# jonepatr/lets_face_it

Measured on AMD Instinct MI355X. Metric: FLAME frames/s, full training step (fwd+bwd+clip+Adam), final_model.yaml batch 256 per GPU, higher is better.
Workload: dtype f32 (GEMM operands split into bf16 hi+lo, f32 accumulate; three products in the forward GEMMs, two in the backward GEMMs)

## Files before the change

### include/lfi.h

```cpp
#ifndef LFI_H
#define LFI_H

#ifdef __cplusplus
extern "C" {
#endif

#define LFI_OK 0
#define LFI_ERR_ARG (-1)
#define LFI_ERR_LAUNCH (-2)
#define LFI_ERR_UNSUPPORTED (-3)

const char* lfi_last_error(void);
int lfi_version(void);

typedef struct {
  int M, N, K;
  const float* A; long lda; int a_kcontig;
  const float* B; long ldb; int b_kcontig;
  float* C; long ldc;
  const float* bias;
  const float* G; long ldg;
  int batch; long strideA, strideB, strideC, strideBias, strideG;
  int accumulate;
  int act; float slope;
  int splitk; float* work;
  int precision;
  int a_bf16;
  float* colsum_part; long ld_part;
} lfi_gemm_desc;

long lfi_gemm_work_floats(const lfi_gemm_desc* d);
long lfi_gemm_colpart_rows(const lfi_gemm_desc* d);
int lfi_gemm_f32(const lfi_gemm_desc* d, void* stream);

long lfi_planes_elems(long rows, int cols);
int lfi_planes_from_f32(const float* X, long ldx, long rows, int cols, void* planes, void* stream);
typedef struct {
  int M, N, K;
  const void* Ap; int a_nkt; long a_stride;
  const void* Bp; int b_nkt; long b_stride;
  float* C; long ldc;
  const float* bias; const float* G; long ldg;
  int batch; long strideC, strideBias, strideG;
  int accumulate, act; float slope;
  int skip;
  int a_fmt, b_fmt;
  int splitk; float* work;
  int store_f32;
  void* Cr; int cr_nkt; long cr_col0;
  const void* Gr; int gr_nkt; long gr_col0;
  float* colsum_part; long ld_part;
  int out_hi_only;
  int tile;
} lfi_pgemm_desc;
long lfi_gemm_planes_work_floats(const lfi_pgemm_desc* d);
long lfi_gemm_planes_colpart_rows(const lfi_pgemm_desc* d);
int lfi_gemm_planes(const lfi_pgemm_desc* d, void* stream);

long lfi_colsum_work_floats(int rows, int cols, int batch);
int lfi_colsum_f32(const float* X, long ldx, long strideX, int rows, int cols, int batch,
                   float* out, long strideOut, float scale, int accumulate, float* work, void* stream);

int lfi_cols_fold(const float* src, long lds, long rows, const int* a, const int* b, int ncols, float* dst, long ldd,
                  void* stream);

typedef struct {
  int B, T, N, start;
  int hist, hid;
  int ldcond, col;
  int precision;
  int dup;
  int lstm;
  int bwd_two_products;
  int stash_f16;
} lfi_enc_desc;

long lfi_encode_windows_work_floats(const lfi_enc_desc* d);
int lfi_encode_windows_fwd(const lfi_enc_desc* d, const float* Xp, const float* whh ,
                           const float* b_ih, const float* b_hh, const float* mask,
                           float* cond, float* gates, float* hseq, float* work, void* stream);
int lfi_encode_windows_bwd(const lfi_enc_desc* d, const float* dcond, int lddcond, const float* whh ,
                           const float* gates, const float* hseq, float* dgi, float* dgh,
                           float* bias_part , float* work, void* stream);
long lfi_encode_windows_bias_rows(const lfi_enc_desc* d);
int lfi_encode_windows_bias_grads(const float* bias_part, long rows, int hid, float* db_ih, float* db_hh, void* stream);
int lfi_encode_windows_compact_dgi(const lfi_enc_desc* d);
int lfi_encode_windows_grad_stash_bf16(const lfi_enc_desc* d);
int lfi_encode_windows_stash_f16_ok(const lfi_enc_desc* d);
int lfi_encode_windows_fwd_variant(const lfi_enc_desc* d, int masked, int stashed);
int lfi_encode_windows_scatter(const lfi_enc_desc* d, const float* dgi, const float* dgh, const float* mask, float* dXp,
                               void* stream);
int lfi_gather_windows(const float* X, int B, int T, int dim, int N, int start, int hist, int incl, const float* mask,
                       float* cond, int ldcond, int col, void* stream);
int lfi_pad_rows(const float* src, long rows, int cols, long lds, float* dst, long ldd, void* stream);
int lfi_dropout_masks(int count, float* const* out, const long* n, const float* keep, unsigned long long seed,
                      unsigned long long offset, void* stream);
int lfi_fill_frame_nb(const float* base, float offset, int B, int N, float* cond, int ldcond, int col, void* stream);
int lfi_leaky_grad(float* d, long ldd, const float* y, long ldy, int rows, int cols, float slope, void* stream);

typedef struct {
  int B, N, C, H, D, Ks;
  int affine;
  int lstm;
  float scale_eps;
  int gemm_precision;
} lfi_flow_dims;

typedef struct {
  const float *an_bias, *an_logs;
  const float *inv_l, *inv_u, *inv_logs;
  const float *inv_p, *inv_sign;
  const float *inv_w;
  const float *w_ih, *w_hh, *b_ih, *b_hh;
  const float *w_fl, *b_fl, *l_fl;
} lfi_flow_params;

long lfi_flow_prep_floats(const lfi_flow_dims* d);
int lfi_flow_prep(const lfi_flow_dims* d, const lfi_flow_params* p, float* prep, int with_inverse, void* stream);

long lfi_flow_stash_floats(const lfi_flow_dims* d);
int lfi_flow_seq_fwd(const lfi_flow_dims* d, const lfi_flow_params* p, const float* prep,
                     const float* x0, int T, int start, const float* gic,
                     float* stash, float* z, float* nll, void* stream);
long lfi_flow_bstash_floats(const lfi_flow_dims* d);
int lfi_flow_seq_bwd(const lfi_flow_dims* d, const lfi_flow_params* p, const float* prep,
                     const float* stash, float gscale, float* bstash, void* stream);

int lfi_flow_bwd_emits_planes(const lfi_flow_dims* d);
int lfi_flow_seq_bwd_planes(const lfi_flow_dims* d, const lfi_flow_params* p, const float* prep,
                            const float* stash, float gscale, float* bstash, void* dgi_planes,
                            int hi_only , void* stream);

typedef struct {
  float *an_bias, *an_logs, *inv_l, *inv_u, *inv_logs, *inv_w;
  float *w_ih, *w_hh, *b_ih, *b_hh, *w_fl, *b_fl, *l_fl;
} lfi_flow_grads;
long lfi_flow_param_grads_work_floats(const lfi_flow_dims* d);
int lfi_flow_param_grads(const lfi_flow_dims* d, const lfi_flow_params* p, const float* prep,
                         const float* stash, const float* bstash, const float* c, long ldc, float gscale,
                         const lfi_flow_grads* g, int accumulate, float* work, void* stream,
                         void* bias_stream );

float* lfi_flow_stash_ptr(const lfi_flow_dims* d, float* stash, int which);
float* lfi_flow_bstash_ptr(const lfi_flow_dims* d, float* bstash, int which);

int lfi_actnorm_init_stats(const float* x, int rows, int C, double* sums, void* stream);
int lfi_actnorm_init_apply(const double* sums, double count, int C, float scale, float* bias, float* logs, void* stream);
int lfi_flow_step(const lfi_flow_dims* d, const lfi_flow_params* p, const float* prep, int k, int rows,
                  const float* x_in, long ldx, const float* h_prev, const float* c_prev, const float* gic_k,
                  float* x_out, long ldxo, float* h_out, float* c_out, float* ldc_acc, int reverse, void* stream);
int lfi_flow_seq_rev_ok(const lfi_flow_dims* d);
long lfi_flow_seq_rev_work_floats(const lfi_flow_dims* d);
int lfi_flow_seq_rev(const lfi_flow_dims* d, const lfi_flow_params* p, const float* prep, const float* z, const float* gic,
                     float* x_out, float* logdet, float* h, float* cstate, float* work, void* stream);

int lfi_actnorm_forward(const float* x, int rows, int C, const float* bias, const float* logs, int reverse, float* out,
                        float* dlogdet, void* stream);
long lfi_invconv_work_floats(int C);
int lfi_invconv_weights(int C, const float* inv_l, const float* inv_u, const float* inv_logs, const float* inv_p,
                        const float* inv_sign, const float* inv_w, int with_inverse, float* W, float* Winv, float* dlogdet,
                        float* work, void* stream);

typedef struct {
  int kind, hid;
  const float *w1, *b1;
  const float *w_ih, *w_hh, *b_ih, *b_hh;
  int col;
} lfi_p1enc;

long lfi_flow_sample_work_floats(const lfi_flow_dims* d);
long lfi_flow_sample_p1_work_floats(const lfi_flow_dims* d, const lfi_p1enc* e, int hist1);
int lfi_flow_sample_seq(const lfi_flow_dims* d, const lfi_flow_params* p, const float* prep,
                        const float* wct , long E, int hist1,
                        float* pre_static, const float* noise,
                        float* faces, int seq_len, int start, int nframes,
                        float* h, float* cstate ,
                        const lfi_p1enc* p1 , float* p1work ,
                        float* work, void* stream);
int lfi_absmax_f32(int count, const float* const* ptrs, const long* n, unsigned* out_bits, void* stream);
int lfi_stream_create_partial(int cus_per_xcd, void** stream);
int lfi_stream_destroy(void* stream);
int lfi_flow_sample_seq_from(const lfi_flow_dims* d, const lfi_flow_params* p, const float* prep,
                             const float* wct, long E, int hist1, float* pre_static, const float* noise,
                             float* faces, int seq_len, int start, int nframes, int first_frame,
                             float* h, float* cstate, const lfi_p1enc* p1, float* p1work, float* work, void* stream);
long lfi_flow_sample_nll_work_floats(const lfi_flow_dims* d);
int lfi_flow_sample_seq_nll(const lfi_flow_dims* d, const lfi_flow_params* p, const float* prep,
                            const float* wct, long E, int hist1, float* pre_static, const float* noise,
                            float* faces, int seq_len, int start, int nframes, int first_frame,
                            float* h, float* cstate, const lfi_p1enc* p1, float* p1work, float* work,
                            float* nll, float* nll_work, void* stream);
long lfi_flow_score_work_floats(const lfi_flow_dims* d);
int lfi_flow_score_seq_from(const lfi_flow_dims* d, const lfi_flow_params* p, const float* prep,
                            const float* wct, long E, int hist1, float* pre_static,
                            float* faces, int seq_len, int start, int nframes, int first_frame,
                            float* h, float* cstate, const lfi_p1enc* p1, float* p1work, float* work,
                            float* score_work, float* z, float* nll, void* stream);
long lfi_flow_step_rows_work_floats(const lfi_flow_dims* d);
int lfi_flow_step_rows_from(const lfi_flow_dims* d, const lfi_flow_params* p, const float* prep,
                            const float* wct, long E, int hist1, float* pre_static, const float* noise,
                            float* faces, int seq_len, int start, int nframes, int first_frame,
                            float* h, float* cstate, const lfi_p1enc* p1, float* p1work, float* work,
                            float* nll, float* nll_work, const int* observed, float* rows_work, void* stream);
int lfi_stream_advance(int B, int count, float* const* win, const float* const* src, const int* hist, const int* dim,
                       const float* noise, float* noise_dst, int C, float* frame_nb, unsigned* guard_bits, void* stream);
int lfi_stream_advance_rows(int B, int count, float* const* win, const float* const* src, const int* hist, const int* dim,
                            int face_win, const float* noise, float* noise_dst, int C, float* frame_nb,
                            const unsigned char* observed, int* role, unsigned* guard_bits, void* stream);
int lfi_stream_reset_rows(int B, int nrows, const int* rows, int count, float* const* win, const float* const* seed,
                          const long* seed_ld, const int* hist, const int* dim, const int* lead_zero, float* h, float* cstate,
                          int Ks, int H, float* frame_nb, unsigned* guard_bits, void* stream);
long lfi_stream_row_floats(int count, const int* hist, const int* dim, int Ks, int H, int lstm, int has_frame_nb);
int lfi_stream_save_rows(int B, int nrows, const int* rows, int count, const float* const* win, const int* hist, const int* dim,
                         const float* h, const float* cstate, int Ks, int H, const float* frame_nb, int zero_state, float* out,
                         long ld_out, void* stream);
int lfi_stream_load_rows(int B, int nrows, const int* rows, const int* entries, int nentries, int count, float* const* win,
                         const int* hist, const int* dim, float* h, float* cstate, int Ks, int H, float* frame_nb, const float* in,
                         long ld_in, unsigned* guard_bits, void* stream);

int lfi_grad_sumsq(const float* g, long n, double* sumsq, double* work , void* stream);
int lfi_adam_clip_step(float* p, const float* g, float* m, float* v, long n, const double* sumsq,
                       float clip, float gmul, float lr, float beta1, float beta2, float eps, int step_count,
                       void* stream);

int lfi_adam_clip_step_ex(float* p, const float* g, float* m, float* v, float* vmax, long n, const double* sumsq, float clip,
                          float gmul, float lr, float beta1, float beta2, float eps, float weight_decay, int step_count,
                          const float* hyper, void* stream);

int lfi_sgd_clip_step(float* p, const float* g, float* buf, long n, const double* sumsq, float clip, float gmul, float lr,
                      float momentum, float dampening, float weight_decay, int nesterov, int step_count, void* stream);
int lfi_rmsprop_clip_step(float* p, const float* g, float* sq, float* buf, float* gavg, long n, const double* sumsq, float clip,
                          float gmul, float lr, float alpha, float eps, float weight_decay, float momentum, void* stream);

int lfi_set_step_params(void* params, unsigned long long seed, unsigned long long offset, float step_size, float inv_sqrt_bc2,
                        void* stream);
int lfi_dropout_masks_dev(int count, float* const* out, const long* n, const float* keep, const unsigned long long* seed_offset,
                          void* stream);
int lfi_adam_clip_step_dev(float* p, const float* g, float* m, float* v, long n, const double* sumsq, float clip, float gmul,
                           float beta1, float beta2, float eps, const float* hyper , void* stream);

int lfi_gather_sequences(const float* src, long rows, int dim, const long* starts, int B, int T, float* dst, void* stream);
int lfi_jerk_mean(const float* x, int B, int T, int C, float* out, double* work , void* stream);

int lfi_debug_set_stamps(void* device_buffer);
int lfi_selftest_mfma(int* out, void* stream);

#ifdef __cplusplus
}
#endif
#endif
```

### lets_face_it_amd/_lib.py

```python
import ctypes as C
import os

_HERE = os.path.dirname(os.path.abspath(__file__))
LIB_PATH = os.environ.get("LFI_LIB_PATH") or os.path.join(_HERE, "liblfi_hip.so")

c_float_p = C.POINTER(C.c_float)
c_double_p = C.POINTER(C.c_double)


class GemmDesc(C.Structure):
    _fields_ = [
        ("M", C.c_int), ("N", C.c_int), ("K", C.c_int),
        ("A", C.c_void_p), ("lda", C.c_long), ("a_kcontig", C.c_int),
        ("B", C.c_void_p), ("ldb", C.c_long), ("b_kcontig", C.c_int),
        ("C", C.c_void_p), ("ldc", C.c_long),
        ("bias", C.c_void_p),
        ("G", C.c_void_p), ("ldg", C.c_long),
        ("batch", C.c_int), ("strideA", C.c_long), ("strideB", C.c_long), ("strideC", C.c_long),
        ("strideBias", C.c_long), ("strideG", C.c_long),
        ("accumulate", C.c_int),
        ("act", C.c_int), ("slope", C.c_float),
        ("splitk", C.c_int), ("work", C.c_void_p),
        ("precision", C.c_int), ("a_bf16", C.c_int),
        ("colsum_part", C.c_void_p), ("ld_part", C.c_long),
    ]


class PGemmDesc(C.Structure):
    _fields_ = [
        ("M", C.c_int), ("N", C.c_int), ("K", C.c_int),
        ("Ap", C.c_void_p), ("a_nkt", C.c_int), ("a_stride", C.c_long),
        ("Bp", C.c_void_p), ("b_nkt", C.c_int), ("b_stride", C.c_long),
        ("C", C.c_void_p), ("ldc", C.c_long),
        ("bias", C.c_void_p), ("G", C.c_void_p), ("ldg", C.c_long),
        ("batch", C.c_int), ("strideC", C.c_long), ("strideBias", C.c_long), ("strideG", C.c_long),
        ("accumulate", C.c_int), ("act", C.c_int), ("slope", C.c_float), ("skip", C.c_int),
        ("a_fmt", C.c_int), ("b_fmt", C.c_int),
        ("splitk", C.c_int), ("work", C.c_void_p),
        ("store_f32", C.c_int),
        ("Cr", C.c_void_p), ("cr_nkt", C.c_int), ("cr_col0", C.c_long),
        ("Gr", C.c_void_p), ("gr_nkt", C.c_int), ("gr_col0", C.c_long),
        ("colsum_part", C.c_void_p), ("ld_part", C.c_long),
        ("out_hi_only", C.c_int), ("tile", C.c_int),
    ]


class EncDesc(C.Structure):
    _fields_ = [("B", C.c_int), ("T", C.c_int), ("N", C.c_int), ("start", C.c_int),
                ("hist", C.c_int), ("hid", C.c_int), ("ldcond", C.c_int), ("col", C.c_int), ("precision", C.c_int),
                ("dup", C.c_int), ("lstm", C.c_int), ("bwd_two_products", C.c_int), ("stash_f16", C.c_int)]


class FlowDims(C.Structure):
    _fields_ = [("B", C.c_int), ("N", C.c_int), ("C", C.c_int), ("H", C.c_int), ("D", C.c_int), ("Ks", C.c_int),
                ("affine", C.c_int), ("lstm", C.c_int), ("scale_eps", C.c_float), ("gemm_precision", C.c_int)]


_FLOW_PARAM_FIELDS = ["an_bias", "an_logs", "inv_l", "inv_u", "inv_logs", "inv_p", "inv_sign", "inv_w",
                      "w_ih", "w_hh", "b_ih", "b_hh", "w_fl", "b_fl", "l_fl"]
_FLOW_GRAD_FIELDS = ["an_bias", "an_logs", "inv_l", "inv_u", "inv_logs", "inv_w",
                     "w_ih", "w_hh", "b_ih", "b_hh", "w_fl", "b_fl", "l_fl"]


class P1Enc(C.Structure):
    _fields_ = [("kind", C.c_int), ("hid", C.c_int), ("w1", C.c_void_p), ("b1", C.c_void_p), ("w_ih", C.c_void_p),
                ("w_hh", C.c_void_p), ("b_ih", C.c_void_p), ("b_hh", C.c_void_p), ("col", C.c_int)]


class FlowParams(C.Structure):
    _fields_ = [(n, C.c_void_p) for n in _FLOW_PARAM_FIELDS]


class FlowGrads(C.Structure):
    _fields_ = [(n, C.c_void_p) for n in _FLOW_GRAD_FIELDS]


class LfiError(RuntimeError):
    pass


_lib = None


def lib():
    global _lib
    if _lib is not None:
        return _lib
    if not os.path.exists(LIB_PATH):
        raise LfiError(
            "liblfi_hip.so not found at %s: build it with `make -C lets_face_it_amd/csrc` "
            "(there is no fallback path)" % LIB_PATH)
    L = C.CDLL(LIB_PATH)
    vp, i, l, f, d = C.c_void_p, C.c_int, C.c_long, C.c_float, C.c_double
    P = C.POINTER
    sig = {
        "lfi_last_error": (C.c_char_p, []),
        "lfi_version": (i, []),
        "lfi_gemm_work_floats": (l, [P(GemmDesc)]),
        "lfi_gemm_f32": (i, [P(GemmDesc), vp]),
        "lfi_gemm_colpart_rows": (l, [P(GemmDesc)]),
        "lfi_planes_elems": (l, [l, i]),
        "lfi_planes_from_f32": (i, [vp, l, l, i, vp, vp]),
        "lfi_gemm_planes": (i, [P(PGemmDesc), vp]),
        "lfi_flow_bwd_emits_planes": (i, [P(FlowDims)]),
        "lfi_flow_seq_bwd_planes": (i, [P(FlowDims), P(FlowParams), vp, vp, f, vp, vp, i, vp]),
        "lfi_encode_windows_grad_stash_bf16": (i, [P(EncDesc)]),
        "lfi_encode_windows_stash_f16_ok": (i, [P(EncDesc)]),
        "lfi_encode_windows_fwd_variant": (i, [P(EncDesc), i, i]),
        "lfi_gemm_planes_work_floats": (l, [P(PGemmDesc)]),
        "lfi_gemm_planes_colpart_rows": (l, [P(PGemmDesc)]),
        "lfi_colsum_work_floats": (l, [i, i, i]),
        "lfi_colsum_f32": (i, [vp, l, l, i, i, i, vp, l, f, i, vp, vp]),
        "lfi_cols_fold": (i, [vp, l, l, vp, vp, i, vp, l, vp]),
        "lfi_encode_windows_work_floats": (l, [P(EncDesc)]),
        "lfi_encode_windows_fwd": (i, [P(EncDesc), vp, vp, vp, vp, vp, vp, vp, vp, vp, vp]),
        "lfi_encode_windows_bwd": (i, [P(EncDesc), vp, i, vp, vp, vp, vp, vp, vp, vp, vp]),
        "lfi_encode_windows_bias_rows": (l, [P(EncDesc)]),
        "lfi_encode_windows_bias_grads": (i, [vp, l, i, vp, vp, vp]),
        "lfi_encode_windows_compact_dgi": (i, [P(EncDesc)]),
        "lfi_encode_windows_scatter": (i, [P(EncDesc), vp, vp, vp, vp, vp]),
        "lfi_gather_windows": (i, [vp, i, i, i, i, i, i, i, vp, vp, i, i, vp]),
        "lfi_pad_rows": (i, [vp, l, i, l, vp, l, vp]),
        "lfi_dropout_masks": (i, [i, P(vp), P(l), P(f), C.c_ulonglong, C.c_ulonglong, vp]),
        "lfi_dropout_masks_dev": (i, [i, P(vp), P(l), P(f), vp, vp]),
        "lfi_set_step_params": (i, [vp, C.c_ulonglong, C.c_ulonglong, f, f, vp]),
        "lfi_adam_clip_step_dev": (i, [vp, vp, vp, vp, l, vp, f, f, f, f, f, vp, vp]),
        "lfi_leaky_grad": (i, [vp, l, vp, l, i, i, f, vp]),
        "lfi_fill_frame_nb": (i, [vp, f, i, i, vp, i, i, vp]),
        "lfi_flow_prep_floats": (l, [P(FlowDims)]),
        "lfi_flow_prep": (i, [P(FlowDims), P(FlowParams), vp, i, vp]),
        "lfi_flow_stash_floats": (l, [P(FlowDims)]),
        "lfi_flow_bstash_floats": (l, [P(FlowDims)]),
        "lfi_flow_stash_ptr": (vp, [P(FlowDims), vp, i]),
        "lfi_flow_bstash_ptr": (vp, [P(FlowDims), vp, i]),
        "lfi_flow_seq_fwd": (i, [P(FlowDims), P(FlowParams), vp, vp, i, i, vp, vp, vp, vp, vp]),
        "lfi_flow_seq_bwd": (i, [P(FlowDims), P(FlowParams), vp, vp, f, vp, vp]),
        "lfi_flow_param_grads_work_floats": (l, [P(FlowDims)]),
        "lfi_flow_param_grads": (i, [P(FlowDims), P(FlowParams), vp, vp, vp, vp, l, f, P(FlowGrads), i, vp, vp, vp]),
        "lfi_actnorm_init_stats": (i, [vp, i, i, vp, vp]),
        "lfi_actnorm_init_apply": (i, [vp, d, i, f, vp, vp, vp]),
        "lfi_flow_step": (i, [P(FlowDims), P(FlowParams), vp, i, i, vp, l, vp, vp, vp, vp, l, vp, vp, vp, i, vp]),
        "lfi_flow_seq_rev_ok": (i, [P(FlowDims)]),
        "lfi_flow_seq_rev_work_floats": (l, [P(FlowDims)]),
        "lfi_flow_seq_rev": (i, [P(FlowDims), P(FlowParams), vp, vp, vp, vp, vp, vp, vp, vp, vp]),
        "lfi_flow_sample_work_floats": (l, [P(FlowDims)]),
        "lfi_flow_sample_p1_work_floats": (l, [P(FlowDims), P(P1Enc), i]),
        "lfi_flow_sample_seq": (i, [P(FlowDims), P(FlowParams), vp, vp, l, i, vp, vp, vp, i, i, i, vp, vp, P(P1Enc), vp, vp,
                                    vp]),
        "lfi_flow_sample_seq_from": (i, [P(FlowDims), P(FlowParams), vp, vp, l, i, vp, vp, vp, i, i, i, i, vp, vp, P(P1Enc), vp, vp,
                                         vp]),
        "lfi_flow_sample_nll_work_floats": (l, [P(FlowDims)]),
        "lfi_flow_sample_seq_nll": (i, [P(FlowDims), P(FlowParams), vp, vp, l, i, vp, vp, vp, i, i, i, i, vp, vp, P(P1Enc), vp, vp,
                                        vp, vp, vp]),
        "lfi_flow_score_work_floats": (l, [P(FlowDims)]),
        "lfi_flow_score_seq_from": (i, [P(FlowDims), P(FlowParams), vp, vp, l, i, vp, vp, i, i, i, i, vp, vp, P(P1Enc), vp, vp,
                                        vp, vp, vp, vp]),
        "lfi_flow_step_rows_work_floats": (l, [P(FlowDims)]),
        "lfi_flow_step_rows_from": (i, [P(FlowDims), P(FlowParams), vp, vp, l, i, vp, vp, vp, i, i, i, i, vp, vp, P(P1Enc), vp, vp,
                                        vp, vp, vp, vp, vp]),
        "lfi_absmax_f32": (i, [i, P(vp), P(l), vp, vp]),
        "lfi_stream_advance": (i, [i, i, P(vp), P(vp), P(i), P(i), vp, vp, i, vp, vp, vp]),
        "lfi_stream_advance_rows": (i, [i, i, P(vp), P(vp), P(i), P(i), i, vp, vp, i, vp, vp, vp, vp, vp]),
        "lfi_stream_reset_rows": (i, [i, i, P(i), i, P(vp), P(vp), P(l), P(i), P(i), P(i), vp, vp, i, i, vp, vp, vp]),
        "lfi_stream_row_floats": (l, [i, P(i), P(i), i, i, i, i]),
        "lfi_stream_save_rows": (i, [i, i, P(i), i, P(vp), P(i), P(i), vp, vp, i, i, vp, i, vp, l, vp]),
        "lfi_stream_load_rows": (i, [i, i, P(i), P(i), i, i, P(vp), P(i), P(i), vp, vp, i, i, vp, vp, l, vp, vp]),
        "lfi_stream_create_partial": (i, [i, P(vp)]),
        "lfi_stream_destroy": (i, [vp]),
        "lfi_grad_sumsq": (i, [vp, l, vp, vp, vp]),
        "lfi_adam_clip_step": (i, [vp, vp, vp, vp, l, vp, f, f, f, f, f, f, i, vp]),
        "lfi_adam_clip_step_ex": (i, [vp, vp, vp, vp, vp, l, vp, f, f, f, f, f, f, f, i, vp, vp]),
        "lfi_sgd_clip_step": (i, [vp, vp, vp, l, vp, f, f, f, f, f, f, i, i, vp]),
        "lfi_rmsprop_clip_step": (i, [vp, vp, vp, vp, vp, l, vp, f, f, f, f, f, f, f, vp]),
        "lfi_actnorm_forward": (i, [vp, i, i, vp, vp, i, vp, vp, vp]),
        "lfi_invconv_work_floats": (l, [i]),
        "lfi_invconv_weights": (i, [i, vp, vp, vp, vp, vp, vp, i, vp, vp, vp, vp, vp]),
        "lfi_gather_sequences": (i, [vp, l, i, vp, i, i, vp, vp]),
        "lfi_jerk_mean": (i, [vp, i, i, i, vp, vp, vp]),
        "lfi_selftest_mfma": (i, [vp, vp]),
        "lfi_debug_set_stamps": (i, [vp]),
    }
    for name, (res, args) in sig.items():
        fn = getattr(L, name)
        fn.restype = res
        fn.argtypes = args
    _lib = L
    return L


EXPORTS = [
    "lfi_last_error", "lfi_version", "lfi_gemm_work_floats", "lfi_gemm_f32", "lfi_gemm_colpart_rows", "lfi_planes_elems", "lfi_planes_from_f32",
    "lfi_gemm_planes", "lfi_gemm_planes_work_floats", "lfi_gemm_planes_colpart_rows",
    "lfi_flow_bwd_emits_planes", "lfi_flow_seq_bwd_planes", "lfi_encode_windows_grad_stash_bf16", "lfi_encode_windows_stash_f16_ok", "lfi_encode_windows_fwd_variant", "lfi_colsum_work_floats",
    "lfi_colsum_f32", "lfi_cols_fold", "lfi_encode_windows_work_floats", "lfi_encode_windows_fwd", "lfi_encode_windows_bwd",
    "lfi_encode_windows_bias_rows", "lfi_encode_windows_bias_grads",
    "lfi_encode_windows_scatter", "lfi_encode_windows_compact_dgi", "lfi_gather_windows", "lfi_pad_rows", "lfi_dropout_masks", "lfi_leaky_grad", "lfi_fill_frame_nb", "lfi_flow_prep_floats", "lfi_flow_prep",
    "lfi_flow_stash_floats", "lfi_flow_bstash_floats", "lfi_flow_stash_ptr", "lfi_flow_bstash_ptr",
    "lfi_flow_seq_fwd", "lfi_flow_seq_bwd", "lfi_flow_param_grads_work_floats", "lfi_flow_param_grads",
    "lfi_actnorm_init_stats", "lfi_actnorm_init_apply", "lfi_flow_step", "lfi_flow_seq_rev_ok", "lfi_flow_seq_rev_work_floats",
    "lfi_flow_seq_rev", "lfi_flow_sample_work_floats",
    "lfi_flow_sample_p1_work_floats", "lfi_flow_sample_seq", "lfi_flow_sample_seq_from", "lfi_flow_sample_nll_work_floats", "lfi_flow_sample_seq_nll", "lfi_flow_score_work_floats", "lfi_flow_score_seq_from", "lfi_flow_step_rows_work_floats", "lfi_flow_step_rows_from", "lfi_absmax_f32", "lfi_stream_advance", "lfi_stream_advance_rows", "lfi_stream_reset_rows", "lfi_stream_row_floats",
    "lfi_stream_save_rows", "lfi_stream_load_rows", "lfi_stream_create_partial", "lfi_stream_destroy", "lfi_grad_sumsq", "lfi_adam_clip_step", "lfi_adam_clip_step_ex",
    "lfi_sgd_clip_step", "lfi_rmsprop_clip_step", "lfi_set_step_params", "lfi_dropout_masks_dev", "lfi_adam_clip_step_dev", "lfi_selftest_mfma", "lfi_debug_set_stamps",
    "lfi_gather_sequences", "lfi_jerk_mean", "lfi_actnorm_forward", "lfi_invconv_work_floats", "lfi_invconv_weights",
]


def translate_oom(fn):
    import functools

    import torch

    @functools.wraps(fn)
    def wrapper(*args, **kwargs):
        try:
            return fn(*args, **kwargs)
        except torch.OutOfMemoryError as e:
            msg = str(e)
            if msg.startswith("CUDA out of memory"):
                raise
            raise torch.OutOfMemoryError("CUDA out of memory. [ROCm: " + msg + "]") from e

    return wrapper


def check(rc, what=""):
    if rc != 0:
        msg = lib().lfi_last_error()
        raise LfiError("%s failed (%d): %s" % (what or "lfi call", rc, msg.decode() if msg else ""))


def ptr(t):
    return None if t is None else t.data_ptr()
```

### lets_face_it_amd/csrc/lfi_gemm_common.h

```cpp
#pragma once
#include <stdarg.h>
#include <stdio.h>
#include <stdlib.h>

#include "lfi_common.h"

namespace {

#ifndef LFI_GEMM_BKT
#define LFI_GEMM_BKT 16
#endif
#ifndef LFI_GEMM_LDSPIPE
#define LFI_GEMM_LDSPIPE 1
#endif
constexpr int BKT = LFI_GEMM_BKT;
#define LFI_GSKIP(bit) (XT >= 2 && (g.skip & (bit)))

struct GemmArgs {
  int M, N, K;
  const float* A; long lda;
  const float* B; long ldb;
  float* C; long ldc;
  const float* bias;
  const float* G; long ldg;
  long strideA, strideB, strideC, strideBias, strideG;
  int accumulate, act;
  float slope;
  int splitk, kchunk;
  float* work;
  int tiles_m, tiles_n;
  int vecA, vecB;
  int vecC;
  const __bf16* Ap; const __bf16* Bp;
  int nkt, nktA, nktB;
  long pstrideA, pstrideB;
  float* colpart; long ldpart;
  int gm;
  int skip;
  int storeC;
  __bf16* Cr; int nktCr; long colCr;
  const __bf16* Gr; int nktGr; long colGr;
  int hiOnly;
};

__device__ __forceinline__ float apply_act(float v, int act, float slope, const float* G, long gidx) {
  if (act == 1) return v > 0.0f ? v : v * slope;
  if (act == 2) return G[gidx] > 0.0f ? v : v * slope;
  return v;
}

typedef __bf16 bf16x8 __attribute__((ext_vector_type(8)));
typedef __bf16 bf16x4 __attribute__((ext_vector_type(4)));
extern __shared__ __attribute__((aligned(16))) __bf16 xsmem[];
typedef __bf16 bf16x2 __attribute__((ext_vector_type(2)));
typedef float float2_t __attribute__((ext_vector_type(2)));

__device__ __forceinline__ void split2(float a, float b, unsigned* hi, unsigned* lo) {
  const bf16x2 h = __builtin_convertvector((float2_t){a, b}, bf16x2);
  const unsigned hb = __builtin_bit_cast(unsigned, h);
  const float ha = __builtin_bit_cast(float, hb << 16), hbv = __builtin_bit_cast(float, hb & 0xffff0000u);
  const bf16x2 l = __builtin_convertvector((float2_t){a - ha, b - hbv}, bf16x2);
  *hi = hb;
  *lo = __builtin_bit_cast(unsigned, l);
}


__device__ __forceinline__ void gemm_epilogue(const GemmArgs& g, const f32x16 (&acc)[2][2], int m0, int n0, int wm, int wn,
                                              int l31, int half, int batch, int split) {
  const bool partial = g.splitk > 1;
  float* __restrict__ Cb = partial ? g.work + ((long)batch * g.splitk + split) * (long)g.M * g.N : g.C + batch * g.strideC;
  const long ldc = partial ? g.N : g.ldc;
  const float* bias = g.bias ? g.bias + batch * g.strideBias : nullptr;
  const float* G = g.G ? g.G + batch * g.strideG : nullptr;
  const bool need_c = !partial && g.accumulate != 0, need_g = !partial && g.act == 2;
#pragma unroll
  for (int mt = 0; mt < 2; ++mt)
#pragma unroll
    for (int nt = 0; nt < 2; ++nt) {
      const int col = n0 + wn * 64 + nt * 32 + l31;
      if (col >= g.N) continue;
      const float bv = (!partial && bias) ? bias[col] : 0.0f;
      float cold[16], gold[16];
#pragma unroll
      for (int r = 0; r < 16; ++r) {
        const int row = min(m0 + wm * 64 + mt * 32 + (r & 3) + 8 * (r >> 2) + 4 * half, g.M - 1);
        cold[r] = need_c ? Cb[(long)row * ldc + col] : 0.0f;
        gold[r] = need_g ? G[(long)row * g.ldg + col] : 1.0f;
      }
#pragma unroll
      for (int r = 0; r < 16; ++r) {
        const int row = m0 + wm * 64 + mt * 32 + (r & 3) + 8 * (r >> 2) + 4 * half;
        if (row >= g.M) continue;
        float v = acc[mt][nt][r];
        if (!partial) {
          v += bv;
          if (g.accumulate == 2) v += cold[r];
          if (g.act == 1) v = v > 0.0f ? v : v * g.slope;
          else if (g.act == 2) v = gold[r] > 0.0f ? v : v * g.slope;
          if (g.accumulate == 1) v += cold[r];
        }
        Cb[(long)row * ldc + col] = v;
      }
    }
}

template <int BN>
__device__ __forceinline__ void gemm_epilogue_n(const GemmArgs& g, const f32x16 (&acc)[2][2], int m0, int n0, int wm, int wn,
                                                int l31, int half, int batch, int split) {
  gemm_epilogue(g, acc, m0, n0, wm, wn, l31, half, batch, split);
}

typedef unsigned u32x4 __attribute__((ext_vector_type(4)));
__device__ __forceinline__ u32x4 pg_u4(const uint4& v) { return (u32x4){v.x, v.y, v.z, v.w}; }
template <int BN, int NTH>
__device__ __forceinline__ void gemm_emit_planes(const GemmArgs& g, const float* lds, int rows_per_pass, int row0, int n0, int batch) {
  constexpr int WLD = BN + 4;
  const int tid = threadIdx.x, lane = tid & 63, wave = tid >> 6;
  constexpr int NW = NTH / 64;
  const long gcol0 = (long)batch * g.strideC + n0;
  if (!g.Cr) return;
  constexpr int KT = BN / 16;
  const int nb = (rows_per_pass / 32) * KT;
  const int uoff = lfi_u_plane_offset(lane & 31, lane >> 5);
  for (int b = wave; b < nb; b += NW) {
    const int rtl = b / KT, ktl = b - rtl * KT;
    if (row0 + rtl * 32 >= g.M || n0 + ktl * 16 >= g.N) continue;
    const int r = rtl * 32 + (lane & 31), c = ktl * 16 + (lane >> 5) * 8;
    const f32x4 a = *reinterpret_cast<const f32x4*>(lds + r * WLD + c), bq = *reinterpret_cast<const f32x4*>(lds + r * WLD + c + 4);
    const bool rok = row0 + r < g.M;
    float v[8] = {a[0], a[1], a[2], a[3], bq[0], bq[1], bq[2], bq[3]};
#pragma unroll
    for (int e = 0; e < 8; ++e) v[e] = (rok && n0 + c + e < g.N) ? v[e] : 0.0f;
    uint4 h, l;
    split2(v[0], v[1], &h.x, &l.x); split2(v[2], v[3], &h.y, &l.y);
    split2(v[4], v[5], &h.z, &l.z); split2(v[6], v[7], &h.w, &l.w);
    const long rt = (row0 + rtl * 32) >> 5, kt = (g.colCr + gcol0 + ktl * 16) >> 4;
    char* dst = reinterpret_cast<char*>(g.Cr) + ((rt * g.nktCr + kt) * 2) * 1024 + uoff;
    __builtin_nontemporal_store(pg_u4(h), reinterpret_cast<u32x4*>(dst));
    if (!g.hiOnly) __builtin_nontemporal_store(pg_u4(l), reinterpret_cast<u32x4*>(dst + 1024));
  }
}
template <int BN, int NTH>
__device__ __forceinline__ void gemm_sign_tile_from_planes(const GemmArgs& g, float* lds, int rows_per_pass, int row0, int n0, int batch) {
  constexpr int WLD = BN + 4, KT = BN / 16, NW = NTH / 64;
  const int tid = threadIdx.x, lane = tid & 63, wave = tid >> 6;
  const long gcol0 = (long)batch * g.strideC + n0;
  const int nb = (rows_per_pass / 32) * KT;
  for (int b = wave; b < nb; b += NW) {
    const int rtl = b / KT, ktl = b - rtl * KT;
    const int r = rtl * 32 + (lane & 31), c = ktl * 16 + (lane >> 5) * 8;
    uint4 h = {0u, 0u, 0u, 0u};
    if (row0 + rtl * 32 < g.M && n0 + ktl * 16 < g.N) {
      const long rt = (row0 + rtl * 32) >> 5, kt = (g.colGr + gcol0 + ktl * 16) >> 4;
      h = *reinterpret_cast<const uint4*>(reinterpret_cast<const char*>(g.Gr) + ((rt * g.nktGr + kt) * 2) * 1024 +
                                          lfi_u_plane_offset(lane & 31, lane >> 5));
    }
    f32x4 a, bq;
    a[0] = __builtin_bit_cast(float, h.x << 16); a[1] = __builtin_bit_cast(float, h.x & 0xffff0000u);
    a[2] = __builtin_bit_cast(float, h.y << 16); a[3] = __builtin_bit_cast(float, h.y & 0xffff0000u);
    bq[0] = __builtin_bit_cast(float, h.z << 16); bq[1] = __builtin_bit_cast(float, h.z & 0xffff0000u);
    bq[2] = __builtin_bit_cast(float, h.w << 16); bq[3] = __builtin_bit_cast(float, h.w & 0xffff0000u);
    *reinterpret_cast<f32x4*>(lds + r * WLD + c) = a;
    *reinterpret_cast<f32x4*>(lds + r * WLD + c + 4) = bq;
  }
}

template <int BN, int NTH = 256, int MT = 2, bool COLP = false, bool PL = false, bool L16 = false, typename ACC>
__device__ __forceinline__ void gemm_epilogue_wide(const GemmArgs& g, const ACC& acc, float* lds, int rows_per_pass,
                                                   int m0, int n0, int wm, int wn, int l31, int half, int batch, int split, int bm,
                                                   bool has_acc = true) {
  constexpr int WLD = BN + 4;
  constexpr int F4 = BN / 4;
  constexpr int SWEEP = NTH / F4;
  const int tid = threadIdx.x;
  const bool partial = g.splitk > 1;
  float* __restrict__ Cb = partial ? g.work + ((long)batch * g.splitk + split) * (long)g.M * g.N : g.C + batch * g.strideC;
  const long ldc = partial ? g.N : g.ldc;
  const float* bias = g.bias ? g.bias + batch * g.strideBias : nullptr;
  const float* G = g.G ? g.G + batch * g.strideG : nullptr;
  const bool need_c = !partial && g.accumulate != 0, need_g = !partial && g.act == 2;
  const int rrow = tid / F4, c4 = (tid % F4) * 4;
  const int col_g = n0 + c4;
  for (int p0 = 0; p0 < bm; p0 += rows_per_pass) {
    if (PL && need_g && g.Gr) {
      gemm_sign_tile_from_planes<BN, NTH>(g, lds, rows_per_pass, m0 + p0, n0, batch);
      __syncthreads();
    } else if (need_c || need_g) {
      const float* src = need_g ? G : Cb;
      const long lds_src = need_g ? g.ldg : ldc;
      for (int r = rrow; r < rows_per_pass; r += SWEEP) {
        const int row = m0 + p0 + r;
        f32x4 v = {0.f, 0.f, 0.f, 0.f};
        if (row < g.M && col_g < g.N) {
          if (col_g + 3 < g.N) v = *reinterpret_cast<const f32x4*>(src + (long)row * lds_src + col_g);
          else
            for (int j = 0; j < 4; ++j)
              if (col_g + j < g.N) v[j] = src[(long)row * lds_src + col_g + j];
        }
        *reinterpret_cast<f32x4*>(lds + r * WLD + c4) = v;
      }
      __syncthreads();
    }
    if constexpr (L16) {
      static_assert(!L16 || MT == 2, "16 x 16 accumulator tiles: 64-row patches");
      const int lane = threadIdx.x & 63, c15 = lane & 15, r4 = (lane >> 4) * 4;
#pragma unroll
      for (int mi = 0; mi < 4; ++mi)
        if (has_acc && wm * 64 + mi * 16 >= p0 && wm * 64 + mi * 16 < p0 + rows_per_pass)
#pragma unroll
        for (int ni = 0; ni < 4; ++ni) {
          const int cl = wn * 64 + ni * 16 + c15;
          const int col = n0 + cl;
          const float bv = (!partial && bias && col < g.N) ? bias[col] : 0.0f;
#pragma unroll
          for (int r = 0; r < 4; ++r) {
            const int rl = wm * 64 - p0 + mi * 16 + r4 + r;
            float v = acc[mi][ni][r];
            if (!partial) {
              v += bv;
              const float o = (need_c || need_g) ? lds[rl * WLD + cl] : 0.0f;
              if (g.accumulate == 2) v += o;
              if (g.act == 1) v = v > 0.0f ? v : v * g.slope;
              else if (g.act == 2) v = o > 0.0f ? v : v * g.slope;
              if (g.accumulate == 1) v += o;
            }
            lds[rl * WLD + cl] = v;
          }
        }
    } else
    if (has_acc) {
#pragma unroll
      for (int mt = 0; mt < MT; ++mt)
        if (wm * MT * 32 + mt * 32 >= p0 && wm * MT * 32 + mt * 32 < p0 + rows_per_pass)
#pragma unroll
        for (int nt = 0; nt < 2; ++nt) {
          const int cl = wn * 64 + nt * 32 + l31;
          const int col = n0 + cl;
          const float bv = (!partial && bias && col < g.N) ? bias[col] : 0.0f;
#pragma unroll
          for (int r = 0; r < 16; ++r) {
            const int rl = wm * MT * 32 - p0 + mt * 32 + (r & 3) + 8 * (r >> 2) + 4 * half;
            float v = acc[mt][nt][r];
            if (!partial) {
              v += bv;
              const float o = (need_c || need_g) ? lds[rl * WLD + cl] : 0.0f;
              if (g.accumulate == 2) v += o;
              if (g.act == 1) v = v > 0.0f ? v : v * g.slope;
              else if (g.act == 2) v = o > 0.0f ? v : v * g.slope;
              if (g.accumulate == 1) v += o;
            }
            lds[rl * WLD + cl] = v;
          }
        }
    }
    __syncthreads();
    if (PL && !partial) gemm_emit_planes<BN, NTH>(g, lds, rows_per_pass, m0 + p0, n0, batch);
    f32x4 csum = {0.f, 0.f, 0.f, 0.f};
    for (int r = rrow; r < rows_per_pass && (!PL || partial || g.storeC || COLP); r += SWEEP) {
      const int row = m0 + p0 + r;
      if (row < g.M && col_g < g.N) {
        const f32x4 v = *reinterpret_cast<const f32x4*>(lds + r * WLD + c4);
        if (COLP) csum += v;
        if (PL && !partial && !g.storeC) continue;
        if (col_g + 3 < g.N) {
#ifndef LFI_EPI_NT_MODE
#define LFI_EPI_NT_MODE 2
#endif
          if (LFI_EPI_NT_MODE == 0 || (LFI_EPI_NT_MODE == 2 && partial)) *reinterpret_cast<f32x4*>(Cb + (long)row * ldc + col_g) = v;
          else __builtin_nontemporal_store(v, reinterpret_cast<f32x4*>(Cb + (long)row * ldc + col_g));
        }
        else
          for (int j = 0; j < 4; ++j)
            if (col_g + j < g.N) Cb[(long)row * ldc + col_g + j] = v[j];
      }
    }
    if (COLP && g.colpart && !partial) {
      __syncthreads();
      *reinterpret_cast<f32x4*>(lds + rrow * WLD + c4) = csum;
      __syncthreads();
      if (tid < BN && n0 + tid < g.N) {
        float v = 0.0f;
        for (int i = 0; i < SWEEP; ++i) v += lds[i * WLD + tid];
        const int npass = (bm + rows_per_pass - 1) / rows_per_pass;
        g.colpart[((long)(m0 / bm) * npass + p0 / rows_per_pass) * g.ldpart + batch * g.strideC + n0 + tid] = v;
      }
      __syncthreads();
    } else if (p0 + rows_per_pass < bm) __syncthreads();
  }
}

typedef unsigned gu32x4 __attribute__((ext_vector_type(4)));
typedef unsigned gu32x2 __attribute__((ext_vector_type(2)));
template <int MODE>
__device__ __forceinline__ void gemm_epilogue_direct16(const GemmArgs& g, const f32x4 (&acc)[4][4], int m0, int n0, int wm, int wn, int lane,
                                                       int batch, int split) {
  const int l15 = lane & 15, g4 = lane >> 4;
  const int r0 = m0 + wm * 64, c0 = n0 + wn * 64;
  const float* bias = g.bias ? g.bias + batch * g.strideBias : nullptr;
  f32x4 bv[4];
#pragma unroll
  for (int j = 0; j < 4; ++j) {
    const int col = c0 + 16 * j + 4 * g4;
    bv[j] = (f32x4){0.f, 0.f, 0.f, 0.f};
    if (bias && col < g.N) bv[j] = *reinterpret_cast<const f32x4*>(bias + col);
  }
  static_assert(MODE == 3 || MODE == 4, "plane outputs only");
  f32x4 csum[4];
#pragma unroll
  for (int j = 0; j < 4; ++j) csum[j] = (f32x4){0.f, 0.f, 0.f, 0.f};
  {
    const long gcol0 = g.colCr + (long)batch * g.strideC + c0;
#pragma unroll
    for (int i = 0; i < 4; ++i) {
      const int row = r0 + 16 * i + l15;
      const bool blk = (r0 + 16 * (i & ~1)) < g.M;
      const long rt = (r0 + 16 * i) >> 5;
      const __amdgpu_buffer_rsrc_t rs = __builtin_amdgcn_make_buffer_rsrc(reinterpret_cast<char*>(g.Cr) + (rt * g.nktCr + (gcol0 >> 4)) * 2048, 0,
                                                                         0x7fffffff, 0x00020000);
      const unsigned voff = (unsigned)(lfi_u_plane_offset(16 * (i & 1) + l15, g4 >> 1) + (g4 & 1) * 8);
      __amdgpu_buffer_rsrc_t rg = rs;
      if constexpr (MODE == 4) {
        const long ggcol0 = g.colGr + (long)batch * g.strideC + c0;
        rg = __builtin_amdgcn_make_buffer_rsrc(const_cast<char*>(reinterpret_cast<const char*>(g.Gr)) + (rt * g.nktGr + (ggcol0 >> 4)) * 2048, 0,
                                               0x7fffffff, 0x00020000);
      }
#pragma unroll
      for (int j = 0; j < 4; ++j) {
        const int col = c0 + 16 * j + 4 * g4;
        f32x4 v = acc[i][j] + bv[j];
        if constexpr (MODE == 4) {
          gu32x2 m2 = {0u, 0u};
          if (blk && c0 + 16 * j < g.N) m2 = __builtin_amdgcn_raw_buffer_load_b64(rg, voff, 2048 * j, 0);
          const float o0 = __builtin_bit_cast(float, m2[0] << 16), o1 = __builtin_bit_cast(float, m2[0] & 0xffff0000u);
          const float o2 = __builtin_bit_cast(float, m2[1] << 16), o3 = __builtin_bit_cast(float, m2[1] & 0xffff0000u);
          v[0] = o0 > 0.0f ? v[0] : v[0] * g.slope; v[1] = o1 > 0.0f ? v[1] : v[1] * g.slope;
          v[2] = o2 > 0.0f ? v[2] : v[2] * g.slope; v[3] = o3 > 0.0f ? v[3] : v[3] * g.slope;
        } else if (g.act == 1) {
#pragma unroll
          for (int r = 0; r < 4; ++r) v[r] = v[r] > 0.0f ? v[r] : v[r] * g.slope;
        }
        if (row >= g.M || col >= g.N) v = (f32x4){0.f, 0.f, 0.f, 0.f};
        if constexpr (MODE == 4) csum[j] += v;
        uint2 h, l;
        split2(v[0], v[1], &h.x, &l.x);
        split2(v[2], v[3], &h.y, &l.y);
        if (blk && c0 + 16 * j < g.N) {
          __builtin_amdgcn_raw_buffer_store_b64((gu32x2){h.x, h.y}, rs, voff, 2048 * j, 2);
          if (!g.hiOnly) __builtin_amdgcn_raw_buffer_store_b64((gu32x2){l.x, l.y}, rs, voff, 2048 * j + 1024, 2);
        }
      }
    }
  }
  if constexpr (MODE == 4) {
    if (g.colpart) {
#pragma unroll
      for (int j = 0; j < 4; ++j) {
        f32x4 v = csum[j];
#pragma unroll
        for (int o = 1; o < 16; o <<= 1) {
#pragma unroll
          for (int r = 0; r < 4; ++r) v[r] += __shfl_xor(v[r], o, 64);
        }
        const int col = c0 + 16 * j + 4 * g4;
        if (l15 == 0 && col < g.N)
          *reinterpret_cast<f32x4*>(g.colpart + ((long)(m0 >> 7) * 2 + wm) * g.ldpart + (long)batch * g.strideC + col) = v;
      }
    }
  }
}

__device__ __forceinline__ void gemm_tile_of_block(const GemmArgs& g, int* tm, int* tn, int* batch, int* split) {
  const int ntile = g.tiles_m * g.tiles_n;
  const long total = (long)gridDim.x * gridDim.y * gridDim.z;
  long lin = blockIdx.x + (long)gridDim.x * (blockIdx.y + (long)gridDim.y * blockIdx.z);
  {
    const long q = total >> 3, idx = lin >> 3;
    const int r = (int)(total & 7), xcd = (int)(lin & 7);
    lin = (xcd < r ? xcd * (q + 1) : r * (q + 1) + (xcd - r) * q) + idx;
  }
  int bid = (int)(lin % ntile);
  const long rest = lin / ntile;
  *batch = (int)(rest % gridDim.y);
  *split = (int)(rest / gridDim.y);
  const int GM = g.gm > 0 ? g.gm : 8;
  const int per_group = GM * g.tiles_n;
  const int grp = bid / per_group, in_grp = bid - grp * per_group;
  const int rows_here = min(GM, g.tiles_m - grp * GM);
  *tm = grp * GM + in_grp % rows_here;
  *tn = in_grp / rows_here;
}

#ifndef LFI_EPI_ROWS
#define LFI_EPI_ROWS 128
#endif

__global__ __launch_bounds__(256) void gemm_splitk_reduce_kernel(GemmArgs g) {
  const long mn = (long)g.M * g.N;
  const int batch = blockIdx.y;
  const float* bias = g.bias ? g.bias + batch * g.strideBias : nullptr;
  const float* G = g.G ? g.G + batch * g.strideG : nullptr;
  float* C = g.C + batch * g.strideC;
  for (long i = (long)blockIdx.x * 256 + threadIdx.x; i < mn; i += (long)gridDim.x * 256) {
    const int row = (int)(i / g.N), col = (int)(i % g.N);
    const float* w = g.work + (long)batch * g.splitk * mn + i;
    float v = 0.0f;
    int s = 0;
    for (; s + 8 <= g.splitk; s += 8) {
      float t[8];
#pragma unroll
      for (int u = 0; u < 8; ++u) t[u] = w[(long)(s + u) * mn];
#pragma unroll
      for (int u = 0; u < 8; ++u) v += t[u];
    }
    for (; s < g.splitk; ++s) v += w[(long)s * mn];
    if (bias) v += bias[col];
    if (g.accumulate == 2) v += C[(long)row * g.ldc + col];
    v = apply_act(v, g.act, g.slope, G, (long)row * g.ldg + col);
    if (g.accumulate == 1) v += C[(long)row * g.ldc + col];
    C[(long)row * g.ldc + col] = v;
  }
}

__global__ __launch_bounds__(256) void gemm_splitk_reduce4_kernel(GemmArgs g) {
  const long mn = (long)g.M * g.N, mn4 = mn >> 2;
  const int n4 = g.N >> 2;
  const int batch = blockIdx.y;
  const float* bias = g.bias ? g.bias + batch * g.strideBias : nullptr;
  const float* G = g.G ? g.G + batch * g.strideG : nullptr;
  float* C = g.C + batch * g.strideC;
  for (long i = (long)blockIdx.x * 256 + threadIdx.x; i < mn4; i += (long)gridDim.x * 256) {
    const int row = (int)(i / n4), col = (int)(i - (long)row * n4) * 4;
    const float* w = g.work + (long)batch * g.splitk * mn + 4 * i;
    f32x4 v = {0.f, 0.f, 0.f, 0.f};
    int s = 0;
    for (; s + 8 <= g.splitk; s += 8) {
      f32x4 t[8];
#pragma unroll
      for (int u = 0; u < 8; ++u) t[u] = __builtin_nontemporal_load(reinterpret_cast<const f32x4*>(w + (long)(s + u) * mn));
#pragma unroll
      for (int u = 0; u < 8; ++u) v += t[u];
    }
    for (; s < g.splitk; ++s) v += __builtin_nontemporal_load(reinterpret_cast<const f32x4*>(w + (long)s * mn));
    f32x4* cp = reinterpret_cast<f32x4*>(C + (long)row * g.ldc + col);
    f32x4 c0 = {0.f, 0.f, 0.f, 0.f};
    if (g.accumulate) c0 = *cp;
#pragma unroll
    for (int j = 0; j < 4; ++j) {
      float x = v[j];
      if (bias) x += bias[col + j];
      if (g.accumulate == 2) x += c0[j];
      x = apply_act(x, g.act, g.slope, G, (long)row * g.ldg + col + j);
      if (g.accumulate == 1) x += c0[j];
      v[j] = x;
    }
    *cp = v;
  }
}

}
```

### lets_face_it_amd/csrc/lfi_pgemm.hip

```cpp
#include "lfi_gemm_common.h"
#include <type_traits>

namespace {

constexpr int QRING = 3;
constexpr int QSLOT = 24 * 1024;

typedef __attribute__((address_space(3))) void plds_void;
typedef __attribute__((address_space(1))) const void pglb_void;
typedef __bf16 pbf16x4 __attribute__((ext_vector_type(4)));
typedef __attribute__((address_space(3))) pbf16x4 plds_v4;

template <bool TF>
__device__ __forceinline__ bf16x8 pg_frag(const char* blk, int uoff, int toff) {
  if (!TF) return *reinterpret_cast<const bf16x8*>(blk + uoff);
  const pbf16x4 lo = __builtin_amdgcn_ds_read_tr16_b64_v4bf16((plds_v4*)(blk + toff));
  const pbf16x4 hi = __builtin_amdgcn_ds_read_tr16_b64_v4bf16((plds_v4*)(blk + (toff ^ 128)));
  bf16x8 r;
  r[0] = lo[0]; r[1] = lo[1]; r[2] = lo[2]; r[3] = lo[3];
  r[4] = hi[0]; r[5] = hi[1]; r[6] = hi[2]; r[7] = hi[3];
  return r;
}

#ifdef LFI_PG_EXP_16
__device__ __forceinline__ f32x16 pg_mfma16(bf16x8 a, bf16x8 b, f32x16 c) {
  f32x4 q0 = {c[0], c[1], c[2], c[3]}, q1 = {c[4], c[5], c[6], c[7]};
  q0 = __builtin_amdgcn_mfma_f32_16x16x32_bf16(a, b, q0, 0, 0, 0);
  q1 = __builtin_amdgcn_mfma_f32_16x16x32_bf16(a, b, q1, 0, 0, 0);
  c[0] = q0[0]; c[1] = q0[1]; c[2] = q0[2]; c[3] = q0[3];
  c[4] = q1[0]; c[5] = q1[1]; c[6] = q1[2]; c[7] = q1[3];
  return c;
}
#define PG_MFMA(a, b, c) pg_mfma16(a, b, c)
#else
#define PG_MFMA(a, b, c) __builtin_amdgcn_mfma_f32_32x32x16_bf16(a, b, c, 0, 0, 0)
#endif

template <bool AT, bool BT, bool COLP, int WMT, int WNT>
__global__ __launch_bounds__(512, 4) void gemm_planes_kernel(GemmArgs g) {
  constexpr int XT = 2;
  constexpr int NA = 4 * WMT;
  static_assert(WMT * WNT == 8 && NA + 4 * WNT == 24, "eight waves, 24 blocks per slot");
  const int tid = threadIdx.x;
  const int lane = tid & 63, wave = __builtin_amdgcn_readfirstlane(tid >> 6);
  const int l31 = lane & 31, half = lane >> 5;
  int tm, tn, batch, split;
  gemm_tile_of_block(g, &tm, &tn, &batch, &split);
  const int m0 = tm * 64 * WMT, n0 = tn * 64 * WNT;
  const bool noalo = LFI_GSKIP(1);
  const int ktc = g.kchunk >> 4;
  const int kt0 = split * ktc;
  const int nkt = max(min(g.nkt - kt0, ktc), 0);
  char* lds = reinterpret_cast<char*>(xsmem);
  const int tsub = lane >> 5, trow = ((lane & 31) >> 1) ^ (tsub << 2);
  const int lpT = tsub * 2048 + trow * 32 + (lane & 1) * 16, lpR = lane * 16;
  const char* baseA = reinterpret_cast<const char*>(g.Ap + batch * g.pstrideA) +
                      (AT ? (long)(tm * 2 * WMT) * 4096 + lpT : (long)(tm * 2 * WMT) * g.nktA * 2048 + lpR);
  const char* baseB = reinterpret_cast<const char*>(g.Bp + batch * g.pstrideB) +
                      (BT ? (long)(tn * 2 * WNT) * 4096 + lpT : (long)(tn * 2 * WNT) * g.nktB * 2048 + lpR);
  const char* src[3];
  int doff[3];
  bool srcB[3];
#pragma unroll
  for (int i = 0; i < 3; ++i) {
    const int j = wave * 3 + i;
    const int isB = j >= NA, jj = isB ? j - NA : j;
    const int plane = (!isB && noalo) ? 0 : (jj & 1);
    const long mt = jj >> 1;
    src[i] = (isB ? baseB + (BT ? mt * 4096 : mt * g.nktB * 2048) : baseA + (AT ? mt * 4096 : mt * g.nktA * 2048)) + plane * 1024;
    srcB[i] = isB != 0;
    doff[i] = j * 1024;
  }
  const long rowA = (long)g.nktA * 2048, rowB = (long)g.nktB * 2048;
  auto dma = [&](int kt, int slot) {
    const int ka = kt0 + max(min(kt, nkt - 1), 0);
    const long koA = AT ? (long)(ka >> 1) * rowA + (ka & 1) * 512 : (long)ka * 2048;
    const long koB = BT ? (long)(ka >> 1) * rowB + (ka & 1) * 512 : (long)ka * 2048;
#pragma unroll
    for (int i = 0; i < 3; ++i)
      __builtin_amdgcn_global_load_lds((pglb_void*)(src[i] + (srcB[i] ? koB : koA)), (plds_void*)(lds + slot * QSLOT + doff[i]), 16, 0, 0);
  };
  const int wm = wave / WNT, wn = wave % WNT;
  const int uoff = lfi_u_plane_offset(lane & 31, lane >> 5);
  const int tg = lane >> 4, tq = (lane >> 2) & 3, tp = lane & 3, tkh = tg >> 1, tmh = tg & 1;
  const int toff = tmh * 512 + (((tkh * 8 + tq) ^ (tmh << 2)) * 32) + (((tp >> 1) ^ tkh) << 4) + (tp & 1) * 8;
  const int fa = (wm * 4) * 1024;
  const int fb = NA * 1024 + (wn * 4) * 1024;
  auto fragA = [&](int slot, int off) { return pg_frag<AT>(lds + slot * QSLOT + fa + off, uoff, toff); };
  auto fragB = [&](int slot, int off) { return pg_frag<BT>(lds + slot * QSLOT + fb + off, uoff, toff); };

  f32x16 acc[2][2];
#pragma unroll
  for (int i = 0; i < 2; ++i)
#pragma unroll
    for (int j = 0; j < 2; ++j)
#pragma unroll
      for (int r = 0; r < 16; ++r) acc[i][j][r] = 0.0f;

  if (nkt > 0) {
    bf16x8 ah[2], al[2], bh[2], bl[2];
    dma(0, 0); dma(1, 1); dma(2, 2);
    asm volatile("s_waitcnt vmcnt(6)" ::: "memory");
    __builtin_amdgcn_s_barrier();
#pragma unroll
    for (int t2 = 0; t2 < 2; ++t2) {
      ah[t2] = fragA(0, (t2 * 2) * 1024);
      if (!noalo) al[t2] = fragA(0, (t2 * 2 + 1) * 1024);
      else al[t2] = ah[t2];
      bh[t2] = fragB(0, (t2 * 2) * 1024); bl[t2] = fragB(0, (t2 * 2 + 1) * 1024);
    }
    asm volatile("s_waitcnt vmcnt(3)\n\ts_waitcnt lgkmcnt(0)" ::: "memory");
    __builtin_amdgcn_s_barrier();

    int cur = 0;
    for (int t = 0; t < nkt; ++t) {
      const int nxt = cur == 2 ? 0 : cur + 1;
      bf16x8 nah[2], nal[2], nbh[2], nbl[2];
      dma(t + 3, cur);
      __builtin_amdgcn_sched_barrier(0);
      if (!LFI_GSKIP(1)) {
#pragma unroll
        for (int nt = 0; nt < 2; ++nt) acc[0][nt] = PG_MFMA(al[0], bh[nt], acc[0][nt]);
      }
      if (!LFI_GSKIP(2)) {
#pragma unroll
        for (int nt = 0; nt < 2; ++nt) acc[0][nt] = PG_MFMA(ah[0], bl[nt], acc[0][nt]);
      }
#pragma unroll
      for (int nt = 0; nt < 2; ++nt) acc[0][nt] = PG_MFMA(ah[0], bh[nt], acc[0][nt]);
      __builtin_amdgcn_sched_barrier(0);
      nah[0] = fragA(nxt, 0);
      if (!noalo) nal[0] = fragA(nxt, 1024);
      else nal[0] = nah[0];
#pragma unroll
      for (int nt = 0; nt < 2; ++nt) { nbh[nt] = fragB(nxt, (nt * 2) * 1024); nbl[nt] = fragB(nxt, (nt * 2 + 1) * 1024); }
      __builtin_amdgcn_sched_barrier(0);
      if (!LFI_GSKIP(1)) {
#pragma unroll
        for (int nt = 0; nt < 2; ++nt) acc[1][nt] = PG_MFMA(al[1], bh[nt], acc[1][nt]);
      }
      if (!LFI_GSKIP(2)) {
#pragma unroll
        for (int nt = 0; nt < 2; ++nt) acc[1][nt] = PG_MFMA(ah[1], bl[nt], acc[1][nt]);
      }
#pragma unroll
      for (int nt = 0; nt < 2; ++nt) acc[1][nt] = PG_MFMA(ah[1], bh[nt], acc[1][nt]);
      __builtin_amdgcn_sched_barrier(0);
      nah[1] = fragA(nxt, 2048);
      if (!noalo) nal[1] = fragA(nxt, 3072);
      else nal[1] = nah[1];
      asm volatile("s_waitcnt vmcnt(3)\n\ts_waitcnt lgkmcnt(0)" ::: "memory");
      __builtin_amdgcn_s_barrier();
#pragma unroll
      for (int i = 0; i < 2; ++i) { ah[i] = nah[i]; al[i] = nal[i]; bh[i] = nbh[i]; bl[i] = nbl[i]; }
      cur = nxt;
    }
    asm volatile("s_waitcnt vmcnt(0)" ::: "memory");
  }
  __syncthreads();
  if (g.vecC) gemm_epilogue_wide<64 * WNT, 512, 2, COLP, true>(g, acc, reinterpret_cast<float*>(xsmem), WNT == 4 ? 64 : 128, m0, n0, wm, wn,
                                                             l31, half, batch, split, 64 * WMT);
  else gemm_epilogue_n<64 * WNT>(g, acc, m0, n0, wm, wn, l31, half, batch, split);
}

#define PG_MFMA16(a, b, c) __builtin_amdgcn_mfma_f32_16x16x32_bf16(a, b, c, 0, 0, 0)
#define PG_MFMA16X(a, b, c) (TRP ? PG_MFMA16(b, a, c) : PG_MFMA16(a, b, c))
template <bool AT, bool BT, bool COLP, int WMT, int WNT, int TRP = 0>
__global__ __launch_bounds__(512, 4) void gemm_planes16_kernel(GemmArgs g) {
  constexpr int NA = 4 * WMT;
  static_assert(WMT * WNT == 8 && NA + 4 * WNT == 24, "eight waves, 24 blocks per slot");
  const int tid = threadIdx.x;
  const int lane = tid & 63, wave = __builtin_amdgcn_readfirstlane(tid >> 6);
  int tm, tn, batch, split;
  gemm_tile_of_block(g, &tm, &tn, &batch, &split);
  const int m0 = tm * 64 * WMT, n0 = tn * 64 * WNT;
  const int ktc = g.kchunk >> 4;
  const int kt0 = split * ktc;
  const int npair = max(min(g.nkt - kt0, ktc), 0) >> 1;
  char* lds = reinterpret_cast<char*>(xsmem);
  const long rowA = (long)g.nktA * 2048, rowB = (long)g.nktB * 2048;
  const char* baseA = reinterpret_cast<const char*>(g.Ap + batch * g.pstrideA) +
                      (AT ? (long)(tm * 2 * WMT) * 4096 + (long)(kt0 >> 1) * rowA : (long)(tm * 2 * WMT) * rowA + (long)kt0 * 2048);
  const char* baseB = reinterpret_cast<const char*>(g.Bp + batch * g.pstrideB) +
                      (BT ? (long)(tn * 2 * WNT) * 4096 + (long)(kt0 >> 1) * rowB : (long)(tn * 2 * WNT) * rowB + (long)kt0 * 2048);
  const int prow = lane >> 1, srow = prow ^ ((prow & 16) ? 4 : 0);
  const int laneR = lane * 16, laneT = srow * 32 + (lane & 1) * 16;
  int sof[3], doff[3];
#pragma unroll
  for (int i = 0; i < 3; ++i) {
    const int j = 8 * i + wave;
    const bool isB = 8 * i >= NA;
    const int jj = isB ? j - NA : j;
    const int mt = jj >> 1, h = jj & 1;
    const bool tr = isB ? BT : AT;
    sof[i] = (tr ? mt * 4096 : mt * (int)(isB ? rowB : rowA)) + h * 2048 + (isB ? 0 : 1024);
    doff[i] = j * 1024;
  }
#define PG_RSRC(ptr) __builtin_amdgcn_make_buffer_rsrc(const_cast<char*>(ptr), 0, 0x7fffffff, 0x00020000)
  auto dma = [&](int ph, int slot) {
    const int pp = max(min(ph >> 1, npair - 1), 0);
    const char* pa = baseA + (AT ? pp * rowA : (long)pp * 4096);
    const char* pb = baseB + (BT ? pp * rowB : (long)pp * 4096);
#pragma unroll
    for (int i = 0; i < 3; ++i) {
      const bool isB = 8 * i >= NA;
      __builtin_amdgcn_raw_ptr_buffer_load_lds(PG_RSRC(isB ? pb : pa), (plds_void*)(lds + slot * QSLOT + doff[i]), 16,
                                               (isB ? BT : AT) ? laneT : laneR, sof[i] + ((ph & 1) ? (isB ? 1024 : -1024) : 0), 0, 0);
    }
  };
#undef PG_RSRC
  const int wm = wave / WNT, wn = wave % WNT;
  const int g4 = lane >> 4, tq = (lane >> 2) & 3, tp = lane & 3;
  const int fo = (g4 & 1) * 1024 + lfi_u_plane_offset(lane & 15, g4 >> 1);
  const int kr = 16 * (g4 & 1) + 8 * (g4 >> 1) + tq;
  const int toff = (kr ^ ((kr & 16) ? 4 : 0)) * 32 + (((tp >> 1) ^ ((kr >> 3) & 1)) << 4) + (tp & 1) * 8;
  const char* ldsA = lds + (wm * 4) * 1024;
  const char* ldsB = lds + NA * 1024 + (wn * 4) * 1024;
  auto fragA = [&](int slot, int i) -> bf16x8 {
    if constexpr (AT) return pg_frag<true>(ldsA + slot * QSLOT + i * 1024, 0, toff);
    else return *reinterpret_cast<const bf16x8*>(ldsA + slot * QSLOT + (i >> 1) * 2048 + (i & 1) * 512 + fo);
  };
  auto fragB = [&](int slot, int i) -> bf16x8 {
    if constexpr (BT) return pg_frag<true>(ldsB + slot * QSLOT + i * 1024, 0, toff);
    else return *reinterpret_cast<const bf16x8*>(ldsB + slot * QSLOT + (i >> 1) * 2048 + (i & 1) * 512 + fo);
  };

  f32x4 acc[4][4];
#pragma unroll
  for (int i = 0; i < 4; ++i)
#pragma unroll
    for (int j = 0; j < 4; ++j) acc[i][j] = (f32x4){0.f, 0.f, 0.f, 0.f};

  if (npair > 0) {
    bf16x8 al[4], bh[4];
    dma(0, 0); dma(1, 1); dma(2, 2);
    asm volatile("s_waitcnt vmcnt(6)" ::: "memory");
    __builtin_amdgcn_s_barrier();
#pragma unroll
    for (int i = 0; i < 4; ++i) { al[i] = fragA(0, i); bh[i] = fragB(0, i); }
    asm volatile("s_waitcnt vmcnt(3)\n\ts_waitcnt lgkmcnt(0)" ::: "memory");
    __builtin_amdgcn_s_barrier();

    auto pair = [&](auto SX, int p) {
      constexpr int sx = decltype(SX)::value, sy = (sx + 1) % 3, sn = (sx + 2) % 3;
      bf16x8 ah[4], bl[4], nal[4], nbh[4];
      dma(2 * p + 3, sx);
      __builtin_amdgcn_sched_barrier(0);
#pragma unroll
      for (int i = 0; i < 4; ++i) {
#pragma unroll
        for (int j = 0; j < 4; ++j) acc[i][j] = PG_MFMA16X(al[i], bh[j], acc[i][j]);
        __builtin_amdgcn_sched_barrier(0);
        if (i == 0) {
#pragma unroll
          for (int q = 0; q < 4; ++q) ah[q] = fragA(sy, q);
        }
        bl[i] = fragB(sy, i);
        __builtin_amdgcn_sched_barrier(0);
      }
      asm volatile("s_waitcnt vmcnt(3)\n\ts_waitcnt lgkmcnt(0)" ::: "memory");
      __builtin_amdgcn_s_barrier();
      dma(2 * p + 4, sy);
      __builtin_amdgcn_sched_barrier(0);
#pragma unroll
      for (int i = 0; i < 4; ++i)
#pragma unroll
        for (int j = 0; j < 4; ++j) acc[i][j] = PG_MFMA16X(ah[i], bh[j], acc[i][j]);
      __builtin_amdgcn_sched_barrier(0);
#pragma unroll
      for (int i = 0; i < 4; ++i) {
#pragma unroll
        for (int j = 0; j < 4; ++j) acc[i][j] = PG_MFMA16X(ah[i], bl[j], acc[i][j]);
        __builtin_amdgcn_sched_barrier(0);
        if (i == 0) {
#pragma unroll
          for (int q = 0; q < 4; ++q) nbh[q] = fragB(sn, q);
        }
        nal[i] = fragA(sn, i);
        __builtin_amdgcn_sched_barrier(0);
      }
      asm volatile("s_waitcnt vmcnt(3)\n\ts_waitcnt lgkmcnt(0)" ::: "memory");
      __builtin_amdgcn_s_barrier();
#pragma unroll
      for (int i = 0; i < 4; ++i) { al[i] = nal[i]; bh[i] = nbh[i]; }
    };
    for (int p = 0; p < npair; p += 3) {
      pair(std::integral_constant<int, 0>{}, p);
      if (p + 1 >= npair) break;
      pair(std::integral_constant<int, 2>{}, p + 1);
      if (p + 2 >= npair) break;
      pair(std::integral_constant<int, 1>{}, p + 2);
    }
    asm volatile("s_waitcnt vmcnt(0)" ::: "memory");
  }
  if constexpr (TRP != 0) {
    int lanez = lane, m0z = m0, n0z = n0;
    asm volatile("" : "+v"(lanez), "+s"(m0z), "+s"(n0z));
    gemm_epilogue_direct16<TRP>(g, acc, m0z, n0z, wm, wn, lanez, batch, split);
  } else {
    __syncthreads();
    gemm_epilogue_wide<64 * WNT, 512, 2, COLP, true, true>(g, acc, reinterpret_cast<float*>(xsmem), WNT == 4 ? 64 : 128, m0, n0, wm, wn,
                                                           lane & 31, lane >> 5, batch, split, 64 * WMT);
  }
}

template <bool AT, bool COLP, int WMT, int WNT, int TRP = 0>
__global__ __launch_bounds__(512, 4) void gemm_planes16t_kernel(GemmArgs g) {
  constexpr int NA = 4 * WMT, NY = WNT / 2;
  static_assert(WMT * WNT == 8 && NA + 4 * WNT == 24, "eight waves, 24 blocks per slot");
  const int tid = threadIdx.x;
  const int lane = tid & 63, wave = __builtin_amdgcn_readfirstlane(tid >> 6);
  int tm, tn, batch, split;
  gemm_tile_of_block(g, &tm, &tn, &batch, &split);
  const int m0 = tm * 64 * WMT, n0 = tn * 64 * WNT;
  const int ktc = g.kchunk >> 4;
  const int kt0 = split * ktc;
  const int npair = max(min(g.nkt - kt0, ktc), 0) >> 1;
  char* lds = reinterpret_cast<char*>(xsmem);
  const long rowA = (long)g.nktA * 2048, rowB = (long)g.nktB * 2048;
  const char* baseA = reinterpret_cast<const char*>(g.Ap + batch * g.pstrideA) +
                      (AT ? (long)(tm * 2 * WMT) * 4096 + (long)(kt0 >> 1) * rowA : (long)(tm * 2 * WMT) * rowA + (long)kt0 * 2048);
  const char* baseB = reinterpret_cast<const char*>(g.Bp + batch * g.pstrideB) + (long)(tn * 2 * WNT) * 4096 + (long)(kt0 >> 1) * rowB;
  const int prow = lane >> 1, srow = prow ^ ((prow & 16) ? 4 : 0);
  const int laneR = lane * 16, laneT = srow * 32 + (lane & 1) * 16;
  int sofX[3], doffX[3], sofY[2], doffY[2];
#pragma unroll
  for (int i = 0; i < 3; ++i) {
    const int j = 8 * i + wave;
    const bool isB = 8 * i >= NA;
    const int jj = isB ? j - NA : j;
    const int mt = jj >> 1, h = jj & 1;
    sofX[i] = (isB || AT) ? mt * 4096 + h * 2048 : mt * (int)rowA + h * 2048;
    doffX[i] = j * 1024;
  }
#pragma unroll
  for (int i = 0; i < NY; ++i) {
    const int jj = 8 * i + wave;
    sofY[i] = (jj >> 1) * 4096 + (jj & 1) * 2048 + 1024;
    doffY[i] = (NA + jj) * 1024;
  }
#define PG_RSRC(ptr) __builtin_amdgcn_make_buffer_rsrc(const_cast<char*>(ptr), 0, 0x7fffffff, 0x00020000)
  auto dmaX = [&](int pair, int slot) {
    const int pp = max(min(pair, npair - 1), 0);
    const char* pa = baseA + (AT ? pp * rowA : (long)pp * 4096);
    const char* pb = baseB + pp * rowB;
#pragma unroll
    for (int i = 0; i < 3; ++i) {
      const bool isB = 8 * i >= NA;
      __builtin_amdgcn_raw_ptr_buffer_load_lds(PG_RSRC(isB ? pb : pa), (plds_void*)(lds + slot * QSLOT + doffX[i]), 16, (isB || AT) ? laneT : laneR,
                                               sofX[i], 0, 0);
    }
  };
  auto dmaY = [&](int pair, int slot) {
    const int pp = max(min(pair, npair - 1), 0);
    const char* pb = baseB + pp * rowB;
#pragma unroll
    for (int i = 0; i < NY; ++i)
      __builtin_amdgcn_raw_ptr_buffer_load_lds(PG_RSRC(pb), (plds_void*)(lds + slot * QSLOT + doffY[i]), 16, laneT, sofY[i], 0, 0);
  };
#undef PG_RSRC
  const int wm = wave / WNT, wn = wave % WNT;
  const int g4 = lane >> 4, tq = (lane >> 2) & 3, tp = lane & 3;
  const int fo = (g4 & 1) * 1024 + lfi_u_plane_offset(lane & 15, g4 >> 1);
  const int kr = 16 * (g4 & 1) + 8 * (g4 >> 1) + tq;
  const int toff = (kr ^ ((kr & 16) ? 4 : 0)) * 32 + (((tp >> 1) ^ ((kr >> 3) & 1)) << 4) + (tp & 1) * 8;
  const char* ldsA = lds + (wm * 4) * 1024;
  const char* ldsB = lds + NA * 1024 + (wn * 4) * 1024;
  auto fragA = [&](int slot, int i) -> bf16x8 {
    if constexpr (AT) return pg_frag<true>(ldsA + slot * QSLOT + i * 1024, 0, toff);
    else return *reinterpret_cast<const bf16x8*>(ldsA + slot * QSLOT + (i >> 1) * 2048 + (i & 1) * 512 + fo);
  };
  auto fragB = [&](int slot, int i) -> bf16x8 { return pg_frag<true>(ldsB + slot * QSLOT + i * 1024, 0, toff); };

  f32x4 acc[4][4];
#pragma unroll
  for (int i = 0; i < 4; ++i)
#pragma unroll
    for (int j = 0; j < 4; ++j) acc[i][j] = (f32x4){0.f, 0.f, 0.f, 0.f};

  if (npair > 0) {
    bf16x8 ah[4], bh[4];
    dmaX(0, 0); dmaY(0, 1); dmaX(1, 2);
    if (NY == 2) asm volatile("s_waitcnt vmcnt(5)" ::: "memory");
    else asm volatile("s_waitcnt vmcnt(4)" ::: "memory");
    __builtin_amdgcn_s_barrier();
#pragma unroll
    for (int i = 0; i < 4; ++i) { ah[i] = fragA(0, i); bh[i] = fragB(0, i); }
    asm volatile("s_waitcnt vmcnt(3)\n\ts_waitcnt lgkmcnt(0)" ::: "memory");
    __builtin_amdgcn_s_barrier();

    auto pair = [&](auto SX, int p) {
      constexpr int sx = decltype(SX)::value, sy = (sx + 1) % 3, sn = (sx + 2) % 3;
      bf16x8 bl[4], nah[4], nbh[4];
      dmaY(p + 1, sx);
      __builtin_amdgcn_sched_barrier(0);
#pragma unroll
      for (int i = 0; i < 4; ++i) {
#pragma unroll
        for (int j = 0; j < 4; ++j) acc[i][j] = PG_MFMA16X(ah[i], bh[j], acc[i][j]);
        __builtin_amdgcn_sched_barrier(0);
        bl[i] = fragB(sy, i);
        __builtin_amdgcn_sched_barrier(0);
      }
      if (NY == 2) asm volatile("s_waitcnt vmcnt(2)\n\ts_waitcnt lgkmcnt(0)" ::: "memory");
      else asm volatile("s_waitcnt vmcnt(1)\n\ts_waitcnt lgkmcnt(0)" ::: "memory");
      __builtin_amdgcn_s_barrier();
      dmaX(p + 2, sy);
      __builtin_amdgcn_sched_barrier(0);
#pragma unroll
      for (int i = 0; i < 4; ++i) {
#pragma unroll
        for (int j = 0; j < 4; ++j) acc[i][j] = PG_MFMA16X(ah[i], bl[j], acc[i][j]);
        __builtin_amdgcn_sched_barrier(0);
        if (i == 0) {
#pragma unroll
          for (int q = 0; q < 4; ++q) nbh[q] = fragB(sn, q);
        }
        nah[i] = fragA(sn, i);
        __builtin_amdgcn_sched_barrier(0);
      }
      asm volatile("s_waitcnt vmcnt(3)\n\ts_waitcnt lgkmcnt(0)" ::: "memory");
      __builtin_amdgcn_s_barrier();
#pragma unroll
      for (int i = 0; i < 4; ++i) { ah[i] = nah[i]; bh[i] = nbh[i]; }
    };
    for (int p = 0; p < npair; p += 3) {
      pair(std::integral_constant<int, 0>{}, p);
      if (p + 1 >= npair) break;
      pair(std::integral_constant<int, 2>{}, p + 1);
      if (p + 2 >= npair) break;
      pair(std::integral_constant<int, 1>{}, p + 2);
    }
    asm volatile("s_waitcnt vmcnt(0)" ::: "memory");
  }
  if constexpr (TRP != 0) {
    int lanez = lane, m0z = m0, n0z = n0;
    asm volatile("" : "+v"(lanez), "+s"(m0z), "+s"(n0z));
    gemm_epilogue_direct16<TRP>(g, acc, m0z, n0z, wm, wn, lanez, batch, split);
  } else {
    __syncthreads();
    gemm_epilogue_wide<64 * WNT, 512, 2, COLP, true, true>(g, acc, reinterpret_cast<float*>(xsmem), WNT == 4 ? 64 : 128, m0, n0, wm, wn,
                                                           lane & 31, lane >> 5, batch, split, 64 * WMT);
  }
}

__global__ __launch_bounds__(256) void planes_from_f32_kernel(const float* __restrict__ X, long ldx, int rows, int cols, long nblk,
                                                             int nkt, int vec, __bf16* __restrict__ out) {
  for (long idx = (long)blockIdx.x * 256 + threadIdx.x; idx < nblk * 64; idx += (long)gridDim.x * 256) {
    const int l = (int)(idx & 63);
    const long q = idx >> 6;
    const int kt = (int)(q % nkt);
    const long rt = q / nkt;
    const long row = rt * 32 + (l & 31);
    const int k0 = kt * 16 + 8 * (l >> 5);
    float v[8];
    if (row < rows && vec && k0 + 8 <= cols) {
      const f32x4 a = *reinterpret_cast<const f32x4*>(X + row * ldx + k0), b = *reinterpret_cast<const f32x4*>(X + row * ldx + k0 + 4);
      v[0] = a[0]; v[1] = a[1]; v[2] = a[2]; v[3] = a[3]; v[4] = b[0]; v[5] = b[1]; v[6] = b[2]; v[7] = b[3];
    } else {
#pragma unroll
      for (int e = 0; e < 8; ++e) v[e] = (row < rows && k0 + e < cols) ? X[row * ldx + k0 + e] : 0.0f;
    }
    uint4 h, lo;
    split2(v[0], v[1], &h.x, &lo.x); split2(v[2], v[3], &h.y, &lo.y);
    split2(v[4], v[5], &h.z, &lo.z); split2(v[6], v[7], &h.w, &lo.w);
    char* dst = reinterpret_cast<char*>(out) + q * 2048 + lfi_u_plane_offset(l & 31, l >> 5);
    *reinterpret_cast<uint4*>(dst) = h;
    *reinterpret_cast<uint4*>(dst + 1024) = lo;
  }
}

bool planes16_ok(const GemmArgs& a) {
  if (!lfi_env_on("LFI_PGEMM_16")) return false;
  return a.vecC && a.skip == 0 && (a.nkt & 1) == 0 && ((a.kchunk >> 4) & 1) == 0;
}

bool planes16t_ok(const GemmArgs& a) {
  if (!lfi_env_on("LFI_PGEMM_16T")) return false;
  return a.vecC && a.skip == 1 && (a.nkt & 1) == 0 && ((a.kchunk >> 4) & 1) == 0;
}

int planes16_direct_mode(const GemmArgs& a) {
  if (!lfi_env_on("LFI_PGEMM_DIRECT")) return 0;
  if (!(a.vecC && a.act != 2 && a.accumulate == 0 && !a.colpart && (a.N & 3) == 0) || a.splitk > 1) return 0;
  if (a.Cr && !a.storeC) return ((a.strideC & 31) == 0 && (a.colCr & 15) == 0) ? 3 : 0;
  return 0;
}

bool planes16_direct_mask_ok(const GemmArgs& a) {
  if (!lfi_env_on("LFI_PGEMM_DIRECT")) return false;
  return a.vecC && a.act == 2 && a.Gr && !a.G && a.accumulate == 0 && a.colpart && a.splitk == 1 && a.Cr && !a.storeC && !a.bias &&
         (a.N & 3) == 0 && (a.strideC & 31) == 0 && (a.colCr & 15) == 0 && (a.colGr & 15) == 0 && (a.ldpart & 3) == 0;
}

template <bool COLP, int WMT, int WNT>
int launch_planes(const GemmArgs& a, int at, int bt, dim3 grid, size_t lds, hipStream_t st) {
  static bool attr = false;
  if (!attr) {
    hipError_t e1 = hipFuncSetAttribute((const void*)gemm_planes_kernel<false, false, COLP, WMT, WNT>, hipFuncAttributeMaxDynamicSharedMemorySize, (int)lds);
    hipError_t e2 = hipFuncSetAttribute((const void*)gemm_planes_kernel<false, true, COLP, WMT, WNT>, hipFuncAttributeMaxDynamicSharedMemorySize, (int)lds);
    hipError_t e3 = hipFuncSetAttribute((const void*)gemm_planes_kernel<true, false, COLP, WMT, WNT>, hipFuncAttributeMaxDynamicSharedMemorySize, (int)lds);
    hipError_t e4 = hipFuncSetAttribute((const void*)gemm_planes_kernel<true, true, COLP, WMT, WNT>, hipFuncAttributeMaxDynamicSharedMemorySize, (int)lds);
    if (e1 != hipSuccess || e2 != hipSuccess || e3 != hipSuccess || e4 != hipSuccess) {
      lfi_set_error("lfi_gemm_planes: cannot reserve %zu bytes of LDS", lds);
      return LFI_ERR_LAUNCH;
    }
    attr = true;
  }
  if (bt && planes16t_ok(a)) {
    static bool attr16t = false;
    if (!attr16t) {
      hipError_t e1 = hipFuncSetAttribute((const void*)gemm_planes16t_kernel<false, COLP, WMT, WNT>, hipFuncAttributeMaxDynamicSharedMemorySize, (int)lds);
      hipError_t e2 = hipFuncSetAttribute((const void*)gemm_planes16t_kernel<true, COLP, WMT, WNT>, hipFuncAttributeMaxDynamicSharedMemorySize, (int)lds);
      if (e1 != hipSuccess || e2 != hipSuccess) {
        lfi_set_error("lfi_gemm_planes: cannot reserve %zu bytes of LDS", lds);
        return LFI_ERR_LAUNCH;
      }
      attr16t = true;
    }
    if (COLP && WMT == 2 && !at && planes16_direct_mask_ok(a)) {
      static bool attr4 = false;
      if (!attr4) {
        if (hipFuncSetAttribute((const void*)gemm_planes16t_kernel<false, true, 2, 4, 4>, hipFuncAttributeMaxDynamicSharedMemorySize, (int)lds) != hipSuccess) {
          lfi_set_error("lfi_gemm_planes: cannot reserve %zu bytes of LDS", lds);
          return LFI_ERR_LAUNCH;
        }
        attr4 = true;
      }
      hipLaunchKernelGGL((gemm_planes16t_kernel<false, true, 2, 4, 4>), grid, dim3(512), lds, st, a);
    } else if (at) hipLaunchKernelGGL((gemm_planes16t_kernel<true, COLP, WMT, WNT>), grid, dim3(512), lds, st, a);
    else hipLaunchKernelGGL((gemm_planes16t_kernel<false, COLP, WMT, WNT>), grid, dim3(512), lds, st, a);
  } else if (!at && !bt && planes16_ok(a) && !COLP && planes16_direct_mode(a)) {
    static bool attrd16 = false;
    if (!attrd16) {
      if (hipFuncSetAttribute((const void*)gemm_planes16_kernel<false, false, false, WMT, WNT, 3>, hipFuncAttributeMaxDynamicSharedMemorySize, (int)lds) != hipSuccess) {
        lfi_set_error("lfi_gemm_planes: cannot reserve %zu bytes of LDS", lds);
        return LFI_ERR_LAUNCH;
      }
      attrd16 = true;
    }
    hipLaunchKernelGGL((gemm_planes16_kernel<false, false, false, WMT, WNT, 3>), grid, dim3(512), lds, st, a);
  } else if (planes16_ok(a)) {
    static bool attr16 = false;
    if (!attr16) {
      bool ok = hipFuncSetAttribute((const void*)gemm_planes16_kernel<false, false, COLP, WMT, WNT>, hipFuncAttributeMaxDynamicSharedMemorySize, (int)lds) == hipSuccess;
      ok = ok && hipFuncSetAttribute((const void*)gemm_planes16_kernel<false, true, COLP, WMT, WNT>, hipFuncAttributeMaxDynamicSharedMemorySize, (int)lds) == hipSuccess;
      ok = ok && hipFuncSetAttribute((const void*)gemm_planes16_kernel<true, false, COLP, WMT, WNT>, hipFuncAttributeMaxDynamicSharedMemorySize, (int)lds) == hipSuccess;
      ok = ok && hipFuncSetAttribute((const void*)gemm_planes16_kernel<true, true, COLP, WMT, WNT>, hipFuncAttributeMaxDynamicSharedMemorySize, (int)lds) == hipSuccess;
      if (!ok) {
        lfi_set_error("lfi_gemm_planes: cannot reserve %zu bytes of LDS", lds);
        return LFI_ERR_LAUNCH;
      }
      attr16 = true;
    }
    if (!at && !bt) hipLaunchKernelGGL((gemm_planes16_kernel<false, false, COLP, WMT, WNT>), grid, dim3(512), lds, st, a);
    else if (!at) hipLaunchKernelGGL((gemm_planes16_kernel<false, true, COLP, WMT, WNT>), grid, dim3(512), lds, st, a);
    else if (!bt) hipLaunchKernelGGL((gemm_planes16_kernel<true, false, COLP, WMT, WNT>), grid, dim3(512), lds, st, a);
    else hipLaunchKernelGGL((gemm_planes16_kernel<true, true, COLP, WMT, WNT>), grid, dim3(512), lds, st, a);
  } else if (!at && !bt) hipLaunchKernelGGL((gemm_planes_kernel<false, false, COLP, WMT, WNT>), grid, dim3(512), lds, st, a);
  else if (!at) hipLaunchKernelGGL((gemm_planes_kernel<false, true, COLP, WMT, WNT>), grid, dim3(512), lds, st, a);
  else if (!bt) hipLaunchKernelGGL((gemm_planes_kernel<true, false, COLP, WMT, WNT>), grid, dim3(512), lds, st, a);
  else hipLaunchKernelGGL((gemm_planes_kernel<true, true, COLP, WMT, WNT>), grid, dim3(512), lds, st, a);
  return LFI_OK;
}

bool planes_tall_tile(const lfi_pgemm_desc* d) {
  if (d->tile == 1) return false;
  if (d->tile == 2) return true;
  const double w256 = (double)lfi_cdiv(d->N, 256) * 256.0 / d->N, w128 = (double)lfi_cdiv(d->N, 128) * 128.0 / d->N;
  return w128 < 0.9 * w256;
}

}

extern "C" long lfi_planes_elems(long rows, int cols) {
  if (rows <= 0 || cols <= 0) return 0;
  return ((rows + 255) / 256 * 256) * (long)((cols + 15) / 16 * 16) * 2;
}

extern "C" int lfi_planes_from_f32(const float* X, long ldx, long rows, int cols, void* planes, void* stream) {
  LFI_REQUIRE(rows >= 0 && cols >= 0, "lfi_planes_from_f32: bad dims %ld x %d", rows, cols);
  if (rows == 0 || cols == 0) return LFI_OK;
  LFI_REQUIRE(X && planes, "lfi_planes_from_f32: null pointer");
  LFI_REQUIRE((reinterpret_cast<uintptr_t>(planes) & 15) == 0, "lfi_planes_from_f32: planes must be 16-byte aligned");
  const int nkt = (cols + 15) / 16;
  const long nblk = (rows + 255) / 256 * 8 * nkt;
  const int vec = ((reinterpret_cast<uintptr_t>(X) & 15) == 0 && (ldx & 3) == 0) ? 1 : 0;
  const long threads = nblk * 64;
  hipLaunchKernelGGL(planes_from_f32_kernel, dim3((unsigned)min((threads + 255) / 256, 65535L * 8)), dim3(256), 0, (hipStream_t)stream,
                     X, ldx, (int)rows, cols, nblk, nkt, vec, reinterpret_cast<__bf16*>(planes));
  LFI_LAUNCH_CHECK("lfi_planes_from_f32");
  return LFI_OK;
}

extern "C" long lfi_gemm_planes_work_floats(const lfi_pgemm_desc* d) {
  if (!d || d->splitk <= 1) return 0;
  return (long)d->batch * d->splitk * d->M * d->N;
}

extern "C" long lfi_gemm_planes_colpart_rows(const lfi_pgemm_desc* d) {
  if (!d || d->M <= 0 || d->N <= 0 || d->splitk > 1) return 0;
  if (d->batch > 1 && !(d->strideC > 0 && d->strideC * d->batch <= d->ldc)) return 0;
  if (d->ldc % 4 != 0 || d->strideC % 4 != 0 || (d->act == 2 && d->accumulate != 0)) return 0;
  return planes_tall_tile(d) ? (long)lfi_cdiv(d->M, 256) * 2 : (long)lfi_cdiv(d->M, 128) * 2;
}

extern "C" int lfi_gemm_planes(const lfi_pgemm_desc* d, void* stream) {
  LFI_REQUIRE(d, "lfi_gemm_planes: null descriptor");
  LFI_REQUIRE(d->M >= 0 && d->N >= 0 && d->K >= 0 && d->batch >= 1 && d->batch <= 65535, "lfi_gemm_planes: bad dims M=%d N=%d K=%d batch=%d",
              d->M, d->N, d->K, d->batch);
  if (d->M == 0 || d->N == 0) return LFI_OK;
  const bool store = d->store_f32 != 0;
  LFI_REQUIRE(d->Ap && d->Bp && (d->C || !store), "lfi_gemm_planes: null operand");
  LFI_REQUIRE(store || d->Cr, "lfi_gemm_planes: store_f32 = 0 and no plane output: the result would go nowhere");
  LFI_REQUIRE(d->K > 0, "lfi_gemm_planes: K = 0");
  LFI_REQUIRE(d->act >= 0 && d->act <= 2 && (d->act != 2 || d->G || d->Gr), "lfi_gemm_planes: bad act %d", d->act);
  const int nkt = (d->K + 15) / 16;
  LFI_REQUIRE((d->a_fmt ? 2L * d->a_nkt >= (d->M + 15) / 16 : d->a_nkt >= nkt) && (d->b_fmt ? 2L * d->b_nkt >= (d->N + 15) / 16 : d->b_nkt >= nkt),
              "lfi_gemm_planes: plane buffers hold %ld / %ld column tiles per row tile: too few for this product", (long)d->a_nkt, (long)d->b_nkt);
  LFI_REQUIRE(d->a_nkt > 0 && d->b_nkt > 0, "lfi_gemm_planes: a_nkt / b_nkt = column tiles per row tile of the plane buffers");
  LFI_REQUIRE((reinterpret_cast<uintptr_t>(d->Ap) & 15) == 0 && (reinterpret_cast<uintptr_t>(d->Bp) & 15) == 0 &&
              (d->a_stride & 7) == 0 && (d->b_stride & 7) == 0, "lfi_gemm_planes: planes must be 16-byte aligned");
  int splitk = d->splitk < 1 ? 1 : d->splitk;
  if (splitk > nkt) splitk = nkt;
  LFI_REQUIRE(splitk == 1 || d->work, "lfi_gemm_planes: splitk needs a workspace");
  LFI_REQUIRE(splitk == 1 || (!d->Cr && !d->colsum_part && store), "lfi_gemm_planes: plane outputs / column sums need splitk = 1");
  const bool planes_io = d->Cr || d->Gr;
  if (planes_io) {
    LFI_REQUIRE(d->batch == 1 || (d->strideC > 0 && d->strideC * d->batch <= (d->C ? d->ldc : d->strideC * d->batch) && d->strideC % 32 == 0),
                "lfi_gemm_planes: plane outputs need batch entries side by side in C's columns, 32-column granular");
    LFI_REQUIRE(d->cr_col0 % 16 == 0 && d->gr_col0 % 16 == 0, "lfi_gemm_planes: plane outputs must start on block boundaries");
    LFI_REQUIRE((!d->Cr || (reinterpret_cast<uintptr_t>(d->Cr) & 15) == 0) && (!d->Gr || (reinterpret_cast<uintptr_t>(d->Gr) & 15) == 0),
                "lfi_gemm_planes: planes must be 16-byte aligned");
  }
  GemmArgs a = {};
  a.M = d->M; a.N = d->N; a.K = d->K;
  a.C = d->C; a.ldc = d->ldc; a.bias = d->bias; a.G = d->G; a.ldg = d->ldg;
  a.strideC = d->strideC; a.strideBias = d->strideBias; a.strideG = d->strideG;
  a.accumulate = d->accumulate; a.act = d->act; a.slope = d->slope;
  a.splitk = splitk;
  {
    int ktc = splitk > 1 ? lfi_cdiv(nkt, splitk) : nkt;
    if (splitk > 1 && (nkt & 1) == 0 && (ktc & 1) && (long)(splitk - 1) * (ktc + 1) < nkt) ++ktc;
    a.kchunk = ktc * 16;
  }
  a.work = d->work;
  a.Ap = reinterpret_cast<const __bf16*>(d->Ap); a.Bp = reinterpret_cast<const __bf16*>(d->Bp);
  a.nkt = nkt; a.nktA = (int)d->a_nkt; a.nktB = (int)d->b_nkt; a.pstrideA = d->a_stride; a.pstrideB = d->b_stride;
  a.skip = d->skip & 3;
  a.colpart = d->colsum_part; a.ldpart = d->ld_part;
  a.storeC = store ? 1 : 0;
  a.Cr = reinterpret_cast<__bf16*>(d->Cr); a.nktCr = d->cr_nkt; a.colCr = d->cr_col0;
  a.Gr = reinterpret_cast<const __bf16*>(d->Gr); a.nktGr = d->gr_nkt; a.colGr = d->gr_col0;
  {
    const bool partial = splitk > 1;
    const bool c_ok = partial ? (((long)d->M * d->N) % 4 == 0 && d->N % 4 == 0 && (reinterpret_cast<uintptr_t>(d->work) & 15) == 0)
                              : (!store || ((reinterpret_cast<uintptr_t>(d->C) & 15) == 0 && d->ldc % 4 == 0 && d->strideC % 4 == 0));
    const bool g_ok = d->act != 2 || d->Gr || ((reinterpret_cast<uintptr_t>(d->G) & 15) == 0 && d->ldg % 4 == 0 && d->strideG % 4 == 0);
    a.vecC = (c_ok && g_ok && !(d->act == 2 && d->accumulate != 0)) ? 1 : 0;
    LFI_REQUIRE(a.vecC || !(planes_io || d->colsum_part), "lfi_gemm_planes: plane outputs / column sums need 16-byte granular C rows");
  }
  a.hiOnly = d->out_hi_only ? 1 : 0;
  const bool tall = planes_tall_tile(d);
  a.tiles_m = lfi_cdiv(d->M, tall ? 256 : 128);
  a.tiles_n = lfi_cdiv(d->N, tall ? 128 : 256);
  {
    static int gm_env = -1;
    if (gm_env < 0) {
      const char* e = getenv("LFI_PGEMM_GM");
      gm_env = e ? atoi(e) : 0;
    }
    a.gm = gm_env > 0 ? gm_env : 8;
  }
  const size_t lds = (size_t)QRING * QSLOT;
  dim3 grid(a.tiles_m * a.tiles_n, d->batch, splitk);
  const int rc = tall ? (a.colpart ? launch_planes<true, 4, 2>(a, d->a_fmt, d->b_fmt, grid, lds, (hipStream_t)stream)
                                   : launch_planes<false, 4, 2>(a, d->a_fmt, d->b_fmt, grid, lds, (hipStream_t)stream))
                      : (a.colpart ? launch_planes<true, 2, 4>(a, d->a_fmt, d->b_fmt, grid, lds, (hipStream_t)stream)
                                   : launch_planes<false, 2, 4>(a, d->a_fmt, d->b_fmt, grid, lds, (hipStream_t)stream));
  if (rc) return rc;
  LFI_LAUNCH_CHECK("lfi_gemm_planes");
  if (splitk > 1) {
    const long mn = (long)d->M * d->N;
    auto al16 = [](const void* p) { return (reinterpret_cast<uintptr_t>(p) & 15) == 0; };
    const bool red4 = d->N % 4 == 0 && al16(d->work) && al16(d->C) && d->ldc % 4 == 0 && d->strideC % 4 == 0 &&
                      (!d->G || (al16(d->G) && d->ldg % 4 == 0 && d->strideG % 4 == 0));
    if (red4) {
      dim3 rgrid((unsigned)min((long)lfi_cdiv(mn / 4, 256), 2048L), d->batch);
      hipLaunchKernelGGL(gemm_splitk_reduce4_kernel, rgrid, dim3(256), 0, (hipStream_t)stream, a);
    } else {
      dim3 rgrid((unsigned)min((long)lfi_cdiv(mn, 256), 2048L), d->batch);
      hipLaunchKernelGGL(gemm_splitk_reduce_kernel, rgrid, dim3(256), 0, (hipStream_t)stream, a);
    }
    LFI_LAUNCH_CHECK("lfi_gemm_planes split-k reduce");
  }
  return LFI_OK;
}
```

### lets_face_it_amd/engine.py

```python
import atexit
import contextlib
import ctypes as C
import math
import os
import struct
import warnings
import weakref

import torch

from . import _lib
from ._lib import EncDesc, FlowDims, FlowGrads, FlowParams, GemmDesc, P1Enc, PGemmDesc, check, ptr, translate_oom
from .stream import SampleStream, StreamRows, check_return_nll

ENC_ORDER = ("p1_face", "p2_face", "p1_speech", "p2_speech")
FLOW_FIELDS = ("an_bias", "an_logs", "inv_l", "inv_u", "inv_logs", "inv_w", "w_ih", "w_hh", "b_ih", "b_hh",
               "wct", "bct", "w_fl", "b_fl", "l_fl")
ENC_LEAVES = ("weight_ih", "weight_hh", "bias_ih", "bias_hh")
BWD_CLASSES = ("dpre", "cond_wgrad", "cond_dgrad", "flow_pgrads", "enc_dwih", "enc_dwhh", "enc_bptt")


def _stream():
    return torch.cuda.current_stream().cuda_stream


class EncoderSpec:

    def __init__(self, name, enc, in_dim, hist, hid, dropout):
        self.name, self.enc, self.in_dim, self.hist, self.hid, self.dropout = name, enc, in_dim, hist, hid, dropout
        self.ng = 4 if enc == "lstm" else 3
        if enc in ("rnn", "lstm"):
            self.dim = 2 * hid
        elif enc == "mlp":
            self.dim = hid
        elif enc == "none":
            self.dim = in_dim * hist
        elif enc == "frame_nb":
            self.dim = 1
        else:
            raise NotImplementedError(
                "encoder type %r for %s: 'rnn' (GRU), 'lstm', 'mlp' and 'none' have HIP kernels in this build ('cnn' has a "
                "broken output size in the reference, models.py:48)" % (enc, name))
        self.col = 0
        self.win = (in_dim * hist + 3) // 4 * 4


class ModelSpec:

    def __init__(self, hparams):
        cond, glow, data = hparams.Conditioning, hparams.Glow, hparams.Data
        self.C = int(cond["p1_face"]["dim"])
        self.S = int(data["speech_dim"])
        self.D = int(cond["cond_dim"])
        self.H = int(glow["hidden_channels"])
        self.Ks = int(glow["K"]) * int(glow["L"])
        self.affine = 1 if glow["flow_coupling"] == "affine" else 0
        self.rnn_type = glow.get("rnn_type") or "gru"
        self.lu = bool(glow["LU_decomposed"])
        self.scale_eps = float(glow["scale_eps"])
        self.actnorm_scale = float(glow["actnorm_scale"])
        if glow["flow_permutation"] != "invconv":
            raise NotImplementedError("flow_permutation %r: only 'invconv' works in the reference too "
                                      "(Permute2d is broken, modules.py:98-118)" % glow["flow_permutation"])
        self.use_frame_nb = bool(cond.get("use_frame_nb"))
        self.start = max(cond[m]["history"] for m in ENC_ORDER)
        self.encoders = []
        col = 0
        for m in ENC_ORDER:
            cfg = cond[m]
            hist = int(cfg["history"])
            if m != "p1_face" and not hist:
                continue
            in_dim = int(cfg["dim"]) if m.endswith("face") else self.S
            e = EncoderSpec(m, cfg["enc"], in_dim, hist, int(cfg["hidden_dim"] or 0), float(cfg["dropout"] or 0))
            e.col = col
            col += e.dim
            self.encoders.append(e)
        if self.use_frame_nb:
            e = EncoderSpec("frame_nb", "frame_nb", 1, 1, 0, 0.0)
            e.col = col
            col += 1
            self.encoders.append(e)
        self.E = col
        self.Ch = self.C // 2
        self.C2 = self.C - self.Ch
        self.Cout = 2 * self.C2 if self.affine else self.C2
        self.G = (4 if self.rnn_type == "lstm" else 3) * self.H
        self.I = self.Ch + self.D
        p1 = self.encoders[0]
        self.p1_cols = p1.dim
        fcol, self.fold_a, self.fold_b, self.unfold = 0, [], [], []
        for e in self.encoders:
            while fcol % 4:
                self.fold_a.append(-1)
                self.fold_b.append(-1)
                fcol += 1
            e.fcol = fcol
            e.fdim = e.hid if e.enc in ("rnn", "lstm") else e.dim
            for j in range(e.fdim):
                self.fold_a.append(e.col + j)
                self.fold_b.append(e.col + e.hid + j if e.enc in ("rnn", "lstm") else -1)
            self.unfold += [fcol + (j % e.fdim) for j in range(e.dim)]
            fcol += e.fdim
        self.Ef = fcol
        self.ldf = (fcol + 31) // 32 * 32

    @classmethod
    def flow_only(cls, C, H, D, Ks, E, affine, rnn_type, lu, scale_eps, actnorm_scale):
        s = object.__new__(cls)
        s.C, s.S, s.D, s.H, s.Ks, s.E = int(C), 0, int(D), int(H), int(Ks), int(E)
        s.affine, s.rnn_type, s.lu = int(bool(affine)), rnn_type or "gru", bool(lu)
        s.scale_eps, s.actnorm_scale = float(scale_eps), float(actnorm_scale)
        s.use_frame_nb, s.start, s.encoders, s.p1_cols = False, 0, [], 0
        s.Ch = s.C // 2
        s.C2 = s.C - s.Ch
        s.Cout = 2 * s.C2 if s.affine else s.C2
        s.G = (4 if s.rnn_type == "lstm" else 3) * s.H
        s.I = s.Ch + s.D
        s.fold_a, s.fold_b, s.unfold = list(range(s.E)), [-1] * s.E, list(range(s.E))
        s.Ef = s.E
        s.ldf = (s.E + 31) // 32 * 32
        return s

    def flow_shapes(self):
        Ks, C, H, D, E, G, I, Cout = self.Ks, self.C, self.H, self.D, self.E, self.G, self.I, self.Cout
        shapes = {
            "an_bias": (Ks, C), "an_logs": (Ks, C),
            "w_ih": (Ks, G, I), "w_hh": (Ks, G, H), "b_ih": (Ks, G), "b_hh": (Ks, G),
            "wct": (Ks, D, E), "bct": (Ks, D),
            "w_fl": (Ks, Cout, H), "b_fl": (Ks, Cout), "l_fl": (Ks, Cout),
        }
        if self.lu:
            shapes.update({"inv_l": (Ks, C, C), "inv_u": (Ks, C, C), "inv_logs": (Ks, C)})
        else:
            shapes["inv_w"] = (Ks, C, C)
        return shapes


class _Ctx:
    pass


class GlowEngine:

    @translate_oom
    def __init__(self, spec, device):
        self.spec = spec
        self.device = torch.device(device)
        if self.device.type != "cuda":
            raise _lib.LfiError("GlowEngine needs a GPU device (got %s); there is no CPU path" % device)
        self.L = _lib.lib()
        self.layout = {}
        off = 0
        for e in spec.encoders:
            if e.enc in ("rnn", "lstm"):
                g = e.ng * e.hid
                for leaf, shape in zip(ENC_LEAVES, ((g, e.in_dim), (g, e.hid), (g,), (g,))):
                    self.layout["enc.%s.%s" % (e.name, leaf)] = (off, shape)
                    off += math.prod(shape)
            elif e.enc == "mlp":
                for leaf, shape in (("mlp_weight", (e.hid, e.in_dim * e.hist)), ("mlp_bias", (e.hid,))):
                    off = (off + 3) // 4 * 4
                    self.layout["enc.%s.%s" % (e.name, leaf)] = (off, shape)
                    off += math.prod(shape)
        shapes = spec.flow_shapes()
        for name in FLOW_FIELDS:
            if name in shapes:
                self.layout["flow." + name] = (off, shapes[name])
                off += math.prod(shapes[name])
        self.n_params = off
        self.flow_offset = min(o for n, (o, _) in self.layout.items() if n.startswith("flow."))
        f32 = dict(dtype=torch.float32, device=self.device)
        self.params = torch.zeros(off, **f32)
        self.grads = torch.zeros(off, **f32)
        self.adam_m = None
        self.adam_v = None
        self.step_count = 0
        self.param_version = 0
        self.inv_p = torch.zeros(spec.Ks, spec.C, spec.C, **f32)
        self.inv_sign = torch.zeros(spec.Ks, spec.C, **f32)
        self.sumsq = torch.zeros(1, dtype=torch.float64, device=self.device)
        self.sumsq_work = torch.zeros(1024, dtype=torch.float64, device=self.device)
        i32 = dict(dtype=torch.int32, device=self.device)
        self.fold_a = torch.tensor(spec.fold_a, **i32)
        self.fold_b = torch.tensor(spec.fold_b, **i32)
        self.unfold = torch.tensor(spec.unfold, **i32)
        self.wct_f = torch.zeros(spec.Ks * spec.D, spec.ldf, **f32)
        self._side_stream = None
        self._partial_streams = {}
        self._sample_stream = None
        self._partial_refused = False
        self._ws = {}
        self._sample_graphs = {}
        self._sample_seen = {}
        self.prep = None
        self._last = None
        self.timers = None
        self._timer_tags = None
        self.precision = 0
        self.sample_frame_precision = {"bf16x3": 1, "f32": 0, "bf16x6": 5, "fp16x3": 9}.get(os.environ.get("LFI_SAMPLE_FRAME_PRECISION", ""))
        self._mask_calls = 0
        self._enc_stash_f16 = {}
        self._sample_fp16_unsafe = False
        self.backward_products = self.check_backward_products(os.environ.get("LFI_BWD_PRODUCTS", "auto"))
        self._bwd_skip = 0
        self.tile_pin = {k.strip(): int(v) for k, v in (it.split("=") for it in os.environ.get("LFI_TILE_PIN", "").split(",") if it)}
        self.pass_skip = {}
        env = os.environ.get("LFI_PASS_SKIP", "")
        if env.strip() == "none":
            self.pass_skip = {}
        for item in filter(None, [] if env.strip() == "none" else env.split(",")):
            name, bits = item.split("=")
            self.pass_skip[name.strip()] = int(bits)

    def bump_param_version(self):
        self.param_version += 1

    def _skip_bits(self, cls):
        if cls in self.pass_skip:
            return self.pass_skip[cls] & 3
        return self._bwd_skip if cls in BWD_CLASSES else 0

    @staticmethod
    def check_backward_products(value):
        if isinstance(value, str) and value.strip().lower() == "auto":
            return "auto"
        try:
            n = int(value)
        except (TypeError, ValueError):
            n = None
        if n not in (2, 3) or (not isinstance(value, str) and n != value):
            raise ValueError("backward products must be 2, 3 or 'auto', got %r" % (value,))
        return n

    def _want_stash_f16(self, frames):
        env = os.environ.get("LFI_ENC_STASH_F16")
        if env in ("0", "1"):
            return env == "1" and bool(self.precision & 1)
        return self.backward_product_count(frames) == 2

    def backward_product_count(self, frames):
        bp = self.check_backward_products(self.backward_products)
        if not (self.precision & 1):
            return 3
        return (2 if frames >= 8192 else 3) if bp == "auto" else int(bp)

    def enable_timing(self, on=True, only=None):
        self.timers = {} if on else None
        self._timer_tags = None if only is None else set(only)

    def _tic(self, tag):
        if self.timers is None or tag is None or (self._timer_tags is not None and tag not in self._timer_tags):
            return None
        ev = (torch.cuda.Event(enable_timing=True), torch.cuda.Event(enable_timing=True))
        ev[0].record()
        return ev

    def _toc(self, tag, ev):
        if ev is not None:
            ev[1].record()
            self.timers.setdefault(tag, []).append(ev)

    def timing_summary(self):
        torch.cuda.synchronize()
        return {t: (len(evs), sum(a.elapsed_time(b) for a, b in evs) / len(evs)) for t, evs in (self.timers or {}).items()}

    def view(self, name, buf=None):
        off, shape = self.layout[name]
        buf = self.params if buf is None else buf
        return buf[off:off + math.prod(shape)].view(shape)

    def fview(self, name, buf=None):
        return self.view("flow." + name, buf)

    def _flow_dims(self, B, N):
        s = self.spec
        return FlowDims(B, N, s.C, s.H, s.D, s.Ks, s.affine, 1 if s.rnn_type == "lstm" else 0, s.scale_eps, self.precision)

    def _flow_params(self):
        s = self.spec
        p = FlowParams()
        for name in ("an_bias", "an_logs", "w_ih", "w_hh", "b_ih", "b_hh", "w_fl", "b_fl", "l_fl"):
            setattr(p, name, self.fview(name).data_ptr())
        if s.lu:
            p.inv_l, p.inv_u, p.inv_logs = (self.fview(n).data_ptr() for n in ("inv_l", "inv_u", "inv_logs"))
            p.inv_p, p.inv_sign = self.inv_p.data_ptr(), self.inv_sign.data_ptr()
        else:
            p.inv_w = self.fview("inv_w").data_ptr()
        return p

    def _flow_grads(self):
        s = self.spec
        g = FlowGrads()
        for name in ("an_bias", "an_logs", "w_ih", "w_hh", "b_ih", "b_hh", "w_fl", "b_fl", "l_fl"):
            setattr(g, name, self.fview(name, self.grads).data_ptr())
        if s.lu:
            g.inv_l, g.inv_u, g.inv_logs = (self.fview(n, self.grads).data_ptr() for n in ("inv_l", "inv_u", "inv_logs"))
        else:
            g.inv_w = self.fview("inv_w", self.grads).data_ptr()
        return g

    def _buf(self, name, floats, zero=False):
        t = self._ws.get(name)
        if t is None or t.numel() < floats:
            t = torch.zeros(max(int(floats), 1), dtype=torch.float32, device=self.device)
            self._ws[name] = t
            self._order_birth()
        elif zero:
            t.zero_()
        return t

    def _order_birth(self):
        if os.environ.get("LFI_NO_BIRTH_ORDER") == "1":
            return
        if torch.cuda.is_current_stream_capturing():
            return
        cur = torch.cuda.current_stream(self.device)
        for st in [self._side_stream] + list((self.__dict__.get("_partial_streams") or {}).values()):
            if st is not None and st != cur:
                st.wait_stream(cur)

    def draw_masks(self, B, N, seed, key_dev=None):
        segs = [e for e in self.spec.encoders if e.dropout > 0]
        if not segs:
            return None
        if key_dev is None:
            self._mask_calls += 1
        total = sum(N * B * e.hist for e in segs)
        flat = self._buf("dropout_masks", total)
        outs, ns, keeps, masks, off = (C.c_void_p * 4)(), (C.c_long * 4)(), (C.c_float * 4)(), {}, 0
        for i, e in enumerate(segs):
            n = N * B * e.hist
            view = flat[off:off + n].view(N, B, e.hist)
            outs[i], ns[i], keeps[i] = view.data_ptr(), n, 1.0 - e.dropout
            masks[e.name] = view
            off += n
        if key_dev is not None:
            check(self.L.lfi_dropout_masks_dev(len(segs), outs, ns, keeps, key_dev.data_ptr(), _stream()), "lfi_dropout_masks_dev")
        else:
            check(self.L.lfi_dropout_masks(len(segs), outs, ns, keeps, int(seed) & (2 ** 64 - 1), self._mask_calls, _stream()),
                  "lfi_dropout_masks")
        return masks

    def has_dropout(self):
        return any(e.dropout > 0 for e in self.spec.encoders)

    def _fork(self):
        if os.environ.get("LFI_NO_OVERLAP") == "1":
            return None
        if self._side_stream is None:
            self._side_stream = torch.cuda.Stream(device=self.device)
        self._side_stream.wait_stream(torch.cuda.current_stream(self.device))
        return self._side_stream

    def close(self):
        streams, self._partial_streams = self.__dict__.get("_partial_streams") or {}, {}
        for st in streams.values():
            st.synchronize()
            self.L.lfi_stream_destroy(C.c_void_p(st.cuda_stream))

    def __del__(self):
        try:
            self.close()
        except Exception:
            pass

    def _fork_partial(self, cus_per_xcd):
        st = self._partial_streams.get(cus_per_xcd)
        if st is None:
            ptr = C.c_void_p()
            if self.L.lfi_stream_create_partial(int(cus_per_xcd), C.byref(ptr)) != 0:
                if not self._partial_refused:
                    warnings.warn("lets_face_it_amd: no partial-chip stream (%s); the sampler's static part runs on an ordinary "
                                  "second stream" % self.L.lfi_last_error().decode(), RuntimeWarning)
                self._partial_refused = True
                return self._fork()
            st = self._partial_streams[cus_per_xcd] = torch.cuda.ExternalStream(ptr.value, device=self.device)
            if len(self._partial_streams) == 1:
                ref = weakref.ref(self)
                atexit.register(lambda: ref() is not None and ref().close())
        st.wait_stream(torch.cuda.current_stream(self.device))
        return st

    @staticmethod
    def _on(side):
        return torch.cuda.stream(side) if side is not None else contextlib.nullcontext()

    def _join(self):
        if self._side_stream is not None:
            torch.cuda.current_stream(self.device).wait_stream(self._side_stream)

    def gemm(self, M, N, K, A, lda, akc, Bm, ldb, bkc, Cm, ldc, bias=None, act=0, slope=0.01, G=None, ldg=0,
             batch=1, sA=0, sB=0, sC=0, sBias=0, sG=0, accumulate=0, splitk=1, a_off=0, b_off=0, c_off=0, bias_off=0,
             tag=None, ws="scratch.gemm_splitk", cls=None, colsum_into=None, a_bf16=False):
        g = GemmDesc()
        g.M, g.N, g.K = M, N, K
        g.A, g.lda, g.a_kcontig = A.data_ptr() + (2 if a_bf16 else 4) * a_off, lda, akc
        g.a_bf16 = 1 if a_bf16 else 0
        g.B, g.ldb, g.b_kcontig = Bm.data_ptr() + 4 * b_off, ldb, bkc
        g.C, g.ldc = Cm.data_ptr() + 4 * c_off, ldc
        g.bias = None if bias is None else bias.data_ptr() + 4 * bias_off
        g.G, g.ldg = ptr(G), ldg
        g.batch, g.strideA, g.strideB, g.strideC, g.strideBias, g.strideG = batch, sA, sB, sC, sBias, sG
        g.accumulate, g.act, g.slope = accumulate, act, slope
        g.splitk = splitk
        g.precision = self.precision | (self._skip_bits(cls) << 8 if (self.precision & 1) else 0)
        if self.tile_pin and (self.precision & 1):
            g.precision |= {128: 0x20, 256: 0x10}.get(self.tile_pin.get(cls), 0)
        if splitk > 1 or splitk == 0:
            g.work = self._buf(ws, batch * max(splitk, 8) * M * N).data_ptr()
        part, prow = None, 0
        if colsum_into is not None and os.environ.get("LFI_NO_COLPART") != "1":
            prow = int(self.L.lfi_gemm_colpart_rows(C.byref(g)))
            if prow > 0:
                part = self._buf("scratch.colpart", prow * ldc)
                g.colsum_part, g.ld_part = part.data_ptr(), ldc
        ev = self._tic(tag)
        check(self.L.lfi_gemm_f32(C.byref(g), _stream()), "lfi_gemm_f32")
        self._toc(tag, ev)
        if part is not None:
            self.colsum(part, ldc, 0, prow, colsum_into.numel(), 1, colsum_into, 0, ws="scratch.colsum.part")
        return part is not None

    def planes(self, name, X, ldx, rows, cols, x_off=0):
        elems = self.L.lfi_planes_elems(rows, cols) + 256 * ((cols + 15) // 16 * 16) * 2
        buf = self._ws.get(name)
        if buf is None or buf.numel() < elems:
            buf = torch.empty(elems, dtype=torch.bfloat16, device=self.device)
            self._ws[name] = buf
        check(self.L.lfi_planes_from_f32(X.data_ptr() + 4 * x_off, ldx, rows, cols, buf.data_ptr(), _stream()),
              "lfi_planes_from_f32")
        return buf, (cols + 15) // 16

    def plane_buf(self, name, elems):
        buf = self._ws.get(name)
        if buf is None or buf.numel() < elems:
            buf = torch.empty(int(elems), dtype=torch.bfloat16, device=self.device)
            self._ws[name] = buf
        return buf

    def gemm_planes(self, M, N, K, Ap, a_nkt, Bp, b_nkt, Cm, ldc, bias=None, act=0, slope=0.01, G=None, ldg=0, batch=1,
                    a_stride=0, b_stride=0, sC=0, sBias=0, sG=0, accumulate=0, c_off=0, bias_off=0, tag=None, cls=None,
                    a_fmt=0, b_fmt=0, a_off=0, b_off=0, splitk=1, ws="scratch.pgemm_splitk", store=True,
                    Cr=None, cr_nkt=0, cr_col0=0, Gr=None, gr_nkt=0, gr_col0=0, colsum_into=None, hi_only=False, tile=0):
        g = PGemmDesc()
        g.skip = self._skip_bits(cls)
        g.M, g.N, g.K = M, N, K
        g.Ap, g.a_nkt, g.a_stride = Ap.data_ptr() + 2 * a_off, a_nkt, a_stride
        g.Bp, g.b_nkt, g.b_stride = Bp.data_ptr() + 2 * b_off, b_nkt, b_stride
        g.C, g.ldc = (None if Cm is None else Cm.data_ptr() + 4 * c_off), ldc
        g.bias = None if bias is None else bias.data_ptr() + 4 * bias_off
        g.G, g.ldg = ptr(G), ldg
        g.batch, g.strideC, g.strideBias, g.strideG = batch, sC, sBias, sG
        g.accumulate, g.act, g.slope = accumulate, act, slope
        g.a_fmt, g.b_fmt = a_fmt, b_fmt
        g.splitk = splitk
        g.store_f32 = 1 if store else 0
        if splitk > 1:
            g.work = self._buf(ws, batch * splitk * M * N).data_ptr()
        g.Cr, g.cr_nkt, g.cr_col0 = ptr(Cr), cr_nkt, cr_col0
        g.Gr, g.gr_nkt, g.gr_col0 = ptr(Gr), gr_nkt, gr_col0
        g.out_hi_only, g.tile = (1 if hi_only else 0), tile
        part, prow = None, 0
        if colsum_into is not None and os.environ.get("LFI_NO_COLPART") != "1":
            prow = int(self.L.lfi_gemm_planes_colpart_rows(C.byref(g)))
            if prow > 0:
                part = self._buf("scratch.colpart", prow * ldc)
                g.colsum_part, g.ld_part = part.data_ptr(), ldc
        ev = self._tic(tag)
        check(self.L.lfi_gemm_planes(C.byref(g), _stream()), "lfi_gemm_planes")
        self._toc(tag, ev)
        if part is not None:
            self.colsum(part, ldc, 0, prow, colsum_into.numel(), 1, colsum_into, 0, ws="scratch.colsum.part")
        return part is not None

    @staticmethod
    def _fill_splitk(M, N, K, batch=1):
        tiles = ((M + 127) // 128) * ((N + 127) // 128) * batch
        return max(1, min(16, 768 // max(tiles, 1), K // 1024))

    @staticmethod
    def _long_k_splitk(M, N, K, kmin=1024):
        t256 = ((M + 255) // 256) * ((N + 255) // 256)
        t128 = ((M + 127) // 128) * ((N + 127) // 128)
        wide = 1.12 * M * N / (t256 * 65536.0) >= M * N / (t128 * 16384.0)
        sk = 256 // t256 if wide else 512 // t128
        return max(1, min(sk, K // kmin))

    @staticmethod
    def _tail_splitk(M, N, K, batch=1, slots=512):
        tiles = ((M + 127) // 128) * ((N + 127) // 128) * batch
        best, best_eff = 1, 0.0
        for sk in (1, 2, 3, 4, 6, 8):
            if K // sk < 512:
                break
            wg = tiles * sk
            eff = wg / (math.ceil(wg / slots) * slots)
            if eff > best_eff + 0.02:
                best, best_eff = sk, eff
            if eff > 0.85:
                break
        return best

    def colsum(self, X, ldx, strideX, rows, cols, batch, out, strideOut, scale=1.0, accumulate=0, x_off=0, ws="scratch.colsum"):
        w = self._buf(ws, self.L.lfi_colsum_work_floats(rows, cols, batch))
        check(self.L.lfi_colsum_f32(X.data_ptr() + 4 * x_off, ldx, strideX, rows, cols, batch, out.data_ptr(), strideOut,
                                    scale, accumulate, w.data_ptr(), _stream()), "lfi_colsum_f32")

    def _chain_fwd_ok(self):
        s = self.spec
        return (self.precision == 1 and os.environ.get("LFI_PGEMM", "1") != "0" and os.environ.get("LFI_PCHAIN", "1") != "0"
                and s.D % 32 == 0 and s.G % 32 == 0)

    def _chain_ok(self, dims, with_stash):
        if not self._chain_fwd_ok():
            return False
        if not with_stash:
            return True
        F = dims.B * dims.N
        return F % 32 == 0 and bool(self.L.lfi_flow_bwd_emits_planes(C.byref(dims)))

    @staticmethod
    def _planes_splitk(M, N, K, batch=1, kmin=1024, slots=512):
        tiles = ((M + 127) // 128) * ((N + 255) // 256) * batch
        best, best_score = 1, -1.0
        for sk in range(1, 9):
            if sk > 1 and K // sk < kmin:
                break
            wg = tiles * sk
            score = wg / (math.ceil(wg / slots) * slots) * (1.0 - 0.03 * (sk - 1))
            if score > best_score + 1e-9:
                best, best_score = sk, score
        return best

    def run_prep(self, with_inverse=False):
        d = self._flow_dims(1, 1)
        need = self.L.lfi_flow_prep_floats(C.byref(d))
        if self.prep is None or self.prep.numel() < need:
            self.prep = torch.zeros(need, dtype=torch.float32, device=self.device)
        p = self._flow_params()
        s = self.spec
        prep_first = os.environ.get("LFI_PREP_FOLD_FIRST", "1") == "0"
        if prep_first:
            check(self.L.lfi_flow_prep(C.byref(d), C.byref(p), self.prep.data_ptr(), 1 if with_inverse else 0, _stream()),
                  "lfi_flow_prep")
        check(self.L.lfi_cols_fold(self.fview("wct").data_ptr(), s.E, s.Ks * s.D, self.fold_a.data_ptr(),
                                   self.fold_b.data_ptr(), s.Ef, self.wct_f.data_ptr(), s.ldf, _stream()), "lfi_cols_fold")
        if self.precision == 1:
            self._wct_planes = self.planes("wct_planes", self.wct_f, s.ldf, s.Ks * s.D, s.ldf)
        if not prep_first:
            check(self.L.lfi_flow_prep(C.byref(d), C.byref(p), self.prep.data_ptr(), 1 if with_inverse else 0, _stream()),
                  "lfi_flow_prep")
        if self.precision == 1:
            if self._chain_fwd_ok():
                self._wc_r = self.planes("wc_r", self.prep, s.D, s.Ks * s.G, s.D, x_off=self._wc_offset())

    def _check_input(self, x, name, B, Tmin, dim):
        if not (x.is_cuda and x.dtype == torch.float32 and x.is_contiguous() and x.dim() == 3 and x.shape[0] == B
                and x.shape[1] >= Tmin and x.shape[2] == dim):
            raise ValueError("%s: expected contiguous float32 GPU tensor (B=%d, T>=%d, %d), got %s %s on %s"
                             % (name, B, Tmin, dim, tuple(x.shape), x.dtype, x.device))

    def build_features(self, data, faces, B, T, masks, cond, with_stash, skip_p1=False, sampling=False, windows=False, frame0=0,
                       side=None):
        s = self.spec
        N = 1 if windows else T - s.start
        F = N * B
        small = None
        if side is not None and os.environ.get("LFI_ENC_FWD_SMALL_ON_SIDE", "1") != "0":
            rec = sorted((e for e in s.encoders if e.enc in ("rnn", "lstm") and not (e.name == "p1_face" and skip_p1)),
                         key=lambda e: e.hist * e.hid * e.hid)
            small = rec[0] if len(rec) >= 3 else None
        gather_side = side is not None and os.environ.get("LFI_ENC_GATHER_ON_SIDE", "1") != "0"
        for e in s.encoders:
            with (self._on(side) if (e is small or (gather_side and e.enc == "none")) else contextlib.nullcontext()):
                self._build_feature(e, data, faces, B, T, N, F, masks, cond, with_stash, skip_p1, sampling, windows, frame0)

    def _build_feature(self, e, data, faces, B, T, N, F, masks, cond, with_stash, skip_p1, sampling, windows, frame0):
        s = self.spec
        st = _stream()
        p1 = e.name == "p1_face"
        if p1 and skip_p1:
            return
        if e.enc == "frame_nb":
            base = None
            if not sampling:
                base = data.get("frame_nb")
                if base is None:
                    raise KeyError("Conditioning.use_frame_nb is set but the batch has no 'frame_nb' entry")
                if not (base.is_cuda and base.dtype == torch.float32 and base.numel() == B):
                    raise ValueError("frame_nb: expected a float32 GPU tensor of shape (B, 1), got %s %s on %s"
                                     % (tuple(base.shape), base.dtype, base.device))
                base = base.contiguous()
            check(self.L.lfi_fill_frame_nb(ptr(base), 2.0 * frame0 if sampling else (0.0 if windows else 2.0 * s.start), B, N,
                                           cond.data_ptr(), s.ldf, e.fcol, st), "lfi_fill_frame_nb")
            return
        x = faces if p1 else data.get(e.name)
        if x is None:
            raise KeyError("batch is missing modality %r" % e.name)
        self._check_input(x, e.name, B, e.hist if windows else T, e.in_dim)
        Tx = x.shape[1]
        incl = 0 if p1 else 1
        start = (e.hist - incl) if windows else s.start
        if windows and Tx != e.hist:
            raise ValueError("%s: a conditioning window has %d frames, got %d" % (e.name, e.hist, Tx))
        mk = None if masks is None else masks.get(e.name)
        if mk is not None and not (tuple(mk.shape) == (N, B, e.hist) and mk.is_contiguous()
                                   and mk.dtype == torch.float32 and mk.is_cuda):
            raise ValueError("mask for %s must be a contiguous float32 GPU tensor (N, B, hist)" % e.name)
        if e.enc == "none":
            check(self.L.lfi_gather_windows(x.data_ptr(), B, Tx, e.in_dim, N, start, e.hist, incl, ptr(mk),
                                            cond.data_ptr(), s.ldf, e.fcol, st), "lfi_gather_windows")
            return
        hid = e.hid
        if e.enc == "mlp":
            win = self._buf("enc_win." + e.name, F * e.win, zero=False)
            check(self.L.lfi_gather_windows(x.data_ptr(), B, Tx, e.in_dim, N, start, e.hist, incl, ptr(mk),
                                            win.data_ptr(), e.win, 0, st), "lfi_gather_windows")
            self.gemm(F, hid, e.in_dim * e.hist, win, e.win, 1, self.view("enc.%s.mlp_weight" % e.name),
                      e.in_dim * e.hist, 1, cond, s.ldf, bias=self.view("enc.%s.mlp_bias" % e.name), act=1, slope=0.01,
                      c_off=e.fcol)
            return
        lstm = e.enc == "lstm"
        G = e.ng * hid
        xp = self._buf("xp." + e.name, B * Tx * G)
        xa, wa, ldi = self._aligned_input(e, x, B * Tx, G)
        self.gemm(B * Tx, G, e.in_dim, xa, ldi, 1, wa, ldi, 1, xp, G, cls="enc_xproj")
        d = EncDesc(B, Tx, N, start - 1 + incl, e.hist, hid, s.ldf, e.fcol, self.precision, 0, 1 if lstm else 0)
        s16 = bool(with_stash and not lstm and self._want_stash_f16(F) and self.L.lfi_encode_windows_stash_f16_ok(C.byref(d)))
        d.stash_f16 = 1 if s16 else 0
        self._enc_stash_f16[e.name] = s16
        gates = self._buf("enc_gates." + e.name, e.hist * F * (5 if lstm else (2 if s16 else 4)) * hid) if (with_stash or lstm) else None
        hseq = self._buf("enc_hseq." + e.name, e.hist * F * hid)
        work = self._buf("scratch.enc_fwd." + e.name, self.L.lfi_encode_windows_work_floats(C.byref(d)))
        ev = self._tic("enc_fwd." + e.name)
        check(self.L.lfi_encode_windows_fwd(
            C.byref(d), xp.data_ptr(), self.view("enc.%s.weight_hh" % e.name).data_ptr(),
            self.view("enc.%s.bias_ih" % e.name).data_ptr(), self.view("enc.%s.bias_hh" % e.name).data_ptr(),
            ptr(mk), cond.data_ptr(), ptr(gates), hseq.data_ptr(), work.data_ptr(), st), "lfi_encode_windows_fwd")
        self._toc("enc_fwd." + e.name, ev)

    def _aligned_input(self, e, x, rows, G):
        if e.in_dim % 4 == 0 or os.environ.get("LFI_NO_XPAD") == "1":
            return x, self.view("enc.%s.weight_ih" % e.name), e.in_dim
        ldi = (e.in_dim + 3) // 4 * 4
        xa = self._buf("xpad." + e.name, rows * ldi)
        check(self.L.lfi_pad_rows(x.data_ptr(), rows, e.in_dim, e.in_dim, xa.data_ptr(), ldi, _stream()), "lfi_pad_rows")
        wa = self._buf("wihpad." + e.name, G * ldi)
        check(self.L.lfi_pad_rows(self.view("enc.%s.weight_ih" % e.name).data_ptr(), G, e.in_dim, e.in_dim, wa.data_ptr(), ldi,
                                  _stream()), "lfi_pad_rows")
        return xa, wa, ldi

    def _project(self, cond, F, chain=False, with_stash=False):
        s = self.spec
        KD = s.Ks * s.D
        if chain:
            cp, nkc = self.planes("cond_planes", cond, s.ldf, F, s.ldf)
            wp, nkw = self._wct_planes
            nkKD = KD // 16
            c_r = self.plane_buf("c_r", self.L.lfi_planes_elems(F, KD) + 256 * KD * 2)
            self.gemm_planes(F, KD, s.ldf, cp, nkc, wp, nkw, None, KD, bias=self.fview("bct"), act=1, slope=0.01, store=False,
                             Cr=c_r, cr_nkt=nkKD, tag="gemm_cond_fwd", cls="cond_fwd")
            gic = self._buf("gic", s.Ks * F * s.G)
            wr, nkwr = self._wc_r
            self.gemm_planes(F, s.G, s.D, c_r, nkKD, wr, nkwr, gic, s.G, bias=self.fview("b_ih"), batch=s.Ks,
                             a_stride=(s.D // 16) * 1024, b_stride=(s.G // 32) * nkwr * 1024, sC=F * s.G, sBias=s.G,
                             tag="gemm_gic", cls="gic")
            self._cond_planes = (cp, nkc)
            return c_r, gic
        cbuf = self._buf("c", F * KD)
        if self.precision == 1 and os.environ.get("LFI_PGEMM", "1") != "0":
            cp, nkc = self.planes("cond_planes", cond, s.ldf, F, s.ldf)
            wp, nkw = self._wct_planes
            self.gemm_planes(F, KD, s.ldf, cp, nkc, wp, nkw, cbuf, KD, bias=self.fview("bct"), act=1, slope=0.01,
                             tag="gemm_cond_fwd", cls="cond_fwd")
        else:
            self.gemm(F, KD, s.Ef, cond, s.ldf, 1, self.wct_f, s.ldf, 1, cbuf, KD, bias=self.fview("bct"), act=1, slope=0.01,
                      tag="gemm_cond_fwd", cls="cond_fwd")
        gic = self._buf("gic", s.Ks * F * s.G)
        self.gemm(F, s.G, s.D, cbuf, KD, 1, self.prep, s.D, 1, gic, s.G, bias=self.fview("b_ih"),
                  batch=s.Ks, sA=s.D, sB=s.G * s.D, sC=F * s.G, sBias=s.G, b_off=self._wc_offset(), cls="gic")
        return cbuf, gic

    @translate_oom
    def forward(self, batch, masks=None, with_stash=True, init_actnorm=None):
        s = self.spec
        x = batch["p1_face"]
        B, T = x.shape[0], x.shape[1]
        N = T - s.start
        if N <= 0:
            raise ValueError("sequence length %d does not exceed the longest history %d" % (T, s.start))
        F = N * B
        side = self._fork()
        with self._on(side):
            self.run_prep()
        cond = self._buf("cond", F * s.ldf)
        self.build_features(batch, x, B, T, masks, cond, with_stash, side=side)
        self._join()
        dims = self._flow_dims(B, N)
        chain = self._chain_ok(dims, with_stash)
        cbuf, gic = self._project(cond, F, chain, with_stash)
        if init_actnorm is not None:
            self._actnorm_init_walk(x, B, T, F, gic, dims, init_actnorm)
        stash = self._buf("flow_stash", self.L.lfi_flow_stash_floats(C.byref(dims)))
        z = torch.empty(N, B, s.C, dtype=torch.float32, device=self.device)
        nll = torch.empty(N, B, dtype=torch.float32, device=self.device)
        p = self._flow_params()
        check(self.L.lfi_flow_seq_fwd(C.byref(dims), C.byref(p), self.prep.data_ptr(), x.data_ptr(), T, s.start,
                                      gic.data_ptr(), stash.data_ptr(), z.data_ptr(), nll.data_ptr(), _stream()),
              "lfi_flow_seq_fwd")
        ctx = _Ctx()
        ctx.batch, ctx.masks, ctx.B, ctx.T, ctx.N, ctx.F = batch, masks, B, T, N, F
        ctx.cond, ctx.cbuf, ctx.gic, ctx.stash, ctx.dims, ctx.with_stash, ctx.chain = cond, cbuf, gic, stash, dims, with_stash, chain
        ctx.enc_stash_f16 = dict(self._enc_stash_f16)
        self._last = ctx
        return z, nll

    def _actnorm_init_walk(self, x, B, T, F, gic, dims, allreduce):
        s = self.spec
        st = _stream()
        xa = self._buf("init_xa", B * s.C)
        xb = self._buf("init_xb", B * s.C)
        hd = self._buf("init_h", B * s.H)
        cd = self._buf("init_c", B * s.H)
        xa[:B * s.C].view(B, s.C).copy_(x[:, s.start, :])
        sums = torch.zeros(2 * s.C, dtype=torch.float64, device=self.device)
        p = self._flow_params()
        for k in range(s.Ks):
            check(self.L.lfi_actnorm_init_stats(xa.data_ptr(), B, s.C, sums.data_ptr(), st), "lfi_actnorm_init_stats")
            world = allreduce(sums)
            check(self.L.lfi_actnorm_init_apply(sums.data_ptr(), float(B * world), s.C, s.actnorm_scale,
                                                self.fview("an_bias")[k].data_ptr(), self.fview("an_logs")[k].data_ptr(),
                                                st), "lfi_actnorm_init_apply")
            check(self.L.lfi_flow_step(C.byref(dims), C.byref(p), self.prep.data_ptr(), k, B, xa.data_ptr(), s.C, None, None,
                                       gic.data_ptr() + 4 * k * F * s.G, xb.data_ptr(), s.C, hd.data_ptr(), cd.data_ptr(),
                                       None, 0, st), "lfi_flow_step")
            xa, xb = xb, xa
        self.bump_param_version()
        self.run_prep()

    @translate_oom
    def backward(self, gscale, after_flow=None):
        ctx = self._last
        if ctx is None or not ctx.with_stash:
            raise _lib.LfiError("backward() needs a preceding forward(with_stash=True)")
        s = self.spec
        B, T, N, F = ctx.B, ctx.T, ctx.N, ctx.F
        KD = s.Ks * s.D
        st = _stream()
        dims, p = ctx.dims, self._flow_params()
        self._bwd_skip = 1 if self.backward_product_count(F) == 2 else 0
        bst = self._buf("flow_bstash", self.L.lfi_flow_bstash_floats(C.byref(dims)))
        if ctx.chain:
            return self._backward_chain(ctx, gscale, after_flow, bst)
        check(self.L.lfi_flow_seq_bwd(C.byref(dims), C.byref(p), self.prep.data_ptr(), ctx.stash.data_ptr(), gscale,
                                      bst.data_ptr(), st), "lfi_flow_seq_bwd")
        work = self._buf("scratch.pg", self.L.lfi_flow_param_grads_work_floats(C.byref(dims)))
        g = self._flow_grads()
        side = self._fork()
        pg_dims = dims
        if self._skip_bits("flow_pgrads") and (self.precision & 1):
            pg_dims = self._flow_dims(B, N)
            pg_dims.gemm_precision = self.precision | (self._skip_bits("flow_pgrads") << 8)
        check(self.L.lfi_flow_param_grads(C.byref(pg_dims), C.byref(p), self.prep.data_ptr(), ctx.stash.data_ptr(),
                                          bst.data_ptr(), ctx.cbuf.data_ptr(), KD, gscale, C.byref(g), 0, work.data_ptr(),
                                          st, side.cuda_stream if side is not None else None), "lfi_flow_param_grads")
        dgi_off = (self.L.lfi_flow_bstash_ptr(C.byref(dims), bst.data_ptr(), 1) - bst.data_ptr()) // 4
        bct_done = self.gemm(F, s.D, s.G, bst, s.G, 1, self.prep, s.D, 0, ctx.cbuf, KD, act=2, slope=0.01, G=ctx.cbuf, ldg=KD,
                             batch=s.Ks, sA=F * s.G, sB=s.G * s.D, sC=s.D, sG=s.D, a_off=dgi_off, b_off=self._wc_offset(),
                             cls="dpre", colsum_into=self.fview("bct", self.grads))
        dpre = ctx.cbuf
        dwf = self._buf("dwct_f", KD * s.ldf)
        self.gemm(KD, s.ldf, F, dpre, KD, 0, ctx.cond, s.ldf, 0, dwf, s.ldf, tag="gemm_cond_wgrad", splitk=0, cls="cond_wgrad")
        check(self.L.lfi_cols_fold(dwf.data_ptr(), s.ldf, KD, self.unfold.data_ptr(), None, s.E,
                                   self.fview("wct", self.grads).data_ptr(), s.E, st), "lfi_cols_fold")
        if not bct_done:
            self.colsum(dpre, KD, 0, F, KD, 1, self.fview("bct", self.grads), 0)
        self._join()
        if after_flow is not None:
            after_flow()
        rnn = [e for e in s.encoders if e.enc in ("rnn", "lstm", "mlp")]
        if rnn:
            col0 = min(e.fcol for e in rnn)
            W = s.Ef - col0
            ldd = (W + 3) // 4 * 4
            dcond = self._buf("dcond", F * ldd)
            self.gemm(F, W, KD, dpre, KD, 1, self.wct_f, s.ldf, 0, dcond, ldd, b_off=col0, tag="gemm_cond_dgrad",
                      splitk=0, cls="cond_dgrad")
            self._encoders_backward(rnn, ctx, dcond, ldd, col0)

    def _backward_chain(self, ctx, gscale, after_flow, bst):
        s = self.spec
        B, T, N, F = ctx.B, ctx.T, ctx.N, ctx.F
        KD, G, D, Ks = s.Ks * s.D, s.G, s.D, s.Ks
        st = _stream()
        dims, p = ctx.dims, self._flow_params()
        c_r = ctx.cbuf
        nkKD, nkG, nkD = KD // 16, G // 16, D // 16
        dgi_p = self.plane_buf("dgi_planes", self.L.lfi_planes_elems(Ks * F, G) + 256 * G * 2)
        dgi_hi = all(self._skip_bits(c) & 1 for c in ("dpre", "flow_pgrads"))
        dpre_hi = all(self._skip_bits(c) & 1 for c in ("cond_wgrad", "cond_dgrad"))
        pg_skip = self._skip_bits("flow_pgrads")
        g16 = bool((pg_skip & 1) and not (pg_skip & 2) and (self.precision & 1) and os.environ.get("LFI_FLOW_G16", "1") != "0")
        bdims = dims
        if g16:
            bdims = self._flow_dims(B, N)
            bdims.gemm_precision = dims.gemm_precision | (1 << 16)
        check(self.L.lfi_flow_seq_bwd_planes(C.byref(bdims), C.byref(p), self.prep.data_ptr(), ctx.stash.data_ptr(), gscale,
                                             bst.data_ptr(), dgi_p.data_ptr(), 1 if dgi_hi else 0, st), "lfi_flow_seq_bwd_planes")
        work = self._buf("scratch.pg", self.L.lfi_flow_param_grads_work_floats(C.byref(dims)))
        g = self._flow_grads()
        side = self._fork()
        self.gemm_planes(G, D, F, dgi_p, nkG, c_r, nkKD, self.fview("w_ih", self.grads), s.I, batch=Ks, a_fmt=1, b_fmt=1,
                         a_stride=(F // 32) * nkG * 1024, b_stride=nkD * 1024, sC=G * s.I, c_off=s.Ch,
                         splitk=self._planes_splitk(G, D, F, Ks), tag="gemm_dwc", cls="flow_pgrads")
        pg_dims = dims
        if self._skip_bits("flow_pgrads") and (self.precision & 1):
            pg_dims = self._flow_dims(B, N)
            pg_dims.gemm_precision = self.precision | (self._skip_bits("flow_pgrads") << 8) | ((1 << 16) if g16 else 0)
        check(self.L.lfi_flow_param_grads(C.byref(pg_dims), C.byref(p), self.prep.data_ptr(), ctx.stash.data_ptr(),
                                          bst.data_ptr(), None, KD, gscale, C.byref(g), 0, work.data_ptr(),
                                          st, side.cuda_stream if side is not None else None), "lfi_flow_param_grads")
        wr, nkwr = self._wc_r
        bct_done = self.gemm_planes(F, D, G, dgi_p, nkG, wr, nkwr, None, KD, act=2, slope=0.01, batch=Ks, b_fmt=1,
                                    a_stride=(F // 32) * nkG * 1024, b_stride=(G // 32) * nkwr * 1024, sC=D, store=False,
                                    Gr=c_r, gr_nkt=nkKD, Cr=c_r, cr_nkt=nkKD, hi_only=dpre_hi,
                                    colsum_into=self.fview("bct", self.grads), tag="gemm_dpre", cls="dpre")
        if not bct_done:
            raise _lib.LfiError("the dpre product on planes did not take the column-sum epilogue")
        dpre_p = c_r
        self._join()
        cp, nkc = self._cond_planes
        dwf = self._buf("dwct_f", KD * s.ldf)
        self.gemm_planes(KD, s.ldf, F, dpre_p, nkKD, cp, nkc, dwf, s.ldf, a_fmt=1, b_fmt=1,
                         splitk=self._planes_splitk(KD, s.ldf, F), tag="gemm_cond_wgrad", cls="cond_wgrad")
        check(self.L.lfi_cols_fold(dwf.data_ptr(), s.ldf, KD, self.unfold.data_ptr(), None, s.E,
                                   self.fview("wct", self.grads).data_ptr(), s.E, st), "lfi_cols_fold")
        if after_flow is not None:
            after_flow()
        rnn = [e for e in s.encoders if e.enc in ("rnn", "lstm", "mlp")]
        if rnn:
            col0 = min(e.fcol for e in rnn) // 32 * 32
            W = s.Ef - col0
            ldd = (W + 3) // 4 * 4
            dcond = self._buf("dcond", F * ldd)
            wp, nkw = self._wct_planes
            self.gemm_planes(F, W, KD, dpre_p, nkKD, wp, nkw, dcond, ldd, b_fmt=1, b_off=(col0 // 16) * 1024,
                             splitk=self._planes_splitk(F, W, KD), tag="gemm_cond_dgrad", cls="cond_dgrad")
            self._encoders_backward(rnn, ctx, dcond, ldd, col0)

    def _encoders_backward(self, rnn, ctx, dcond, ldd, col0):
        order = self._bptt_order(rnn)
        recurrent = [e for e in order if e.enc != "mlp"]
        small = None
        if (len(recurrent) >= 3 and os.environ.get("LFI_ENC_BWD_SMALL_ON_SIDE", "1") != "0"
                and os.environ.get("LFI_ENC_BWD_OVERLAP", "1") != "0"):
            side = self._fork()
            if side is not None:
                small = recurrent[-1]
                with self._on(side):
                    self._encoder_backward(small, ctx, dcond, ldd, small.fcol - col0, inline=True)
        for e in order:
            if e is small:
                continue
            if e.enc == "mlp":
                self._mlp_backward(e, ctx, dcond, ldd, e.fcol - col0)
            else:
                self._encoder_backward(e, ctx, dcond, ldd, e.fcol - col0)
        self._join()

    @staticmethod
    def _bptt_order(encoders):
        if os.environ.get("LFI_ENC_BWD_ORDER", "1") == "0":
            return list(encoders)
        return sorted(encoders, key=lambda e: -(e.hist * e.hid * e.hid))

    def _mlp_backward(self, e, ctx, dcond, lddcond, col):
        s = self.spec
        F = ctx.F
        K = e.in_dim * e.hist
        check(self.L.lfi_leaky_grad(dcond.data_ptr() + 4 * col, lddcond, ctx.cond.data_ptr() + 4 * e.fcol, s.ldf, F, e.hid,
                                    0.01, _stream()), "lfi_leaky_grad")
        win = self._ws["enc_win." + e.name]
        gname = "enc.%s." % e.name
        self.gemm(e.hid, K, F, dcond, lddcond, 0, win, e.win, 0, self.view(gname + "mlp_weight", self.grads), K,
                  splitk=max(1, min(32, F // 1024)), a_off=col)
        self.colsum(dcond, lddcond, 0, F, e.hid, 1, self.view(gname + "mlp_bias", self.grads), 0, x_off=col)

    def _encoder_backward(self, e, ctx, dcond, lddcond, col, inline=False):
        s = self.spec
        B, N, F = ctx.B, ctx.N, ctx.F
        x = ctx.batch[e.name]
        Tx, hid, G3 = x.shape[1], e.hid, e.ng * e.hid
        st = _stream()
        d = EncDesc(B, Tx, N, s.start - (1 if e.name == "p1_face" else 0), e.hist, hid, lddcond, col, self.precision, 0,
                    1 if e.enc == "lstm" else 0,
                    1 if ((self._skip_bits("enc_bptt") & 1) and (self._skip_bits("enc_dwhh") & 3) == 1) else 0,
                    1 if ctx.enc_stash_f16.get(e.name) else 0)
        gates = self._ws["enc_gates." + e.name]
        hseq = self._ws["enc_hseq." + e.name]
        compact = bool(self.L.lfi_encode_windows_compact_dgi(C.byref(d)))
        dgi = self._buf("enc_dgi." + e.name, e.hist * F * (hid if compact else G3))
        dgh = self._buf("enc_dgh." + e.name, e.hist * F * G3)
        work = self._buf("scratch.enc_bwd." + e.name, self.L.lfi_encode_windows_work_floats(C.byref(d)))
        whh = self.view("enc.%s.weight_hh" % e.name)
        prow = self.L.lfi_encode_windows_bias_rows(C.byref(d))
        part = self._buf("enc_bias_part." + e.name, prow * 4 * hid) if prow else None
        check(self.L.lfi_encode_windows_bwd(C.byref(d), dcond.data_ptr(), lddcond, whh.data_ptr(), gates.data_ptr(),
                                            hseq.data_ptr(), dgi.data_ptr(), dgh.data_ptr(), ptr(part), work.data_ptr(), st),
              "lfi_encode_windows_bwd")
        mk = None if ctx.masks is None else ctx.masks.get(e.name)
        dxp = self._buf("dxp." + e.name, B * Tx * G3)
        gname = "enc.%s." % e.name
        rows = B * Tx
        xa, ldi = self._ws.get("xpad." + e.name), (e.in_dim + 3) // 4 * 4
        if e.in_dim % 4 == 0 or xa is None or os.environ.get("LFI_NO_XPAD") == "1":
            xa, ldi = x, e.in_dim
        side = self._fork() if (os.environ.get("LFI_ENC_BWD_OVERLAP", "1") != "0" and not inline) else None
        with self._on(side):
            check(self.L.lfi_encode_windows_scatter(C.byref(d), dgi.data_ptr(), dgh.data_ptr(), ptr(mk), dxp.data_ptr(),
                                                    _stream()), "lfi_encode_windows_scatter")
            self.gemm(G3, e.in_dim, rows, dxp, G3, 0, xa, ldi, 0, self.view(gname + "weight_ih", self.grads), e.in_dim,
                      splitk=self._long_k_splitk(G3, e.in_dim, rows, kmin=512),
                      ws="scratch.gemm_splitk.side3" if inline else "scratch.gemm_splitk.side", cls="enc_dwih")
        gbi, gbh = self.view(gname + "bias_ih", self.grads), self.view(gname + "bias_hh", self.grads)
        if part is not None:
            check(self.L.lfi_encode_windows_bias_grads(part.data_ptr(), prow, hid, gbi.data_ptr(), gbh.data_ptr(), st),
                  "lfi_encode_windows_bias_grads")
        else:
            self.colsum(dgi, G3, 0, e.hist * F, G3, 1, gbi, 0)
        if e.hist > 1:
            kk = (e.hist - 1) * F
            g16 = bool(self.L.lfi_encode_windows_grad_stash_bf16(C.byref(d)))
            self.gemm(G3, hid, kk, dgh, G3, 0, hseq, hid, 0, self.view(gname + "weight_hh", self.grads), hid,
                      splitk=self._long_k_splitk(G3, hid, kk), a_off=F * G3, cls="enc_dwhh", a_bf16=g16,
                      ws="scratch.gemm_splitk.side2" if inline else "scratch.gemm_splitk")
        else:
            self.view(gname + "weight_hh", self.grads).zero_()
        if part is None:
            self.colsum(dgh, G3, 0, e.hist * F, G3, 1, gbh, 0)

    @translate_oom
    def encode_condition(self, condition, masks=None):
        s = self.spec
        data = {("p1_face" if k == "prev_p1_face" else k): v for k, v in condition.items()}
        faces = data["p1_face"]
        B = faces.shape[0]
        cond = self._buf("step_cond", B * s.ldf, zero=True)
        self.build_features(data, faces, B, 0, masks, cond, with_stash=False, windows=True)
        return cond[:B * s.ldf].view(B, s.ldf).index_select(1, self.unfold.long())

    @translate_oom
    def flow_net(self, x, cond, h_prev, c_prev, reverse, init_actnorm=None):
        s = self.spec
        B = x.shape[0]
        for t, name, w in ((x, "input", s.C), (cond, "condition", s.E)):
            if not (t.is_cuda and t.dtype == torch.float32 and t.dim() == 2 and t.shape == (B, w)):
                raise ValueError("%s: expected a float32 GPU tensor of shape (%d, %d), got %s %s on %s"
                                 % (name, B, w, tuple(t.shape), t.dtype, t.device))
        x, cond = x.contiguous(), cond.contiguous()
        st = _stream()
        self.run_prep(with_inverse=bool(reverse))
        KD = s.Ks * s.D
        cb = self._buf("step_c", B * KD)
        self.gemm(B, KD, s.E, cond, s.E, 1, self.fview("wct"), s.E, 1, cb, KD, bias=self.fview("bct"), act=1, slope=0.01)
        gic = self._buf("step_gic", s.Ks * B * s.G)
        self.gemm(B, s.G, s.D, cb, KD, 1, self.prep, s.D, 1, gic, s.G, bias=self.fview("b_ih"),
                  batch=s.Ks, sA=s.D, sB=s.G * s.D, sC=B * s.G, sBias=s.G, b_off=self._wc_offset())
        dims = self._flow_dims(B, 1)
        p = self._flow_params()
        lstm = s.rnn_type == "lstm"
        f32 = dict(dtype=torch.float32, device=self.device)
        h_new = torch.empty(s.Ks, B, s.H, **f32)
        c_new = torch.empty(s.Ks, B, s.H, **f32) if lstm else None
        ld = torch.zeros(B, **f32)
        bufs = (torch.empty(B, s.C, **f32), torch.empty(B, s.C, **f32))
        sums = torch.zeros(2 * s.C, dtype=torch.float64, device=self.device) if init_actnorm is not None else None
        src = x
        order = range(s.Ks - 1, -1, -1) if reverse else range(s.Ks)
        for i, k in enumerate(order):
            if sums is not None:
                sums.zero_()
                check(self.L.lfi_actnorm_init_stats(src.data_ptr(), B, s.C, sums.data_ptr(), st), "lfi_actnorm_init_stats")
                world = init_actnorm(sums)
                check(self.L.lfi_actnorm_init_apply(sums.data_ptr(), float(B * world), s.C, s.actnorm_scale,
                                                    self.fview("an_bias")[k].data_ptr(), self.fview("an_logs")[k].data_ptr(),
                                                    st), "lfi_actnorm_init_apply")
            hp = None if h_prev is None else h_prev[k]
            cp = None if (c_prev is None or not lstm) else c_prev[k]
            for t in (hp, cp):
                if t is not None and not (t.is_cuda and t.dtype == torch.float32 and t.shape == (B, s.H) and t.is_contiguous()):
                    raise ValueError("recurrent state of flow step %d: expected a contiguous float32 GPU (%d, %d) tensor" % (k, B, s.H))
            dst = bufs[i & 1]
            check(self.L.lfi_flow_step(C.byref(dims), C.byref(p), self.prep.data_ptr(), k, B, src.data_ptr(), s.C, ptr(hp),
                                       ptr(cp), gic.data_ptr() + 4 * k * B * s.G, dst.data_ptr(), s.C, h_new[k].data_ptr(),
                                       ptr(None if c_new is None else c_new[k]), ld.data_ptr(), 1 if reverse else 0, st),
                  "lfi_flow_step")
            src = dst
        if sums is not None:
            self.bump_param_version()
            self.run_prep(with_inverse=bool(reverse))
        const = self.prep[self._ldconst_offset()]
        return src, (ld - const if reverse else ld + const), h_new, c_new

    @staticmethod
    def adam_step_floats(lr, beta1, beta2, step_count):
        import numpy as np
        b1, b2, lr64 = float(np.float32(beta1)), float(np.float32(beta2)), float(np.float32(lr))
        bc1, bc2 = 1.0 - b1 ** int(step_count), 1.0 - b2 ** int(step_count)
        return float(np.float32(lr64 / bc1)), float(np.float32(1.0 / math.sqrt(bc2)))

    def _claim_optimizer(self, name):
        have = self.__dict__.get("_opt_name")
        if have is not None and have != name:
            raise ValueError("the engine holds optimiser state of %r (checkpoint or earlier steps); stepping it with %r would "
                             "reinterpret its buffers - start from fresh state (load_optimizer_state({})) or keep Optim.name" % (have, name))
        self._opt_name = name

    @translate_oom
    def optimizer_step(self, lr, beta1, beta2, eps, clip=0.0, gmul=1.0, hyper_dev=None, weight_decay=0.0, amsgrad=False):
        self._claim_optimizer("adam")
        self.bump_param_version()
        if self.adam_m is None:
            self.adam_m = torch.zeros_like(self.params)
            self.adam_v = torch.zeros_like(self.params)
        if amsgrad and self.__dict__.get("opt_aux") is None:
            self.opt_aux = torch.zeros_like(self.params)
        st = _stream()
        if clip and clip > 0:
            check(self.L.lfi_grad_sumsq(self.grads.data_ptr(), self.n_params, self.sumsq.data_ptr(),
                                        self.sumsq_work.data_ptr(), st), "lfi_grad_sumsq")
        if weight_decay or amsgrad:
            if hyper_dev is None:
                self.step_count += 1
            check(self.L.lfi_adam_clip_step_ex(self.params.data_ptr(), self.grads.data_ptr(), self.adam_m.data_ptr(),
                                               self.adam_v.data_ptr(), ptr(self.opt_aux if amsgrad else None), self.n_params,
                                               self.sumsq.data_ptr(), float(clip or 0.0), gmul, lr, beta1, beta2, eps,
                                               float(weight_decay), self.step_count, hyper_dev, st), "lfi_adam_clip_step_ex")
            return
        if hyper_dev is not None:
            check(self.L.lfi_adam_clip_step_dev(self.params.data_ptr(), self.grads.data_ptr(), self.adam_m.data_ptr(),
                                                self.adam_v.data_ptr(), self.n_params, self.sumsq.data_ptr(),
                                                float(clip or 0.0), gmul, beta1, beta2, eps, hyper_dev, st), "lfi_adam_clip_step_dev")
            return
        self.step_count += 1
        check(self.L.lfi_adam_clip_step(self.params.data_ptr(), self.grads.data_ptr(), self.adam_m.data_ptr(),
                                        self.adam_v.data_ptr(), self.n_params, self.sumsq.data_ptr(),
                                        float(clip or 0.0), gmul, lr, beta1, beta2, eps, self.step_count, st),
              "lfi_adam_clip_step")

    @translate_oom
    def optimizer_step_sgd(self, lr, momentum=0.0, dampening=0.0, weight_decay=0.0, nesterov=False, clip=0.0, gmul=1.0):
        self._claim_optimizer("sgd")
        self.bump_param_version()
        first = momentum and (self.adam_m is None or not self.__dict__.get("_momentum_inited", False))
        if momentum and self.adam_m is None:
            self.adam_m = torch.zeros_like(self.params)
        st = _stream()
        if clip and clip > 0:
            check(self.L.lfi_grad_sumsq(self.grads.data_ptr(), self.n_params, self.sumsq.data_ptr(),
                                        self.sumsq_work.data_ptr(), st), "lfi_grad_sumsq")
        self.step_count += 1
        check(self.L.lfi_sgd_clip_step(self.params.data_ptr(), self.grads.data_ptr(), ptr(self.adam_m if momentum else None),
                                       self.n_params, self.sumsq.data_ptr(), float(clip or 0.0), gmul, lr, float(momentum),
                                       float(dampening), float(weight_decay), 1 if nesterov else 0, 1 if first else 2, st),
              "lfi_sgd_clip_step")
        if momentum:
            self._momentum_inited = True

    @translate_oom
    def optimizer_step_rmsprop(self, lr, alpha=0.99, eps=1e-8, weight_decay=0.0, momentum=0.0, centered=False, clip=0.0, gmul=1.0):
        self._claim_optimizer("rmsprop")
        self.bump_param_version()
        if self.adam_v is None:
            self.adam_v = torch.zeros_like(self.params)
        if momentum and self.adam_m is None:
            self.adam_m = torch.zeros_like(self.params)
        if centered and self.__dict__.get("opt_aux") is None:
            self.opt_aux = torch.zeros_like(self.params)
        st = _stream()
        if clip and clip > 0:
            check(self.L.lfi_grad_sumsq(self.grads.data_ptr(), self.n_params, self.sumsq.data_ptr(),
                                        self.sumsq_work.data_ptr(), st), "lfi_grad_sumsq")
        self.step_count += 1
        check(self.L.lfi_rmsprop_clip_step(self.params.data_ptr(), self.grads.data_ptr(), self.adam_v.data_ptr(),
                                           ptr(self.adam_m if momentum else None), ptr(self.opt_aux if centered else None),
                                           self.n_params, self.sumsq.data_ptr(), float(clip or 0.0), gmul, lr, float(alpha), float(eps),
                                           float(weight_decay), float(momentum), st), "lfi_rmsprop_clip_step")

    def optimizer_state(self):
        aux = self.__dict__.get("opt_aux")
        return {"step_count": int(self.step_count),
                "optimizer": self.__dict__.get("_opt_name"),
                "momentum_inited": bool(self.__dict__.get("_momentum_inited", False)),
                "opt_aux": None if aux is None else aux.detach().clone(),
                "mask_calls": int(self._mask_calls),
                "adam_m": None if self.adam_m is None else self.adam_m.detach().clone(),
                "adam_v": None if self.adam_v is None else self.adam_v.detach().clone()}

    def load_optimizer_state(self, state):
        self.step_count = int(state.get("step_count", 0))
        self._mask_calls = int(state.get("mask_calls", self._mask_calls))
        self._opt_name = state.get("optimizer")
        self._momentum_inited = bool(state.get("momentum_inited", state.get("adam_m") is not None))
        for name in ("adam_m", "adam_v", "opt_aux"):
            t = state.get(name)
            if t is None:
                setattr(self, name, None)
                continue
            if t.numel() != self.n_params:
                raise ValueError("optimizer state holds %d floats, the model has %d parameters" % (t.numel(), self.n_params))
            setattr(self, name, t.to(device=self.device, dtype=torch.float32).reshape(-1).clone())

    def grad_norm(self):
        check(self.L.lfi_grad_sumsq(self.grads.data_ptr(), self.n_params, self.sumsq.data_ptr(),
                                    self.sumsq_work.data_ptr(), _stream()), "lfi_grad_sumsq")
        return float(self.sumsq.sqrt().item())

    @translate_oom
    def sample(self, seq_len, data, noise, masks=None, return_nll=False):
        check_return_nll(return_nll)
        caller = torch.cuda.current_stream(self.device)
        with self._off_legacy_stream(self, "_sample_stream", force=self._sample_static_cus(seq_len - self.spec.start) > 0) as st:
            out = self._sample(seq_len, data, noise, masks, return_nll)
        if st != caller:
            for t in (out if return_nll else (out,)):
                t.record_stream(caller)
        return out

    @contextlib.contextmanager
    def _off_legacy_stream(self, owner, attr, force=False):
        caller = torch.cuda.current_stream(self.device)
        if not force and caller != torch.cuda.default_stream(self.device):
            yield caller
            return
        own = getattr(owner, attr)
        if own is None:
            own = torch.cuda.Stream(device=self.device)
            setattr(owner, attr, own)
        own.wait_stream(caller)
        with torch.cuda.stream(own):
            yield own
        caller.wait_stream(own)

    def _sample(self, seq_len, data, noise, masks=None, return_nll=False):
        s = self.spec
        seed = data["p1_face"]
        B = seed.shape[0]
        nframes = seq_len - s.start
        if nframes <= 0:
            raise ValueError("seq_len %d does not exceed the longest history %d" % (seq_len, s.start))
        self._check_input(seed, "p1_face", B, s.start, s.C)
# ... 308 lines not shown
```

Baseline: 2.199 million.

## Pass packed ReLU sign bits from cond forward GEMM to dpre backward epilogue

The forward conditioning GEMM epilogue now packs the sign of each activation output into 64-bit sign words. The backward dpre GEMM reads these words for its leaky-ReLU mask instead of reloading bf16 hi-plane values of the stored activation. A persistent-tile variant (TRP 5) is also added: each workgroup loops over tiles and prefetches the next tile's operands before running the epilogue. This cuts mask traffic in the backward epilogue and launch/tail overhead, at the cost of a small sign buffer and extra epilogue bit-packing work.

```diff
diff --git a/include/lfi.h b/include/lfi.h
--- a/include/lfi.h
+++ b/include/lfi.h
@@ -52,9 +52,13 @@
   float* colsum_part; long ld_part;
   int out_hi_only;
   int tile;
+  void* sign_out; const void* sign_in;
 } lfi_pgemm_desc;
 long lfi_gemm_planes_work_floats(const lfi_pgemm_desc* d);
 long lfi_gemm_planes_colpart_rows(const lfi_pgemm_desc* d);
+long lfi_planes_sign_words(long rows, long cols);
+int lfi_gemm_planes_signs_ok(const lfi_pgemm_desc* d);
+long lfi_gemm_planes_persist_grid(const lfi_pgemm_desc* d);
 int lfi_gemm_planes(const lfi_pgemm_desc* d, void* stream);
 
 long lfi_colsum_work_floats(int rows, int cols, int batch);
diff --git a/lets_face_it_amd/_lib.py b/lets_face_it_amd/_lib.py
--- a/lets_face_it_amd/_lib.py
+++ b/lets_face_it_amd/_lib.py
@@ -42,6 +42,7 @@
         ("Gr", C.c_void_p), ("gr_nkt", C.c_int), ("gr_col0", C.c_long),
         ("colsum_part", C.c_void_p), ("ld_part", C.c_long),
         ("out_hi_only", C.c_int), ("tile", C.c_int),
+        ("sign_out", C.c_void_p), ("sign_in", C.c_void_p),
     ]
 
 
@@ -109,6 +110,9 @@
         "lfi_encode_windows_fwd_variant": (i, [P(EncDesc), i, i]),
         "lfi_gemm_planes_work_floats": (l, [P(PGemmDesc)]),
         "lfi_gemm_planes_colpart_rows": (l, [P(PGemmDesc)]),
+        "lfi_planes_sign_words": (l, [l, l]),
+        "lfi_gemm_planes_signs_ok": (i, [P(PGemmDesc)]),
+        "lfi_gemm_planes_persist_grid": (l, [P(PGemmDesc)]),
         "lfi_colsum_work_floats": (l, [i, i, i]),
         "lfi_colsum_f32": (i, [vp, l, l, i, i, i, vp, l, f, i, vp, vp]),
         "lfi_cols_fold": (i, [vp, l, l, vp, vp, i, vp, l, vp]),
@@ -190,7 +194,7 @@
 
 EXPORTS = [
     "lfi_last_error", "lfi_version", "lfi_gemm_work_floats", "lfi_gemm_f32", "lfi_gemm_colpart_rows", "lfi_planes_elems", "lfi_planes_from_f32",
-    "lfi_gemm_planes", "lfi_gemm_planes_work_floats", "lfi_gemm_planes_colpart_rows",
+    "lfi_gemm_planes", "lfi_gemm_planes_work_floats", "lfi_gemm_planes_colpart_rows", "lfi_planes_sign_words", "lfi_gemm_planes_signs_ok", "lfi_gemm_planes_persist_grid",
     "lfi_flow_bwd_emits_planes", "lfi_flow_seq_bwd_planes", "lfi_encode_windows_grad_stash_bf16", "lfi_encode_windows_stash_f16_ok", "lfi_encode_windows_fwd_variant", "lfi_colsum_work_floats",
     "lfi_colsum_f32", "lfi_cols_fold", "lfi_encode_windows_work_floats", "lfi_encode_windows_fwd", "lfi_encode_windows_bwd",
     "lfi_encode_windows_bias_rows", "lfi_encode_windows_bias_grads",
diff --git a/lets_face_it_amd/csrc/lfi_gemm_common.h b/lets_face_it_amd/csrc/lfi_gemm_common.h
--- a/lets_face_it_amd/csrc/lfi_gemm_common.h
+++ b/lets_face_it_amd/csrc/lfi_gemm_common.h
@@ -41,6 +41,8 @@
   __bf16* Cr; int nktCr; long colCr;
   const __bf16* Gr; int nktGr; long colGr;
   int hiOnly;
+  unsigned long long* So; const unsigned long long* Si; int npcS;
+  int pbatch;
 };
 
 __device__ __forceinline__ float apply_act(float v, int act, float slope, const float* G, long gidx) {
@@ -291,9 +293,26 @@
 
 typedef unsigned gu32x4 __attribute__((ext_vector_type(4)));
 typedef unsigned gu32x2 __attribute__((ext_vector_type(2)));
-template <int MODE>
-__device__ __forceinline__ void gemm_epilogue_direct16(const GemmArgs& g, const f32x4 (&acc)[4][4], int m0, int n0, int wm, int wn, int lane,
-                                                       int batch, int split) {
+typedef const __attribute__((address_space(4))) GemmArgs GemmArgsK;
+template <typename GA>
+__device__ __forceinline__ long gemm_sign_patch_offset(const GA& g, int r0, int c0, int batch) {
+  const long gcol0 = g.colCr + (long)batch * g.strideC + c0;
+  return ((long)(r0 >> 6) * g.npcS + (gcol0 >> 6)) * 512;
+}
+template <typename GA>
+__device__ __forceinline__ gu32x2 gemm_sign_word_load(const GA& g, int m0, int n0, int wm, int wn, int lane, int batch) {
+  const int r0 = m0 + wm * 64, c0 = n0 + wn * 64;
+  gu32x2 sw = {0u, 0u};
+  if (g.Si && r0 < g.M && c0 < g.N) {
+    const __amdgpu_buffer_rsrc_t rs = __builtin_amdgcn_make_buffer_rsrc(
+        const_cast<char*>(reinterpret_cast<const char*>(g.Si)) + gemm_sign_patch_offset(g, r0, c0, batch), 0, 0x7fffffff, 0x00020000);
+    sw = __builtin_amdgcn_raw_buffer_load_b64(rs, (unsigned)lane * 8u, 0, 0);
+  }
+  return sw;
+}
+template <int MODE, typename GA = GemmArgs, bool SIGNW = true>
+__device__ __forceinline__ void gemm_epilogue_direct16(const GA& g, const f32x4 (&acc)[4][4], int m0, int n0, int wm, int wn, int lane,
+                                                       int batch, int split, gu32x2 sw = (gu32x2){0u, 0u}) {
   const int l15 = lane & 15, g4 = lane >> 4;
   const int r0 = m0 + wm * 64, c0 = n0 + wn * 64;
   const float* bias = g.bias ? g.bias + batch * g.strideBias : nullptr;
@@ -308,6 +327,8 @@
   f32x4 csum[4];
 #pragma unroll
   for (int j = 0; j < 4; ++j) csum[j] = (f32x4){0.f, 0.f, 0.f, 0.f};
+  const bool wsign = SIGNW && MODE == 3 && g.So != nullptr, rsign = MODE == 4 && g.Si != nullptr;
+  unsigned sb[2] = {0u, 0u};
   {
     const long gcol0 = g.colCr + (long)batch * g.strideC + c0;
 #pragma unroll
@@ -329,12 +350,18 @@
         const int col = c0 + 16 * j + 4 * g4;
         f32x4 v = acc[i][j] + bv[j];
         if constexpr (MODE == 4) {
-          gu32x2 m2 = {0u, 0u};
-          if (blk && c0 + 16 * j < g.N) m2 = __builtin_amdgcn_raw_buffer_load_b64(rg, voff, 2048 * j, 0);
-          const float o0 = __builtin_bit_cast(float, m2[0] << 16), o1 = __builtin_bit_cast(float, m2[0] & 0xffff0000u);
-          const float o2 = __builtin_bit_cast(float, m2[1] << 16), o3 = __builtin_bit_cast(float, m2[1] & 0xffff0000u);
-          v[0] = o0 > 0.0f ? v[0] : v[0] * g.slope; v[1] = o1 > 0.0f ? v[1] : v[1] * g.slope;
-          v[2] = o2 > 0.0f ? v[2] : v[2] * g.slope; v[3] = o3 > 0.0f ? v[3] : v[3] * g.slope;
+          bool p0, p1, p2, p3;
+          if (rsign) {
+            const unsigned m4 = sw[i >> 1] >> (16 * (i & 1) + 4 * j);
+            p0 = (m4 & 1u) != 0; p1 = (m4 & 2u) != 0; p2 = (m4 & 4u) != 0; p3 = (m4 & 8u) != 0;
+          } else {
+            gu32x2 m2 = {0u, 0u};
+            if (blk && c0 + 16 * j < g.N) m2 = __builtin_amdgcn_raw_buffer_load_b64(rg, voff, 2048 * j, 0);
+            p0 = __builtin_bit_cast(float, m2[0] << 16) > 0.0f; p1 = __builtin_bit_cast(float, m2[0] & 0xffff0000u) > 0.0f;
+            p2 = __builtin_bit_cast(float, m2[1] << 16) > 0.0f; p3 = __builtin_bit_cast(float, m2[1] & 0xffff0000u) > 0.0f;
+          }
+          v[0] = p0 ? v[0] : v[0] * g.slope; v[1] = p1 ? v[1] : v[1] * g.slope;
+          v[2] = p2 ? v[2] : v[2] * g.slope; v[3] = p3 ? v[3] : v[3] * g.slope;
         } else if (g.act == 1) {
 #pragma unroll
           for (int r = 0; r < 4; ++r) v[r] = v[r] > 0.0f ? v[r] : v[r] * g.slope;
@@ -344,6 +371,11 @@
         uint2 h, l;
         split2(v[0], v[1], &h.x, &l.x);
         split2(v[2], v[3], &h.y, &l.y);
+        if (wsign) {
+          const unsigned m4 = (__builtin_bit_cast(float, h.x << 16) > 0.0f ? 1u : 0u) | (__builtin_bit_cast(float, h.x & 0xffff0000u) > 0.0f ? 2u : 0u) |
+                              (__builtin_bit_cast(float, h.y << 16) > 0.0f ? 4u : 0u) | (__builtin_bit_cast(float, h.y & 0xffff0000u) > 0.0f ? 8u : 0u);
+          sb[i >> 1] |= m4 << (16 * (i & 1) + 4 * j);
+        }
         if (blk && c0 + 16 * j < g.N) {
           __builtin_amdgcn_raw_buffer_store_b64((gu32x2){h.x, h.y}, rs, voff, 2048 * j, 2);
           if (!g.hiOnly) __builtin_amdgcn_raw_buffer_store_b64((gu32x2){l.x, l.y}, rs, voff, 2048 * j + 1024, 2);
@@ -351,6 +383,11 @@
       }
     }
   }
+  if (wsign && r0 < g.M && c0 < g.N) {
+    const __amdgpu_buffer_rsrc_t rw = __builtin_amdgcn_make_buffer_rsrc(reinterpret_cast<char*>(g.So) + gemm_sign_patch_offset(g, r0, c0, batch), 0,
+                                                                       0x7fffffff, 0x00020000);
+    __builtin_amdgcn_raw_buffer_store_b64((gu32x2){sb[0], sb[1]}, rw, (unsigned)lane * 8u, 0, 2);
+  }
   if constexpr (MODE == 4) {
     if (g.colpart) {
 #pragma unroll
@@ -369,10 +406,9 @@
   }
 }
 
-__device__ __forceinline__ void gemm_tile_of_block(const GemmArgs& g, int* tm, int* tn, int* batch, int* split) {
+template <typename GA>
+__device__ __forceinline__ void gemm_tile_of_linear(const GA& g, long lin, long total, int nbatch, int* tm, int* tn, int* batch, int* split) {
   const int ntile = g.tiles_m * g.tiles_n;
-  const long total = (long)gridDim.x * gridDim.y * gridDim.z;
-  long lin = blockIdx.x + (long)gridDim.x * (blockIdx.y + (long)gridDim.y * blockIdx.z);
   {
     const long q = total >> 3, idx = lin >> 3;
     const int r = (int)(total & 7), xcd = (int)(lin & 7);
@@ -380,14 +416,19 @@
   }
   int bid = (int)(lin % ntile);
   const long rest = lin / ntile;
-  *batch = (int)(rest % gridDim.y);
-  *split = (int)(rest / gridDim.y);
+  *batch = (int)(rest % nbatch);
+  *split = (int)(rest / nbatch);
   const int GM = g.gm > 0 ? g.gm : 8;
   const int per_group = GM * g.tiles_n;
   const int grp = bid / per_group, in_grp = bid - grp * per_group;
   const int rows_here = min(GM, g.tiles_m - grp * GM);
   *tm = grp * GM + in_grp % rows_here;
   *tn = in_grp / rows_here;
+}
+__device__ __forceinline__ void gemm_tile_of_block(const GemmArgs& g, int* tm, int* tn, int* batch, int* split) {
+  const long total = (long)gridDim.x * gridDim.y * gridDim.z;
+  const long lin = blockIdx.x + (long)gridDim.x * (blockIdx.y + (long)gridDim.y * blockIdx.z);
+  gemm_tile_of_linear(g, lin, total, (int)gridDim.y, tm, tn, batch, split);
 }
 
 #ifndef LFI_EPI_ROWS
diff --git a/lets_face_it_amd/csrc/lfi_pgemm.hip b/lets_face_it_amd/csrc/lfi_pgemm.hip
--- a/lets_face_it_amd/csrc/lfi_pgemm.hip
+++ b/lets_face_it_amd/csrc/lfi_pgemm.hip
@@ -296,7 +296,7 @@
   if constexpr (TRP != 0) {
     int lanez = lane, m0z = m0, n0z = n0;
     asm volatile("" : "+v"(lanez), "+s"(m0z), "+s"(n0z));
-    gemm_epilogue_direct16<TRP>(g, acc, m0z, n0z, wm, wn, lanez, batch, split);
+    gemm_epilogue_direct16<TRP, GemmArgs, WMT == 2>(g, acc, m0z, n0z, wm, wn, lanez, batch, split);
   } else {
     __syncthreads();
     gemm_epilogue_wide<64 * WNT, 512, 2, COLP, true, true>(g, acc, reinterpret_cast<float*>(xsmem), WNT == 4 ? 64 : 128, m0, n0, wm, wn,
@@ -310,9 +310,16 @@
   static_assert(WMT * WNT == 8 && NA + 4 * WNT == 24, "eight waves, 24 blocks per slot");
   const int tid = threadIdx.x;
   const int lane = tid & 63, wave = __builtin_amdgcn_readfirstlane(tid >> 6);
+  constexpr bool PERS = TRP == 5;
+  constexpr int EMODE = TRP == 5 ? 4 : TRP;
+  const long total = PERS ? (long)g.tiles_m * g.tiles_n * g.pbatch : (long)gridDim.x * gridDim.y * gridDim.z;
+  const long lstep = PERS ? (long)gridDim.x : total;
+  const int nbat = PERS ? g.pbatch : (int)gridDim.y;
+  long lin = blockIdx.x + (long)gridDim.x * (blockIdx.y + (long)gridDim.y * blockIdx.z);
   int tm, tn, batch, split;
-  gemm_tile_of_block(g, &tm, &tn, &batch, &split);
-  const int m0 = tm * 64 * WMT, n0 = tn * 64 * WNT;
+  if constexpr (PERS) gemm_tile_of_linear(g, lin, total, nbat, &tm, &tn, &batch, &split);
+  else gemm_tile_of_block(g, &tm, &tn, &batch, &split);
+  int m0 = tm * 64 * WMT, n0 = tn * 64 * WNT;
   const int ktc = g.kchunk >> 4;
   const int kt0 = split * ktc;
   const int npair = max(min(g.nkt - kt0, ktc), 0) >> 1;
@@ -321,8 +328,16 @@
   const char* baseA = reinterpret_cast<const char*>(g.Ap + batch * g.pstrideA) +
                       (AT ? (long)(tm * 2 * WMT) * 4096 + (long)(kt0 >> 1) * rowA : (long)(tm * 2 * WMT) * rowA + (long)kt0 * 2048);
   const char* baseB = reinterpret_cast<const char*>(g.Bp + batch * g.pstrideB) + (long)(tn * 2 * WNT) * 4096 + (long)(kt0 >> 1) * rowB;
+  [[maybe_unused]] GemmArgsK* gk = PERS ? (GemmArgsK*)__builtin_amdgcn_kernarg_segment_ptr() : nullptr;
+  [[maybe_unused]] auto next_item = [&]() {
+    gemm_tile_of_linear(*gk, lin, total, nbat, &tm, &tn, &batch, &split);
+    m0 = tm * 64 * WMT; n0 = tn * 64 * WNT;
+    baseA = reinterpret_cast<const char*>(gk->Ap + batch * gk->pstrideA) +
+            (AT ? (long)(tm * 2 * WMT) * 4096 + (long)(kt0 >> 1) * rowA : (long)(tm * 2 * WMT) * rowA + (long)kt0 * 2048);
+    baseB = reinterpret_cast<const char*>(gk->Bp + batch * gk->pstrideB) + (long)(tn * 2 * WNT) * 4096 + (long)(kt0 >> 1) * rowB;
+  };
   const int prow = lane >> 1, srow = prow ^ ((prow & 16) ? 4 : 0);
-  const int laneR = lane * 16, laneT = srow * 32 + (lane & 1) * 16;
+  int laneR = lane * 16, laneT = srow * 32 + (lane & 1) * 16;
   int sofX[3], doffX[3], sofY[2], doffY[2];
 #pragma unroll
   for (int i = 0; i < 3; ++i) {
@@ -361,9 +376,19 @@
 #undef PG_RSRC
   const int wm = wave / WNT, wn = wave % WNT;
   const int g4 = lane >> 4, tq = (lane >> 2) & 3, tp = lane & 3;
-  const int fo = (g4 & 1) * 1024 + lfi_u_plane_offset(lane & 15, g4 >> 1);
+  int fo = (g4 & 1) * 1024 + lfi_u_plane_offset(lane & 15, g4 >> 1);
   const int kr = 16 * (g4 & 1) + 8 * (g4 >> 1) + tq;
-  const int toff = (kr ^ ((kr & 16) ? 4 : 0)) * 32 + (((tp >> 1) ^ ((kr >> 3) & 1)) << 4) + (tp & 1) * 8;
+  int toff = (kr ^ ((kr & 16) ? 4 : 0)) * 32 + (((tp >> 1) ^ ((kr >> 3) & 1)) << 4) + (tp & 1) * 8;
+  int lanev = lane;
+  [[maybe_unused]] auto lane_offsets = [&]() {
+    asm volatile("" : "+v"(lanev));
+    const int prow = lanev >> 1, srow = prow ^ ((prow & 16) ? 4 : 0);
+    laneR = lanev * 16; laneT = srow * 32 + (lanev & 1) * 16;
+    const int g4 = lanev >> 4, tq = (lanev >> 2) & 3, tp = lanev & 3;
+    fo = (g4 & 1) * 1024 + lfi_u_plane_offset(lanev & 15, g4 >> 1);
+    const int kr = 16 * (g4 & 1) + 8 * (g4 >> 1) + tq;
+    toff = (kr ^ ((kr & 16) ? 4 : 0)) * 32 + (((tp >> 1) ^ ((kr >> 3) & 1)) << 4) + (tp & 1) * 8;
+  };
   const char* ldsA = lds + (wm * 4) * 1024;
   const char* ldsB = lds + NA * 1024 + (wn * 4) * 1024;
   auto fragA = [&](int slot, int i) -> bf16x8 {
@@ -373,6 +398,10 @@
   auto fragB = [&](int slot, int i) -> bf16x8 { return pg_frag<true>(ldsB + slot * QSLOT + i * 1024, 0, toff); };
 
   f32x4 acc[4][4];
+  gu32x2 sw = {0u, 0u};
+  bool filled = false;
+  if constexpr (PERS) lane_offsets();
+  for (;;) {
 #pragma unroll
   for (int i = 0; i < 4; ++i)
 #pragma unroll
@@ -380,9 +409,14 @@
 
   if (npair > 0) {
     bf16x8 ah[4], bh[4];
-    dmaX(0, 0); dmaY(0, 1); dmaX(1, 2);
-    if (NY == 2) asm volatile("s_waitcnt vmcnt(5)" ::: "memory");
-    else asm volatile("s_waitcnt vmcnt(4)" ::: "memory");
+    if (!filled) {
+      if constexpr (TRP >= 4) sw = gemm_sign_word_load(g, m0, n0, wm, wn, lanev, batch);
+      dmaX(0, 0); dmaY(0, 1); dmaX(1, 2);
+      if (NY == 2) asm volatile("s_waitcnt vmcnt(5)" ::: "memory");
+      else asm volatile("s_waitcnt vmcnt(4)" ::: "memory");
+    } else {
+      asm volatile("s_waitcnt vmcnt(0)" ::: "memory");
+    }
     __builtin_amdgcn_s_barrier();
 #pragma unroll
     for (int i = 0; i < 4; ++i) { ah[i] = fragA(0, i); bh[i] = fragB(0, i); }
@@ -434,13 +468,35 @@
     asm volatile("s_waitcnt vmcnt(0)" ::: "memory");
   }
   if constexpr (TRP != 0) {
-    int lanez = lane, m0z = m0, n0z = n0;
+    int lanez = lanev, m0z = m0, n0z = n0;
+    const int batchz = batch;
+    const gu32x2 swz = sw;
+    bool more = false;
+    if constexpr (PERS) {
+      asm volatile("" : "+s"(gk));
+      lin += lstep;
+      more = lin < total;
+      filled = false;
+      if (more) {
+        next_item();
+        if (npair > 0) {
+          sw = gemm_sign_word_load(*gk, m0, n0, wm, wn, lanev, batch);
+          dmaX(0, 0); dmaY(0, 1); dmaX(1, 2);
+          filled = true;
+        }
+      }
+    }
     asm volatile("" : "+v"(lanez), "+s"(m0z), "+s"(n0z));
-    gemm_epilogue_direct16<TRP>(g, acc, m0z, n0z, wm, wn, lanez, batch, split);
+    if constexpr (PERS) gemm_epilogue_direct16<EMODE>(*gk, acc, m0z, n0z, wm, wn, lanez, batchz, split, swz);
+    else gemm_epilogue_direct16<EMODE>(g, acc, m0z, n0z, wm, wn, lanez, batchz, split, swz);
+    if (!more) break;
+    if constexpr (PERS) lane_offsets();
   } else {
     __syncthreads();
     gemm_epilogue_wide<64 * WNT, 512, 2, COLP, true, true>(g, acc, reinterpret_cast<float*>(xsmem), WNT == 4 ? 64 : 128, m0, n0, wm, wn,
                                                            lane & 31, lane >> 5, batch, split, 64 * WMT);
+    break;
+  }
   }
 }
 
@@ -489,8 +545,40 @@
 
 bool planes16_direct_mask_ok(const GemmArgs& a) {
   if (!lfi_env_on("LFI_PGEMM_DIRECT")) return false;
-  return a.vecC && a.act == 2 && a.Gr && !a.G && a.accumulate == 0 && a.colpart && a.splitk == 1 && a.Cr && !a.storeC && !a.bias &&
+  return a.vecC && a.act == 2 && (a.Gr || a.Si) && !a.G && a.accumulate == 0 && a.colpart && a.splitk == 1 && a.Cr && !a.storeC && !a.bias &&
          (a.N & 3) == 0 && (a.strideC & 31) == 0 && (a.colCr & 15) == 0 && (a.colGr & 15) == 0 && (a.ldpart & 3) == 0;
+}
+
+bool planes_sign_geometry_ok(const GemmArgs& a, int batch) {
+  return a.Cr && (a.nktCr & 3) == 0 && (a.colCr & 63) == 0 && (batch == 1 || (a.strideC & 63) == 0) && a.splitk == 1;
+}
+
+bool planes_takes_direct3(const GemmArgs& a, int at, int bt, bool tall) {
+  if (tall || (bt && planes16t_ok(a))) return false;
+  return !at && !bt && planes16_ok(a) && !a.colpart && planes16_direct_mode(a) == 3;
+}
+bool planes_takes_direct4(const GemmArgs& a, int at, int bt, bool tall) {
+  return bt && planes16t_ok(a) && a.colpart && !tall && !at && planes16_direct_mask_ok(a);
+}
+
+long planes_persist_wgs(long items) {
+  if (!lfi_env_set("LFI_PGEMM_PERSIST")) return 0;
+  constexpr int MAXDEV = 64;
+  static int cus_of[MAXDEV] = {};
+  int dev = 0;
+  if (hipGetDevice(&dev) != hipSuccess || dev < 0 || dev >= MAXDEV) return 0;
+  if (cus_of[dev] == 0) {
+    hipDeviceProp_t prop;
+    if (hipGetDeviceProperties(&prop, dev) != hipSuccess || prop.multiProcessorCount <= 0) return 0;
+    cus_of[dev] = prop.multiProcessorCount;
+  }
+  const int cus = cus_of[dev];
+  long wgs = min(items, 2L * cus);
+  if (const char* e = getenv("LFI_PGEMM_PERSIST_WGS")) {
+    const long cap = atol(e);
+    if (cap > 0) wgs = min(wgs, cap);
+  }
+  return wgs;
 }
 
 template <bool COLP, int WMT, int WNT>
@@ -521,13 +609,19 @@
     if (COLP && WMT == 2 && !at && planes16_direct_mask_ok(a)) {
       static bool attr4 = false;
       if (!attr4) {
-        if (hipFuncSetAttribute((const void*)gemm_planes16t_kernel<false, true, 2, 4, 4>, hipFuncAttributeMaxDynamicSharedMemorySize, (int)lds) != hipSuccess) {
+        if (hipFuncSetAttribute((const void*)gemm_planes16t_kernel<false, true, 2, 4, 4>, hipFuncAttributeMaxDynamicSharedMemorySize, (int)lds) != hipSuccess ||
+            hipFuncSetAttribute((const void*)gemm_planes16t_kernel<false, true, 2, 4, 5>, hipFuncAttributeMaxDynamicSharedMemorySize, (int)lds) != hipSuccess) {
           lfi_set_error("lfi_gemm_planes: cannot reserve %zu bytes of LDS", lds);
           return LFI_ERR_LAUNCH;
         }
         attr4 = true;
       }
-      hipLaunchKernelGGL((gemm_planes16t_kernel<false, true, 2, 4, 4>), grid, dim3(512), lds, st, a);
+      const long items = (long)grid.x * grid.y, wgs = planes_persist_wgs(items);
+      if (wgs > 0 && grid.z == 1) {
+        GemmArgs ap = a;
+        ap.pbatch = (int)grid.y;
+        hipLaunchKernelGGL((gemm_planes16t_kernel<false, true, 2, 4, 5>), dim3((unsigned)wgs), dim3(512), lds, st, ap);
+      } else hipLaunchKernelGGL((gemm_planes16t_kernel<false, true, 2, 4, 4>), grid, dim3(512), lds, st, a);
     } else if (at) hipLaunchKernelGGL((gemm_planes16t_kernel<true, COLP, WMT, WNT>), grid, dim3(512), lds, st, a);
     else hipLaunchKernelGGL((gemm_planes16t_kernel<false, COLP, WMT, WNT>), grid, dim3(512), lds, st, a);
   } else if (!at && !bt && planes16_ok(a) && !COLP && planes16_direct_mode(a)) {
@@ -576,6 +670,11 @@
 extern "C" long lfi_planes_elems(long rows, int cols) {
   if (rows <= 0 || cols <= 0) return 0;
   return ((rows + 255) / 256 * 256) * (long)((cols + 15) / 16 * 16) * 2;
+}
+
+extern "C" long lfi_planes_sign_words(long rows, long cols) {
+  if (rows <= 0 || cols <= 0) return 0;
+  return ((rows + 63) / 64) * ((cols + 63) / 64) * 64;
 }
 
 extern "C" int lfi_planes_from_f32(const float* X, long ldx, long rows, int cols, void* planes, void* stream) {
@@ -605,35 +704,19 @@
   return planes_tall_tile(d) ? (long)lfi_cdiv(d->M, 256) * 2 : (long)lfi_cdiv(d->M, 128) * 2;
 }
 
-extern "C" int lfi_gemm_planes(const lfi_pgemm_desc* d, void* stream) {
-  LFI_REQUIRE(d, "lfi_gemm_planes: null descriptor");
-  LFI_REQUIRE(d->M >= 0 && d->N >= 0 && d->K >= 0 && d->batch >= 1 && d->batch <= 65535, "lfi_gemm_planes: bad dims M=%d N=%d K=%d batch=%d",
-              d->M, d->N, d->K, d->batch);
-  if (d->M == 0 || d->N == 0) return LFI_OK;
+namespace {
+
+int planes_clamped_splitk(const lfi_pgemm_desc* d) {
+  const int nkt = (d->K + 15) / 16;
+  const int splitk = d->splitk < 1 ? 1 : d->splitk;
+  return splitk > nkt ? nkt : splitk;
+}
+
+void planes_args(const lfi_pgemm_desc* d, GemmArgs& a, bool& tall) {
+  const int nkt = (d->K + 15) / 16;
+  const int splitk = planes_clamped_splitk(d);
   const bool store = d->store_f32 != 0;
-  LFI_REQUIRE(d->Ap && d->Bp && (d->C || !store), "lfi_gemm_planes: null operand");
-  LFI_REQUIRE(store || d->Cr, "lfi_gemm_planes: store_f32 = 0 and no plane output: the result would go nowhere");
-  LFI_REQUIRE(d->K > 0, "lfi_gemm_planes: K = 0");
-  LFI_REQUIRE(d->act >= 0 && d->act <= 2 && (d->act != 2 || d->G || d->Gr), "lfi_gemm_planes: bad act %d", d->act);
-  const int nkt = (d->K + 15) / 16;
-  LFI_REQUIRE((d->a_fmt ? 2L * d->a_nkt >= (d->M + 15) / 16 : d->a_nkt >= nkt) && (d->b_fmt ? 2L * d->b_nkt >= (d->N + 15) / 16 : d->b_nkt >= nkt),
-              "lfi_gemm_planes: plane buffers hold %ld / %ld column tiles per row tile: too few for this product", (long)d->a_nkt, (long)d->b_nkt);
-  LFI_REQUIRE(d->a_nkt > 0 && d->b_nkt > 0, "lfi_gemm_planes: a_nkt / b_nkt = column tiles per row tile of the plane buffers");
-  LFI_REQUIRE((reinterpret_cast<uintptr_t>(d->Ap) & 15) == 0 && (reinterpret_cast<uintptr_t>(d->Bp) & 15) == 0 &&
-              (d->a_stride & 7) == 0 && (d->b_stride & 7) == 0, "lfi_gemm_planes: planes must be 16-byte aligned");
-  int splitk = d->splitk < 1 ? 1 : d->splitk;
-  if (splitk > nkt) splitk = nkt;
-  LFI_REQUIRE(splitk == 1 || d->work, "lfi_gemm_planes: splitk needs a workspace");
-  LFI_REQUIRE(splitk == 1 || (!d->Cr && !d->colsum_part && store), "lfi_gemm_planes: plane outputs / column sums need splitk = 1");
-  const bool planes_io = d->Cr || d->Gr;
-  if (planes_io) {
-    LFI_REQUIRE(d->batch == 1 || (d->strideC > 0 && d->strideC * d->batch <= (d->C ? d->ldc : d->strideC * d->batch) && d->strideC % 32 == 0),
-                "lfi_gemm_planes: plane outputs need batch entries side by side in C's columns, 32-column granular");
-    LFI_REQUIRE(d->cr_col0 % 16 == 0 && d->gr_col0 % 16 == 0, "lfi_gemm_planes: plane outputs must start on block boundaries");
-    LFI_REQUIRE((!d->Cr || (reinterpret_cast<uintptr_t>(d->Cr) & 15) == 0) && (!d->Gr || (reinterpret_cast<uintptr_t>(d->Gr) & 15) == 0),
-                "lfi_gemm_planes: planes must be 16-byte aligned");
-  }
-  GemmArgs a = {};
+  a = GemmArgs{};
   a.M = d->M; a.N = d->N; a.K = d->K;
   a.C = d->C; a.ldc = d->ldc; a.bias = d->bias; a.G = d->G; a.ldg = d->ldg;
   a.strideC = d->strideC; a.strideBias = d->strideBias; a.strideG = d->strideG;
@@ -656,12 +739,11 @@
     const bool partial = splitk > 1;
     const bool c_ok = partial ? (((long)d->M * d->N) % 4 == 0 && d->N % 4 == 0 && (reinterpret_cast<uintptr_t>(d->work) & 15) == 0)
                               : (!store || ((reinterpret_cast<uintptr_t>(d->C) & 15) == 0 && d->ldc % 4 == 0 && d->strideC % 4 == 0));
-    const bool g_ok = d->act != 2 || d->Gr || ((reinterpret_cast<uintptr_t>(d->G) & 15) == 0 && d->ldg % 4 == 0 && d->strideG % 4 == 0);
+    const bool g_ok = d->act != 2 || d->Gr || d->sign_in || ((reinterpret_cast<uintptr_t>(d->G) & 15) == 0 && d->ldg % 4 == 0 && d->strideG % 4 == 0);
     a.vecC = (c_ok && g_ok && !(d->act == 2 && d->accumulate != 0)) ? 1 : 0;
-    LFI_REQUIRE(a.vecC || !(planes_io || d->colsum_part), "lfi_gemm_planes: plane outputs / column sums need 16-byte granular C rows");
   }
   a.hiOnly = d->out_hi_only ? 1 : 0;
-  const bool tall = planes_tall_tile(d);
+  tall = planes_tall_tile(d);
   a.tiles_m = lfi_cdiv(d->M, tall ? 256 : 128);
   a.tiles_n = lfi_cdiv(d->N, tall ? 128 : 256);
   {
@@ -671,6 +753,82 @@
       gm_env = e ? atoi(e) : 0;
     }
     a.gm = gm_env > 0 ? gm_env : 8;
+  }
+}
+
+bool planes_signs_path(const GemmArgs& a, const lfi_pgemm_desc* d, bool tall, bool out) {
+  if (!lfi_env_on("LFI_PGEMM_SIGNS")) return false;
+  if (!planes_sign_geometry_ok(a, d->batch)) return false;
+  return out ? planes_takes_direct3(a, d->a_fmt, d->b_fmt, tall) : planes_takes_direct4(a, d->a_fmt, d->b_fmt, tall);
+}
+
+}
+
+extern "C" int lfi_gemm_planes_signs_ok(const lfi_pgemm_desc* d) {
+  if (!d || d->M <= 0 || d->N <= 0 || d->K <= 0 || d->batch < 1 || !d->Ap || !d->Bp) return 0;
+  if (!d->sign_out && !d->sign_in) return 0;
+  GemmArgs a;
+  bool tall;
+  planes_args(d, a, tall);
+  if (d->sign_in) a.Si = reinterpret_cast<const unsigned long long*>(d->sign_in);
+  if (d->sign_out && !planes_signs_path(a, d, tall, true)) return 0;
+  if (d->sign_in && !planes_signs_path(a, d, tall, false)) return 0;
+  return 1;
+}
+
+extern "C" long lfi_gemm_planes_persist_grid(const lfi_pgemm_desc* d) {
+  if (!d || d->M <= 0 || d->N <= 0 || d->K <= 0 || d->batch < 1 || !d->Ap || !d->Bp) return 0;
+  GemmArgs a;
+  bool tall;
+  planes_args(d, a, tall);
+  if (d->sign_in) a.Si = reinterpret_cast<const unsigned long long*>(d->sign_in);
+  if (!planes_takes_direct4(a, d->a_fmt, d->b_fmt, tall) || a.splitk != 1) return 0;
+  return planes_persist_wgs((long)a.tiles_m * a.tiles_n * d->batch);
+}
+
+extern "C" int lfi_gemm_planes(const lfi_pgemm_desc* d, void* stream) {
+  LFI_REQUIRE(d, "lfi_gemm_planes: null descriptor");
+  LFI_REQUIRE(d->M >= 0 && d->N >= 0 && d->K >= 0 && d->batch >= 1 && d->batch <= 65535, "lfi_gemm_planes: bad dims M=%d N=%d K=%d batch=%d",
+              d->M, d->N, d->K, d->batch);
+  if (d->M == 0 || d->N == 0) return LFI_OK;
+  const bool store = d->store_f32 != 0;
+  LFI_REQUIRE(d->Ap && d->Bp && (d->C || !store), "lfi_gemm_planes: null operand");
+  LFI_REQUIRE(store || d->Cr, "lfi_gemm_planes: store_f32 = 0 and no plane output: the result would go nowhere");
+  LFI_REQUIRE(d->K > 0, "lfi_gemm_planes: K = 0");
+  LFI_REQUIRE(d->act >= 0 && d->act <= 2 && (d->act != 2 || d->G || d->Gr || d->sign_in), "lfi_gemm_planes: bad act %d", d->act);
+  const int nkt = (d->K + 15) / 16;
+  LFI_REQUIRE((d->a_fmt ? 2L * d->a_nkt >= (d->M + 15) / 16 : d->a_nkt >= nkt) && (d->b_fmt ? 2L * d->b_nkt >= (d->N + 15) / 16 : d->b_nkt >= nkt),
+              "lfi_gemm_planes: plane buffers hold %ld / %ld column tiles per row tile: too few for this product", (long)d->a_nkt, (long)d->b_nkt);
+  LFI_REQUIRE(d->a_nkt > 0 && d->b_nkt > 0, "lfi_gemm_planes: a_nkt / b_nkt = column tiles per row tile of the plane buffers");
+  LFI_REQUIRE((reinterpret_cast<uintptr_t>(d->Ap) & 15) == 0 && (reinterpret_cast<uintptr_t>(d->Bp) & 15) == 0 &&
+              (d->a_stride & 7) == 0 && (d->b_stride & 7) == 0, "lfi_gemm_planes: planes must be 16-byte aligned");
+  const int splitk = planes_clamped_splitk(d);
+  LFI_REQUIRE(splitk == 1 || d->work, "lfi_gemm_planes: splitk needs a workspace");
+  LFI_REQUIRE(splitk == 1 || (!d->Cr && !d->colsum_part && store), "lfi_gemm_planes: plane outputs / column sums need splitk = 1");
+  const bool planes_io = d->Cr || d->Gr;
+  if (planes_io) {
+    LFI_REQUIRE(d->batch == 1 || (d->strideC > 0 && d->strideC * d->batch <= (d->C ? d->ldc : d->strideC * d->batch) && d->strideC % 32 == 0),
+                "lfi_gemm_planes: plane outputs need batch entries side by side in C's columns, 32-column granular");
+    LFI_REQUIRE(d->cr_col0 % 16 == 0 && d->gr_col0 % 16 == 0, "lfi_gemm_planes: plane outputs must start on block boundaries");
+    LFI_REQUIRE((!d->Cr || (reinterpret_cast<uintptr_t>(d->Cr) & 15) == 0) && (!d->Gr || (reinterpret_cast<uintptr_t>(d->Gr) & 15) == 0),
+                "lfi_gemm_planes: planes must be 16-byte aligned");
+  }
+  GemmArgs a;
+  bool tall;
+  planes_args(d, a, tall);
+  LFI_REQUIRE(a.vecC || !(planes_io || d->colsum_part), "lfi_gemm_planes: plane outputs / column sums need 16-byte granular C rows");
+  if (d->sign_out || d->sign_in) {
+    LFI_REQUIRE(lfi_env_on("LFI_PGEMM_SIGNS"), "lfi_gemm_planes: sign words passed with LFI_PGEMM_SIGNS=0");
+    LFI_REQUIRE(!(d->sign_out && d->sign_in), "lfi_gemm_planes: a product writes sign words or reads them, not both");
+    LFI_REQUIRE(((reinterpret_cast<uintptr_t>(d->sign_out) | reinterpret_cast<uintptr_t>(d->sign_in)) & 7) == 0,
+                "lfi_gemm_planes: sign words must be 8-byte aligned");
+    LFI_REQUIRE(!d->sign_in || (d->act == 2 && !d->Gr && !d->G), "lfi_gemm_planes: sign_in is the act-2 mask: act = 2, and neither G nor Gr");
+    if (d->sign_in) a.Si = reinterpret_cast<const unsigned long long*>(d->sign_in);
+    LFI_REQUIRE(planes_signs_path(a, d, tall, d->sign_out != nullptr),
+                "lfi_gemm_planes: this product cannot take sign words (lfi_gemm_planes_signs_ok: direct plane epilogue, 128 x 256 tiles, Cr columns / "
+                "cr_col0 / strideC in 64s, splitk 1)");
+    if (d->sign_out) a.So = reinterpret_cast<unsigned long long*>(d->sign_out);
+    a.npcS = d->cr_nkt / 4;
   }
   const size_t lds = (size_t)QRING * QSLOT;
   dim3 grid(a.tiles_m * a.tiles_n, d->batch, splitk);
diff --git a/lets_face_it_amd/engine.py b/lets_face_it_amd/engine.py
--- a/lets_face_it_amd/engine.py
+++ b/lets_face_it_amd/engine.py
@@ -204,6 +204,7 @@
         self._sample_fp16_unsafe = False
         self.backward_products = self.check_backward_products(os.environ.get("LFI_BWD_PRODUCTS", "auto"))
         self._bwd_skip = 0
+        self._signs_ok = {}
         self.tile_pin = {k.strip(): int(v) for k, v in (it.split("=") for it in os.environ.get("LFI_TILE_PIN", "").split(",") if it)}
         self.pass_skip = {}
         env = os.environ.get("LFI_PASS_SKIP", "")
@@ -442,7 +443,8 @@
     def gemm_planes(self, M, N, K, Ap, a_nkt, Bp, b_nkt, Cm, ldc, bias=None, act=0, slope=0.01, G=None, ldg=0, batch=1,
                     a_stride=0, b_stride=0, sC=0, sBias=0, sG=0, accumulate=0, c_off=0, bias_off=0, tag=None, cls=None,
                     a_fmt=0, b_fmt=0, a_off=0, b_off=0, splitk=1, ws="scratch.pgemm_splitk", store=True,
-                    Cr=None, cr_nkt=0, cr_col0=0, Gr=None, gr_nkt=0, gr_col0=0, colsum_into=None, hi_only=False, tile=0):
+                    Cr=None, cr_nkt=0, cr_col0=0, Gr=None, gr_nkt=0, gr_col0=0, colsum_into=None, hi_only=False, tile=0,
+                    sign_out=None, sign_in=None, signs_query=False, persist_query=False):
         g = PGemmDesc()
         g.skip = self._skip_bits(cls)
         g.M, g.N, g.K = M, N, K
@@ -461,12 +463,17 @@
         g.Cr, g.cr_nkt, g.cr_col0 = ptr(Cr), cr_nkt, cr_col0
         g.Gr, g.gr_nkt, g.gr_col0 = ptr(Gr), gr_nkt, gr_col0
         g.out_hi_only, g.tile = (1 if hi_only else 0), tile
+        g.sign_out, g.sign_in = ptr(sign_out), ptr(sign_in)
         part, prow = None, 0
         if colsum_into is not None and os.environ.get("LFI_NO_COLPART") != "1":
             prow = int(self.L.lfi_gemm_planes_colpart_rows(C.byref(g)))
             if prow > 0:
                 part = self._buf("scratch.colpart", prow * ldc)
                 g.colsum_part, g.ld_part = part.data_ptr(), ldc
+        if signs_query:
+            return bool(self.L.lfi_gemm_planes_signs_ok(C.byref(g)))
+        if persist_query:
+            return int(self.L.lfi_gemm_planes_persist_grid(C.byref(g)))
         ev = self._tic(tag)
         check(self.L.lfi_gemm_planes(C.byref(g), _stream()), "lfi_gemm_planes")
         self._toc(tag, ev)
@@ -659,8 +666,27 @@
             wp, nkw = self._wct_planes
             nkKD = KD // 16
             c_r = self.plane_buf("c_r", self.L.lfi_planes_elems(F, KD) + 256 * KD * 2)
-            self.gemm_planes(F, KD, s.ldf, cp, nkc, wp, nkw, None, KD, bias=self.fview("bct"), act=1, slope=0.01, store=False,
-                             Cr=c_r, cr_nkt=nkKD, tag="gemm_cond_fwd", cls="cond_fwd")
+            fwd = dict(bias=self.fview("bct"), act=1, slope=0.01, store=False, Cr=c_r, cr_nkt=nkKD, tag="gemm_cond_fwd", cls="cond_fwd")
+            signs = None
+            if with_stash:
+                env = os.environ.get
+                key = (F, self.backward_product_count(F), env("LFI_PGEMM_SIGNS"), env("LFI_PGEMM_DIRECT"), env("LFI_PGEMM_16"),
+                       env("LFI_PGEMM_16T"), env("LFI_NO_COLPART"),
+                       tuple(sorted(self.pass_skip.items())) if self.pass_skip else (), tuple(sorted(self.tile_pin.items())) if self.tile_pin else ())
+                ok = self._signs_ok.get(key)
+                if ok is None:
+                    saved = self._bwd_skip
+                    self._bwd_skip = 1 if key[1] == 2 else 0
+                    try:
+                        ok = (self.gemm_planes(F, KD, s.ldf, cp, nkc, wp, nkw, None, KD, sign_out=c_r, signs_query=True, **fwd)
+                              and self._dpre_product(c_r, F, c_r, signs_query=True))
+                    finally:
+                        self._bwd_skip = saved
+                    self._signs_ok[key] = ok
+                if ok:
+                    signs = self._buf("c_signs", 2 * self.L.lfi_planes_sign_words(F, KD))
+            self._c_signs = signs
+            self.gemm_planes(F, KD, s.ldf, cp, nkc, wp, nkw, None, KD, sign_out=signs, **fwd)
             gic = self._buf("gic", s.Ks * F * s.G)
             wr, nkwr = self._wc_r
             self.gemm_planes(F, s.G, s.D, c_r, nkKD, wr, nkwr, gic, s.G, bias=self.fview("b_ih"), batch=s.Ks,
@@ -713,6 +739,7 @@
         ctx.batch, ctx.masks, ctx.B, ctx.T, ctx.N, ctx.F = batch, masks, B, T, N, F
         ctx.cond, ctx.cbuf, ctx.gic, ctx.stash, ctx.dims, ctx.with_stash, ctx.chain = cond, cbuf, gic, stash, dims, with_stash, chain
         ctx.enc_stash_f16 = dict(self._enc_stash_f16)
+        ctx.signs = self._c_signs if (chain and with_stash) else None
         self._last = ctx
         return z, nll
 
@@ -799,7 +826,6 @@
         nkKD, nkG, nkD = KD // 16, G // 16, D // 16
         dgi_p = self.plane_buf("dgi_planes", self.L.lfi_planes_elems(Ks * F, G) + 256 * G * 2)
         dgi_hi = all(self._skip_bits(c) & 1 for c in ("dpre", "flow_pgrads"))
-        dpre_hi = all(self._skip_bits(c) & 1 for c in ("cond_wgrad", "cond_dgrad"))
         pg_skip = self._skip_bits("flow_pgrads")
         g16 = bool((pg_skip & 1) and not (pg_skip & 2) and (self.precision & 1) and os.environ.get("LFI_FLOW_G16", "1") != "0")
         bdims = dims
@@ -821,11 +847,7 @@
         check(self.L.lfi_flow_param_grads(C.byref(pg_dims), C.byref(p), self.prep.data_ptr(), ctx.stash.data_ptr(),
                                           bst.data_ptr(), None, KD, gscale, C.byref(g), 0, work.data_ptr(),
                                           st, side.cuda_stream if side is not None else None), "lfi_flow_param_grads")
-        wr, nkwr = self._wc_r
-        bct_done = self.gemm_planes(F, D, G, dgi_p, nkG, wr, nkwr, None, KD, act=2, slope=0.01, batch=Ks, b_fmt=1,
-                                    a_stride=(F // 32) * nkG * 1024, b_stride=(G // 32) * nkwr * 1024, sC=D, store=False,
-                                    Gr=c_r, gr_nkt=nkKD, Cr=c_r, cr_nkt=nkKD, hi_only=dpre_hi,
-                                    colsum_into=self.fview("bct", self.grads), tag="gemm_dpre", cls="dpre")
+        bct_done = self._dpre_product(c_r, F, ctx.signs)
         if not bct_done:
             raise _lib.LfiError("the dpre product on planes did not take the column-sum epilogue")
         dpre_p = c_r
@@ -848,6 +870,19 @@
             self.gemm_planes(F, W, KD, dpre_p, nkKD, wp, nkw, dcond, ldd, b_fmt=1, b_off=(col0 // 16) * 1024,
                              splitk=self._planes_splitk(F, W, KD), tag="gemm_cond_dgrad", cls="cond_dgrad")
             self._encoders_backward(rnn, ctx, dcond, ldd, col0)
+
+    def _dpre_product(self, c_r, F, signs, signs_query=False):
+        s = self.spec
+        KD, G, D, Ks = s.Ks * s.D, s.G, s.D, s.Ks
+        nkKD, nkG = KD // 16, G // 16
+        dgi_p = self.plane_buf("dgi_planes", self.L.lfi_planes_elems(Ks * F, G) + 256 * G * 2)
+        dpre_hi = all(self._skip_bits(c) & 1 for c in ("cond_wgrad", "cond_dgrad"))
+        wr, nkwr = self._wc_r
+        return self.gemm_planes(F, D, G, dgi_p, nkG, wr, nkwr, None, KD, act=2, slope=0.01, batch=Ks, b_fmt=1,
+                                a_stride=(F // 32) * nkG * 1024, b_stride=(G // 32) * nkwr * 1024, sC=D, store=False,
+                                Gr=(None if signs is not None else c_r), gr_nkt=nkKD, Cr=c_r, cr_nkt=nkKD, hi_only=dpre_hi,
+                                sign_in=signs, signs_query=signs_query,
+                                colsum_into=self.fview("bct", self.grads), tag="gemm_dpre", cls="dpre")
 
     def _encoders_backward(self, rnn, ctx, dcond, ldd, col0):
         order = self._bptt_order(rnn)
```

Result: faster. 2.228 million (median of 6 runs) (+1.3%).
